# RohitMovva/VexAutonomousPlanner

Measured on NVIDIA B200. Metric: profiled trajectories/sec (8-node paths), higher is better.
Workload: dtype f64

## Files before the change

include/vap.h:

```cpp
#ifndef VAP_H
#define VAP_H

#include <stdint.h>

#ifdef __cplusplus
extern "C" {
#endif

#define VAP_NODE_ATTRS 12
#define VAP_AP_ATTRS 4
#define VAP_FLAG_REVERSE 1
#define VAP_FLAG_STOP 2
#define VAP_FLAG_TANGENT 4

#define VAP_OK 0
#define VAP_ERR_FALSE (-1)
#define VAP_ERR_INDEX (-2)
#define VAP_ERR_VALUE (-3)
#define VAP_ERR_CAPACITY (-4)
#define VAP_ERR_DIVERGED (-5)
#define VAP_ERR_EVENTS (-6)

int vap_version(void);
const char* vap_last_error(void);

int vap_build_path(int64_t B, int N_max, const double* node_attr, const int32_t* node_flags,
                   const int32_t* n_nodes, double* seg, int32_t* first_node, double* param_end,
                   double* seglen, int32_t* n_splines, int32_t* status, double* scratch, double* params,
                   double* derivs, void* stream);

int vap_fit_splines(int64_t R, int n_max, const int32_t* n_pts, const double* xy, const int32_t* tan_has,
                    const double* tan_in, const double* tan_out, const int32_t* bnd_has, const double* bnd,
                    double* seg, double* seglen, double* params, int32_t* status, double* scratch,
                    const double* deriv_in, double* deriv_out, void* stream);

int vap_eval(int64_t n, const int32_t* path, const double* t, int which, int N_max, const double* seg,
             const int32_t* first_node, const double* param_end, const int32_t* n_splines, double* out,
             void* stream);

int vap_build_lut(int64_t B, int N_max, const double* seg, const int32_t* first_node, const double* param_end,
                  const int32_t* n_splines, const int32_t* status, int samples, int64_t Q_cap, double* lut_d,
                  double* lut_t, double* total_len, void* stream);
int64_t vap_lut_index_row_ints(int64_t Q_cap);
int vap_build_lut_index(int64_t B, const int32_t* n_splines, const int32_t* status, int samples, int64_t Q_cap,
                        const double* lut_d, const double* total_len, int32_t* lut_inv, void* stream);

int vap_build_props(int64_t B, int N_max, const int32_t* n_nodes, const double* seg, const int32_t* first_node,
                    const double* param_end, const int32_t* n_splines, const int32_t* status, int spn,
                    int64_t P_cap, double* prop_k, double* prop_h, void* stream);

int vap_query_tables(int64_t n, const int32_t* path, const double* x, int what, const int32_t* n_nodes,
                     const int32_t* n_splines, int samples, int64_t Q_cap, const double* lut_d,
                     const double* lut_t, const double* total_len, int spn, int64_t P_cap, const double* prop_k,
                     const double* prop_h, double* out, void* stream);

int vap_build_dgrid(int64_t n, double dd, double* dgrid, void* stream);

int vap_dist_sample(int64_t B, const int32_t* n_nodes, const int32_t* n_splines, int32_t* status, int64_t n_grid,
                    const double* dgrid, int samples, int64_t Q_cap, const double* lut_d, const double* lut_t,
                    const double* total_len, int spn, int64_t P_cap, const double* prop_k, const double* prop_h,
                    int64_t D_cap, int32_t* n_samples, double* t, double* kap, double* th, void* stream);

int vap_fwd_bwd(int64_t B, int N_max, int A_max, const double* node_attr, const int32_t* node_flags,
                const int32_t* n_nodes, const double* ap_attr, const int32_t* ap_flags, const int32_t* n_ap,
                const double* cons, const int32_t* status, double dd, double dt, double start_vel, double end_vel,
                int64_t D_cap, const int32_t* n_samples, const double* t, const double* kap, const double* th,
                double* vel, int E_cap, double* max_accels, int32_t* bidx, int32_t* bval, int32_t* n_ev,
                double* t_est, int mode, void* stream);

int vap_dist_sample_events(int64_t B, int N_max, int A_max, const double* node_attr, const int32_t* node_flags,
                           const int32_t* n_nodes, const double* ap_attr, const int32_t* ap_flags, const int32_t* n_ap,
                           const double* cons, const int32_t* n_splines, int32_t* status, int64_t n_grid,
                           const double* dgrid, int samples, int64_t Q_cap, const double* lut_d, const double* lut_t,
                           const double* total_len, int spn, int64_t P_cap, const double* prop_k, const double* prop_h,
                           int64_t D_cap, int32_t* n_samples, double* t, double* kap, double* th, int E_cap,
                           double* max_accels, int32_t* bidx, int32_t* bval, int32_t* n_ev, int32_t* vr_idx,
                           double* vr_val, int32_t* st_idx, int32_t* n_vr, double dt, float* ins_est,
                           int32_t* ev_scratch, const int32_t* lut_inv, void* stream);
int64_t vap_event_scratch_ints(int64_t B, int N_max, int A_max);
int64_t vap_pass_row_slots(int64_t D_cap, int chunks);
int vap_fwd_bwd_chunked(int64_t B, const double* cons, const int32_t* status, double dd, double dt, double start_vel,
                        double end_vel, int64_t D_cap, const int32_t* n_samples, const double* kap, const double* th,
                        int E_cap, const double* max_accels, const int32_t* bidx, const int32_t* bval,
                        const int32_t* n_ev, const int32_t* vr_idx, const double* vr_val, const int32_t* st_idx,
                        const int32_t* n_vr, double* rec, double* statB, double* vel_f, double* vel, float* t_est,
                        int32_t* rounds, int chunks, int mode, void* stream);

int vap_velocity_profile(int64_t B, int N_max, int A_max, const double* node_attr, const int32_t* node_flags,
                         const int32_t* n_nodes, const double* ap_attr, const int32_t* ap_flags, const int32_t* n_ap,
                         const double* cons, const int32_t* n_splines, int32_t* status, int64_t n_grid,
                         const double* dgrid, int samples, int64_t Q_cap, const double* lut_d, const double* lut_t,
                         const double* total_len, int spn, int64_t P_cap, const double* prop_k, const double* prop_h,
                         const int32_t* lut_inv, double dd, double dt, double start_vel, double end_vel, int64_t D_cap,
                         int32_t* n_samples, double* t, double* kap, double* th, int E_cap, double* max_accels,
                         int32_t* bidx, int32_t* bval, int32_t* n_ev, int32_t* vr_idx, double* vr_val, int32_t* st_idx,
                         int32_t* n_vr, float* ins_est, int32_t* ev_scratch, double* rec, double* statB, double* vel_f,
                         double* vel, float* t_est, int32_t* rounds, int chunks, int mode, void* stream);

int vap_resample(int64_t B, int N_max, int A_max, const double* node_attr, const int32_t* node_flags,
                 const int32_t* n_nodes, const double* ap_attr, const int32_t* ap_flags, const int32_t* n_ap,
                 const double* cons, int32_t* status, double dt, double dd, const double* seg,
                 const int32_t* first_node, const double* param_end, const int32_t* n_splines, int samples,
                 int64_t Q_cap, const double* lut_d, const double* lut_t, const double* total_len, int spn,
                 int64_t P_cap, const double* prop_k, const double* prop_h, int64_t D_cap,
                 const int32_t* n_samples, const double* vel, int64_t T_cap, double* out, int32_t* nodes_map,
                 int32_t* actions_map, int32_t* n_maps, int32_t* n_out, double* summary, void* stream);

int vap_time_profile(int64_t B, int N_max, int A_max, const double* node_attr, const int32_t* node_flags,
                     const int32_t* n_nodes, const double* ap_attr, const int32_t* ap_flags, const int32_t* n_ap,
                     const double* cons, int32_t* status, double dt, double dd, const double* seg,
                     const int32_t* first_node, const double* param_end, const int32_t* n_splines, int samples,
                     int64_t Q_cap, const double* lut_d, const double* lut_t, const double* total_len, int spn,
                     int64_t P_cap, const double* prop_k, const double* prop_h, int64_t D_cap,
                     const int32_t* n_samples, const double* vel, int64_t T_cap, double* out, int32_t* nodes_map,
                     int32_t* actions_map, int32_t* n_maps, int32_t* n_out, double* summary, int32_t* n_main,
                     double* stage, int E_cap, int32_t* seg_tab, int32_t* ev_scratch, int64_t out_plane_stride,
                     const int32_t* lut_inv, const double* rden, int64_t n_rden, void* stream);
int vap_build_lerp_recip(int64_t n, double dd, double* rden, void* stream);

int64_t vap_workspace_bytes(int64_t B, int N_max, int A_max, int max_splines, int lut_samples, int samples_per_node,
                            int64_t D_cap, int64_t T_cap, int chunks);
int vap_profile_batch(int64_t B, int N_max, int A_max, int max_splines, const double* node_attr,
                      const int32_t* node_flags, const int32_t* n_nodes, const double* ap_attr, const int32_t* ap_flags,
                      const int32_t* n_ap, const double* cons, double dt, double dd, double start_vel, double end_vel,
                      int lut_samples, int samples_per_node, int64_t D_cap, int64_t T_cap, int chunks, const double* dgrid,
                      int64_t n_grid, const double* rden, int64_t n_rden, void* workspace, int64_t workspace_bytes,
                      double* out, int64_t out_plane_stride, int32_t* n_out, int32_t* nodes_map, int32_t* actions_map,
                      int32_t* n_maps, int32_t* status, double* summary, double* vel, int32_t* n_samples, int64_t* need,
                      void* stream);
int vap_summary(int64_t B, int64_t T_cap, int64_t out_plane_stride, const double* out, const int32_t* n_out,
                const int32_t* status, const double* total_len, double* summary, void* stream);

int vap_gl(int64_t n, const int32_t* path, const int32_t* spl, const double* a, const double* b, int mode,
           int max_iter, int npts, const double* gl_pts, const double* gl_wts, int N_max, const double* seg,
           const int32_t* first_node, const double* param_end, double* out, int32_t* qstatus, void* stream);

int vap_turn_profile(int64_t n, const double* q, int mode, int64_t K_cap, double* out_a, double* out_b,
                     int32_t* counts, void* stream);

int vap_lerp(int64_t n, const double* x, int64_t m, const double* xs, const double* ys, double* out, void* stream);
int vap_wheel_trajectory(int64_t n, const double* lin, const double* ang, double track_width, double* left,
                         double* right, void* stream);

int vap_pack_rows(int64_t B, int64_t T_cap, int64_t out_plane_stride, const double* out, const int32_t* n_out,
                  const int32_t* status, int64_t* offsets, double* dst, void* stream);

int vap_export_rows(int64_t B, int64_t T_cap, int64_t out_plane_stride, const double* out, const int32_t* n_out,
                    const int32_t* status, int64_t* offsets, double* dst, void* stream);

int vap_row_kinds(int64_t B, int N_max, int A_max, const double* node_attr, const int32_t* n_nodes, const double* ap_attr,
                  const int32_t* n_ap, const double* cons, const int32_t* status, double dt, const int32_t* nodes_map,
                  const int32_t* actions_map, const int32_t* n_maps, const int32_t* n_out, int64_t T_cap,
                  const int64_t* offsets, int64_t n_kinds, uint8_t* kinds, void* stream);
int vap_format_doubles(int64_t n, const double* x, char* out32, int32_t* lens, void* stream);
int vap_row_text_stride(void);
int vap_format_rows(int64_t R, const double* rows, const uint8_t* kinds, char* slots, int32_t* lens, void* stream);
int vap_compact_rows(int64_t R, const char* slots, const int32_t* lens, const int64_t* offsets, char* text, void* stream);

int vap_diag_read(uint64_t* out_host, int reset);

int vap_bench_dfma(int64_t ctas, int64_t iters, double* out, void* stream);

int vap_test_div_const(int64_t n, uint64_t seed, double b, uint64_t* bad, void* stream);
int vap_test_div_recip(int64_t n, uint64_t seed, uint64_t* bad, void* stream);

#ifdef __cplusplus
}
#endif
#endif
```

vexautonomousplanner_b200/csrc/vap_device.cuh:

```cuda
#pragma once
#include <cstdint>
#include <math.h>

#define NA 12
enum { A_X = 0, A_Y, A_TURN, A_WAIT, A_MAXVEL, A_MAXACC, A_TX, A_TY, A_INMAG, A_OUTMAG, A_RCOS, A_RSIN };
#define F_REVERSE 1
#define F_STOP 2
#define F_TANGENT 4
#define APA 4
enum { P_T = 0, P_WAIT, P_MAXVEL, P_MAXACC };

#define ST_OK 0
#define ST_FALSE (-1)
#define ST_INDEX (-2)
#define ST_VALUE (-3)
#define ST_CAPACITY (-4)
#define ST_DIVERGED (-5)
#define ST_EVENTS (-6)
#define VAP_ROW_LIMIT 50000000LL

#define VAP_PI 3.141592653589793

__device__ __forceinline__ void cp_async16(void* smem, const void* gmem)
{
    unsigned sa = (unsigned)__cvta_generic_to_shared(smem);
    asm volatile("cp.async.ca.shared.global [%0], [%1], 16;" ::"r"(sa), "l"(gmem));
}
__device__ __forceinline__ void cp_async_commit() { asm volatile("cp.async.commit_group;" ::); }
template <int N>
__device__ __forceinline__ void cp_async_wait() { asm volatile("cp.async.wait_group %0;" ::"n"(N) : "memory"); }

__device__ __forceinline__ void mbar_init(unsigned a, unsigned count)
{
    asm volatile("mbarrier.init.shared::cta.b64 [%0], %1;" ::"r"(a), "r"(count) : "memory");
}
__device__ __forceinline__ void mbar_expect_tx(unsigned a, unsigned bytes)
{
    asm volatile("mbarrier.arrive.expect_tx.shared::cta.b64 _, [%0], %1;" ::"r"(a), "r"(bytes) : "memory");
}
__device__ __forceinline__ void bulk_g2s(unsigned dst, const void* src, unsigned bytes, unsigned mbar)
{
    asm volatile("cp.async.bulk.shared::cluster.global.mbarrier::complete_tx::bytes [%0], [%1], %2, [%3];"
                 ::"r"(dst), "l"(src), "r"(bytes), "r"(mbar) : "memory");
}
__device__ __forceinline__ void mbar_wait(unsigned a, unsigned parity)
{
    asm volatile("{\n"
                 ".reg .pred P1;\n"
                 "LAB_WAIT:\n"
                 "mbarrier.try_wait.parity.shared::cta.b64 P1, [%0], %1;\n"
                 "@P1 bra DONE;\n"
                 "bra LAB_WAIT;\n"
                 "DONE:\n"
                 "}" ::"r"(a), "r"(parity) : "memory");
}

__device__ __forceinline__ void fence_mbar_init() { asm volatile("fence.mbarrier_init.release.cluster;" ::: "memory"); }
__device__ __forceinline__ void fence_proxy_async() { asm volatile("fence.proxy.async.shared::cta;" ::: "memory"); }

#ifdef VAP_BOUNDS_CHECK
#define VAP_DIAG_SITES 32
__device__ unsigned long long g_vap_diag[VAP_DIAG_SITES];
#define VAP_CHECK(site, cond) do { if (!(cond)) atomicAdd(&g_vap_diag[site], 1ull); else atomicAdd(&g_vap_diag[16 + ((site) & 15)], 1ull); } while (0)
#else
#define VAP_CHECK(site, cond) do { } while (0)
#endif

struct PathTile { long long b; unsigned x; };
__device__ __forceinline__ PathTile path_tile(unsigned tiles_x)
{
    PathTile p;
    const unsigned q = blockIdx.x / tiles_x;
    p.b = q; p.x = blockIdx.x - q * tiles_x;
    return p;
}

__device__ __forceinline__ double pymin(double a, double b) { return (b < a) ? b : a; }
__device__ __forceinline__ double pymax(double a, double b) { return (b > a) ? b : a; }
__device__ __forceinline__ double norm1d(double x, double y) { return sqrt(fma(y, y, x * x)); }
__device__ __forceinline__ double norm_ax1(double x, double y) { return sqrt(x * x + y * y); }
__device__ __forceinline__ double frac1(double t) { return t - floor(t); }
__device__ __forceinline__ double pymod_pos(double x, double y)
{
    double m = fmod(x, y);
    if (m != 0.0) { if (m < 0) m += y; } else m = 0.0;
    return m;
}

template <int WHICH>
__device__ __forceinline__ void basis(double t, double* H)
{
    double t2 = t * t, t3 = t2 * t;
    if (WHICH == 0) {
        double t4 = t3 * t, t5 = t4 * t;
        H[0] = 1 - 10 * t3 + 15 * t4 - 6 * t5;
        H[1] = 10 * t3 - 15 * t4 + 6 * t5;
        H[2] = t - 6 * t3 + 8 * t4 - 3 * t5;
        H[3] = -4 * t3 + 7 * t4 - 3 * t5;
        H[4] = 0.5 * t2 - 1.5 * t3 + 1.5 * t4 - 0.5 * t5;
        H[5] = 0.5 * t3 - t4 + 0.5 * t5;
    } else if (WHICH == 1) {
        double t4 = t3 * t;
        H[0] = -30 * t2 + 60 * t3 - 30 * t4;
        H[1] = 30 * t2 - 60 * t3 + 30 * t4;
        H[2] = 1 - 18 * t2 + 32 * t3 - 15 * t4;
        H[3] = -12 * t2 + 28 * t3 - 15 * t4;
        H[4] = t - 4.5 * t2 + 6 * t3 - 2.5 * t4;
        H[5] = 1.5 * t2 - 4 * t3 + 2.5 * t4;
    } else {
        H[0] = -60 * t + 180 * t2 - 120 * t3;
        H[1] = 60 * t - 180 * t2 + 120 * t3;
        H[2] = -36 * t + 96 * t2 - 60 * t3;
        H[3] = -24 * t + 84 * t2 - 60 * t3;
        H[4] = 1 - 9 * t + 18 * t2 - 10 * t3;
        H[5] = 3 * t - 12 * t2 + 10 * t3;
    }
}

__device__ __forceinline__ void normalize_param(double t, int nseg, double pend, int& idx, double& u)
{
    double tt = pymax(0.0, pymin(t, pend));
    idx = (int)tt;
    if (idx == nseg) idx = nseg - 1;
    u = tt - (double)idx;
}

template <int WHICH>
__device__ __forceinline__ void eval_spline(const double* __restrict__ seg, int nseg, double pend, double t,
                                            double& ox, double& oy)
{
    int idx; double u;
    normalize_param(t, nseg, pend, idx, u);
    double H[6];
    basis<WHICH>(u, H);
    const double2* s = reinterpret_cast<const double2*>(seg + (size_t)idx * 12);
    double ax = 0.0, ay = 0.0;
#pragma unroll
    for (int i = 0; i < 6; i++) { double2 r = __ldg(s + i); ax += H[i] * r.x; ay += H[i] * r.y; }
    ox = ax; oy = ay;
}

__device__ __forceinline__ void eval_spline_d12(const double* __restrict__ seg, int nseg, double pend, double t,
                                                double& dx, double& dy, double& ddx, double& ddy)
{
    int idx; double u;
    normalize_param(t, nseg, pend, idx, u);
    double H1[6], H2[6];
    basis<1>(u, H1);
    basis<2>(u, H2);
    const double2* s = reinterpret_cast<const double2*>(seg + (size_t)idx * 12);
    double ax = 0.0, ay = 0.0, bx = 0.0, by = 0.0;
#pragma unroll
    for (int i = 0; i < 6; i++) {
        double2 r = __ldg(s + i);
        ax += H1[i] * r.x; ay += H1[i] * r.y;
        bx += H2[i] * r.x; by += H2[i] * r.y;
    }
    dx = ax; dy = ay; ddx = bx; ddy = by;
}

struct PathGeo {
    const double* seg;
    const int* first;
    const double* pend;
    int S;
};
__device__ __forceinline__ int map_spline(const PathGeo& g, double t)
{
    int k = 0;
    if (g.S <= 8) {
        while (k < g.S - 1 && !(t <= (double)g.first[k + 1])) k++;
    } else {
        int lo = 0, hi = g.S - 1;
        while (lo < hi) {
            int mid = (lo + hi) >> 1;
            if (t <= (double)g.first[mid + 1]) hi = mid; else lo = mid + 1;
        }
        k = lo;
    }
    return k;
}
__device__ __forceinline__ PathGeo path_geo(long long b, int N_max, const double* seg, const int* first_node,
                                            const double* param_end, const int* n_splines)
{
    PathGeo g;
    g.seg = seg + (size_t)b * (N_max - 1) * 12;
    g.first = first_node + (size_t)b * (N_max + 1);
    g.pend = param_end + (size_t)b * N_max;
    g.S = n_splines[b];
    return g;
}

template <int WHICH>
__device__ __forceinline__ void eval_path(const PathGeo& g, double t, double& ox, double& oy)
{
    int k = map_spline(g, t);
    int f0 = g.first[k], f1 = g.first[k + 1];
    eval_spline<WHICH>(g.seg + (size_t)f0 * 12, f1 - f0, g.pend[k], t - (double)f0, ox, oy);
}
__device__ __forceinline__ void eval_path_d12(const PathGeo& g, double t, double& dx, double& dy, double& ddx,
                                              double& ddy)
{
    int k = map_spline(g, t);
    int f0 = g.first[k], f1 = g.first[k + 1];
    eval_spline_d12(g.seg + (size_t)f0 * 12, f1 - f0, g.pend[k], t - (double)f0, dx, dy, ddx, ddy);
}

__device__ __forceinline__ void curv_heading(double dx, double dy, double ddx, double ddy, double& kap, double& th)
{
    double s2 = dx * dx + dy * dy;
    double num = dx * ddy - dy * ddx;
// ... 208 lines not shown
```

vexautonomousplanner_b200/csrc/vap_kernels.cu:

```cuda
#include <cuda_runtime.h>
#include <cstdio>
#include <cstring>
#include <cstdlib>

#include "../../include/vap.h"
#include "vap_device.cuh"
#include "vap_velocity.cuh"
#include "vap_timeloop.cuh"
#include "vap_format.cuh"

static thread_local char g_err[512] = "";
static int set_err(const char* where, cudaError_t e)
{
    snprintf(g_err, sizeof(g_err), "%s: %s", where, cudaGetErrorString(e));
    return -100;
}
static int arg_err(const char* msg)
{
    snprintf(g_err, sizeof(g_err), "%s", msg);
    return -101;
}
#define CHECK_LAUNCH(name)                                   \
    do {                                                     \
        cudaError_t e__ = cudaGetLastError();                \
// ... 999 lines not shown
    CHECK_LAUNCH("vap_build_dgrid");
    return 0;
}

extern "C" int vap_build_lerp_recip(int64_t n, double dd, double* rden, void* stream)
{
    if (n <= 0) return 0;
    k_build_lerp_recip<<<blocks_for(n, 256), 256, 0, STREAM>>>(n, dd, rden);
    CHECK_LAUNCH("vap_build_lerp_recip");
    return 0;
}

extern "C" int vap_dist_sample(int64_t B, const int32_t* n_nodes, const int32_t* n_splines, int32_t* status,
                               int64_t n_grid, const double* dgrid, int samples, int64_t Q_cap, const double* lut_d,
                               const double* lut_t, const double* total_len, int spn, int64_t P_cap,
                               const double* prop_k, const double* prop_h, int64_t D_cap, int32_t* n_samples,
                               double* t, double* kap, double* th, void* stream)
{
    if (B <= 0) return 0;
    k_count_samples<<<blocks_for(B, 128), 128, 0, STREAM>>>(B, status, status, n_grid, dgrid, total_len, D_cap, n_samples);
    CHECK_LAUNCH("vap_dist_sample/count");
    const unsigned tx = blocks_for(D_cap, 256);
    if ((long long)tx * B > 2147483647LL) return arg_err("vap_dist_sample: more than 2^31 CTAs (tile the batch)");
    const unsigned grid = tx * (unsigned)B;
    k_dist_sample<<<grid, 256, 0, STREAM>>>(n_nodes, n_splines, status, dgrid, samples, Q_cap, lut_d, lut_t, total_len,
                                            spn, P_cap, prop_k, prop_h, D_cap, n_samples, t, kap, th, tx);
    CHECK_LAUNCH("vap_dist_sample");
    return 0;
}

extern "C" int vap_fwd_bwd(int64_t B, int N_max, int A_max, const double* node_attr, const int32_t* node_flags,
                           const int32_t* n_nodes, const double* ap_attr, const int32_t* ap_flags, const int32_t* n_ap,
                           const double* cons, const int32_t* status, double dd, double dt, double start_vel,
                           double end_vel, int64_t D_cap, const int32_t* n_samples, const double* t, const double* kap,
                           const double* th, double* vel, int E_cap, double* max_accels, int32_t* bidx, int32_t* bval,
                           int32_t* n_ev, double* t_est, int mode, void* stream)
{
    if (B <= 0) return 0;
    if (E_cap < N_max + A_max + 2) return arg_err("vap_fwd_bwd: E_cap < N_max + A_max + 2");
    k_fwd_bwd<<<blocks_for(B, 32), 32, 0, STREAM>>>(B, N_max, A_max, node_attr, node_flags, n_nodes, ap_attr, ap_flags,
                                                   n_ap, cons, status, dd, dt, start_vel, end_vel, D_cap, n_samples, t,
                                                   kap, th, vel, E_cap, max_accels, bidx, bval, n_ev, t_est, mode);
    CHECK_LAUNCH("vap_fwd_bwd");
    return 0;
}

extern "C" int vap_resample(int64_t B, int N_max, int A_max, const double* node_attr, const int32_t* node_flags,
                            const int32_t* n_nodes, const double* ap_attr, const int32_t* ap_flags, const int32_t* n_ap,
                            const double* cons, int32_t* status, double dt, double dd, const double* seg,
                            const int32_t* first_node, const double* param_end, const int32_t* n_splines, int samples,
                            int64_t Q_cap, const double* lut_d, const double* lut_t, const double* total_len, int spn,
                            int64_t P_cap, const double* prop_k, const double* prop_h, int64_t D_cap,
                            const int32_t* n_samples, const double* vel, int64_t T_cap, double* out,
                            int32_t* nodes_map, int32_t* actions_map, int32_t* n_maps, int32_t* n_out, double* summary,
                            void* stream)
{
    if (B <= 0) return 0;
    k_resample<<<blocks_for(B, 32), 32, 0, STREAM>>>(B, N_max, A_max, node_attr, node_flags, n_nodes, ap_attr, ap_flags,
                                                    n_ap, cons, status, dt, dd, seg, first_node, param_end, n_splines,
                                                    samples, Q_cap, lut_d, lut_t, total_len, spn, P_cap, prop_k, prop_h,
                                                    D_cap, n_samples, vel, T_cap, out, nodes_map, actions_map, n_maps,
                                                    n_out, summary, 0, 0);
    CHECK_LAUNCH("vap_resample");
    return 0;
}

extern "C" int vap_gl(int64_t n, const int32_t* path, const int32_t* spl, const double* a, const double* b, int mode,
                      int max_iter, int npts, const double* gl_pts, const double* gl_wts, int N_max, const double* seg,
                      const int32_t* first_node, const double* param_end, double* out, int32_t* qstatus, void* stream)
{
    if (n <= 0) return 0;
    if (npts < 1 || npts > 128) return arg_err("vap_gl: npts must be in [1, 128]");
    k_gl<<<blocks_for(n, 64), 64, 0, STREAM>>>(n, path, spl, a, b, mode, max_iter, npts, gl_pts, gl_wts, N_max, seg,
                                              first_node, param_end, out, qstatus);
    CHECK_LAUNCH("vap_gl");
    return 0;
}

extern "C" int vap_turn_profile(int64_t n, const double* q, int mode, int64_t K_cap, double* out_a, double* out_b,
                                int32_t* counts, void* stream)
{
    if (n <= 0) return 0;
    k_turn_profile<<<blocks_for(n, 64), 64, 0, STREAM>>>(n, q, mode, K_cap, out_a, out_b, counts);
    CHECK_LAUNCH("vap_turn_profile");
    return 0;
}

extern "C" int vap_lerp(int64_t n, const double* x, int64_t m, const double* xs, const double* ys, double* out,
                        void* stream)
{
    if (n <= 0) return 0;
    if (m < 1) return arg_err("vap_lerp: empty table");
    k_lerp<<<blocks_for(n, 128), 128, 0, STREAM>>>(n, x, m, xs, ys, out);
    CHECK_LAUNCH("vap_lerp");
    return 0;
}

extern "C" int vap_wheel_trajectory(int64_t n, const double* lin, const double* ang, double track_width, double* left,
                                    double* right, void* stream)
{
    if (n <= 0) return 0;
    k_wheel<<<blocks_for(n, 256), 256, 0, STREAM>>>(n, lin, ang, track_width, left, right);
    CHECK_LAUNCH("vap_wheel_trajectory");
    return 0;
}

extern "C" int vap_dist_sample_events(int64_t B, int N_max, int A_max, const double* node_attr,
                                      const int32_t* node_flags, const int32_t* n_nodes, const double* ap_attr,
                                      const int32_t* ap_flags, const int32_t* n_ap, const double* cons,
                                      const int32_t* n_splines, int32_t* status, int64_t n_grid, const double* dgrid,
                                      int samples, int64_t Q_cap, const double* lut_d, const double* lut_t,
                                      const double* total_len, int spn, int64_t P_cap, const double* prop_k,
                                      const double* prop_h, int64_t D_cap, int32_t* n_samples, double* t, double* kap,
                                      double* th, int E_cap, double* max_accels, int32_t* bidx, int32_t* bval,
                                      int32_t* n_ev, int32_t* vr_idx, double* vr_val, int32_t* st_idx, int32_t* n_vr,
                                      double dt, float* ins_est, int32_t* ev_scratch, const int32_t* lut_inv,
                                      void* stream)
{
    if (B <= 0) return 0;
    if (E_cap < N_max + A_max + 2) return arg_err("vap_dist_sample_events: E_cap < N_max + A_max + 2");
    int Am = A_max > 0 ? A_max : 1;
    int32_t* ev_wrap = ev_scratch;
    int32_t* ev_nwrap = ev_wrap + (size_t)B * N_max;
    int32_t* ev_apc = ev_nwrap + B;
    int32_t* ev_napc = ev_apc + (size_t)B * Am * EV_AP_CAND;
    cudaError_t e = cudaMemsetAsync(ev_nwrap, 0, sizeof(int32_t) * (size_t)B, STREAM);
    if (e != cudaSuccess) return set_err("vap_dist_sample_events/memset", e);
    e = cudaMemsetAsync(ev_napc, 0, sizeof(int32_t) * (size_t)B * Am, STREAM);
    if (e != cudaSuccess) return set_err("vap_dist_sample_events/memset", e);
    k_count_samples<<<blocks_for(B, 128), 128, 0, STREAM>>>(B, status, status, n_grid, dgrid, total_len, D_cap, n_samples);
    CHECK_LAUNCH("vap_dist_sample_events/count");
    const unsigned tx = blocks_for(D_cap, 256);
    if ((long long)tx * B > 2147483647LL) return arg_err("vap_dist_sample_events: more than 2^31 CTAs (tile the batch)");
    const unsigned grid = tx * (unsigned)B;
    k_dist_sample_ev<<<grid, 256, 0, STREAM>>>(N_max, Am, n_nodes, n_splines, status, ap_attr, n_ap, dgrid, samples, Q_cap,
                                               lut_d, lut_t, total_len, spn, P_cap, prop_k, prop_h, D_cap, n_samples, t,
                                               kap, th, ev_wrap, ev_nwrap, ev_apc, ev_napc, lut_inv, tx);
    CHECK_LAUNCH("vap_dist_sample_events/sample");
    k_resolve_events<<<blocks_for(B, 64), 64, 0, STREAM>>>(B, N_max, Am, node_attr, node_flags, n_nodes, ap_attr, ap_flags,
                                                          n_ap, cons, status, ev_wrap, ev_nwrap, ev_apc, ev_napc, E_cap,
                                                          max_accels, bidx, bval, n_ev, vr_idx, vr_val, st_idx, n_vr, dt, ins_est);
    CHECK_LAUNCH("vap_dist_sample_events/resolve");
    return 0;
}

extern "C" int64_t vap_event_scratch_ints(int64_t B, int N_max, int A_max)
{
    int Am = A_max > 0 ? A_max : 1;
    return B * N_max + B + B * Am * EV_AP_CAND + B * Am;
}

extern "C" int64_t vap_pass_row_slots(int64_t D_cap, int chunks) { return ((D_cap + 8 * (int64_t)chunks + 64 + 1) / 2) * 2; }

template <int NT, bool TMA>
static int launch_passes_v(int64_t B, size_t ss, cudaStream_t st, const double* cons, const int32_t* status, double dd, double dt,
                           double start_vel, double end_vel, long long RS, long long D_cap, const int32_t* n_samples,
                           const double* rec, int E_cap, const double* max_accels, const int32_t* bidx, const int32_t* bval,
                           const int32_t* n_ev, const int32_t* vr_idx, const double* vr_val, const int32_t* st_idx,
                           const int32_t* n_vr, double* vel_f, double* vel, float* t_est, int32_t* rounds, bool backward,
                           int warm, int max_rounds, const double* statB)
{
    const int warps = (NT + 31) / 32;
    const int ring_off = (int)((ss + 127) / 128 * 128);
    const int planes = backward ? 6 : 5;
    const size_t smem = TMA ? (size_t)ring_off + (size_t)warps * (2 * planes * TMA_PLANE_DOUBLES * 8 + 16) : ss;
    cudaError_t e = cudaSuccess;
    if (!backward) {
        if (smem > 48 * 1024) e = cudaFuncSetAttribute(k_fwd_chunked<NT, TMA>, cudaFuncAttributeMaxDynamicSharedMemorySize, (int)smem);
        if (e != cudaSuccess) return set_err("vap_fwd_bwd_chunked/attr", e);
        k_fwd_chunked<NT, TMA><<<(unsigned)B, NT, smem, st>>>(status, cons, dd, start_vel, end_vel, RS, n_samples, rec, E_cap,
                                                             max_accels, bidx, bval, n_ev, vr_idx, vr_val, st_idx, n_vr, vel_f,
                                                             rounds, warm, max_rounds, ring_off);
    } else {
        if (smem > 48 * 1024) e = cudaFuncSetAttribute(k_bwd_chunked<NT, TMA>, cudaFuncAttributeMaxDynamicSharedMemorySize, (int)smem);
        if (e != cudaSuccess) return set_err("vap_fwd_bwd_chunked/attr", e);
        k_bwd_chunked<NT, TMA><<<(unsigned)B, NT, smem, st>>>(status, cons, dd, dt, end_vel, RS, D_cap, n_samples, rec, E_cap,
                                                             max_accels, bidx, bval, n_ev, vel_f, vel, t_est, rounds, warm,
                                                             max_rounds, statB, ring_off);
    }
    return 0;
}
template <int NT, typename... Args>
static int launch_passes(bool tma, Args... args)
{
    return tma ? launch_passes_v<NT, true>(args...) : launch_passes_v<NT, false>(args...);
}

static int run_passes(int64_t B, const double* cons, const int32_t* status, double dd, double dt, double start_vel,
                      double end_vel, int64_t D_cap, const int32_t* n_samples, int E_cap, const double* max_accels,
                      const int32_t* bidx, const int32_t* bval, const int32_t* n_ev, const int32_t* vr_idx,
                      const double* vr_val, const int32_t* st_idx, const int32_t* n_vr, const double* rec,
                      const double* statB, double* vel_f, double* vel, float* t_est, int32_t* rounds, int chunks, int mode,
                      cudaStream_t stream)
{
    const long long RS = vap_pass_row_slots(D_cap, chunks);
    const size_t VC = 3 * (size_t)E_cap + 2;
    const size_t ss = ((size_t)chunks * 4 + E_cap + VC) * sizeof(double) + (E_cap + VC) * sizeof(int);
    int warm = 0, max_rounds = 1 << 30;
    if (const char* ev = getenv("VAP_CHUNK_WARM")) warm = atoi(ev);
#ifdef VAP_DIAG_MAXROUNDS
    if (const char* ev = getenv("VAP_CHUNK_MAXROUNDS")) max_rounds = atoi(ev);
#endif
    if (warm < 0) warm = 0;
    bool tma = true;
    if (const char* ev = getenv("VAP_PASS_TMA")) tma = atoi(ev) != 0;
    auto passes = [&](bool backward) -> int {
        switch (chunks) {
#define VAP_PASS_CASE(N_) case N_: return launch_passes<N_>(tma, B, ss, STREAM, cons, status, dd, dt, start_vel, end_vel, RS, D_cap,   \
                                              n_samples, rec, E_cap, max_accels, bidx, bval, n_ev, vr_idx, vr_val, st_idx, n_vr,  \
                                              vel_f, vel, t_est, rounds, backward, warm, max_rounds, statB);
            VAP_PASS_CASE(8) VAP_PASS_CASE(16) VAP_PASS_CASE(32) VAP_PASS_CASE(64) VAP_PASS_CASE(128) VAP_PASS_CASE(256)
#undef VAP_PASS_CASE
        }
        return 0;
    };
    if (int rc = passes(false)) return rc;
    CHECK_LAUNCH("vap_fwd_bwd_chunked/fwd");
    if (mode == 1) {
        const unsigned tx2 = blocks_for(D_cap, 256);
        if ((long long)tx2 * B > 2147483647LL) return arg_err("vap_fwd_bwd_chunked: more than 2^31 CTAs (tile the batch)");
        k_untranspose<<<tx2 * (unsigned)B, 256, 0, STREAM>>>(status, n_samples, D_cap, RS, chunks, vel_f, vel, tx2);
        CHECK_LAUNCH("vap_fwd_bwd_chunked/untranspose");
        return 0;
    }
    if (int rc = passes(true)) return rc;
    CHECK_LAUNCH("vap_fwd_bwd_chunked/bwd");
    return 0;
}

static int check_pass_args(const char* who, int64_t B, int64_t D_cap, int chunks)
{
    (void)B;
    if (chunks < 8 || chunks > 256 || (chunks & (chunks - 1)) != 0) { snprintf(g_err, sizeof(g_err), "%s: chunks must be a power of two in 8 .. 256", who); return -1; }
    if (D_cap > 400000000LL) { snprintf(g_err, sizeof(g_err), "%s: D_cap too large", who); return -1; }
    if (D_cap & 1) { snprintf(g_err, sizeof(g_err), "%s: D_cap must be even (the passes move 16-byte pairs)", who); return -1; }
    return 0;
}

extern "C" int vap_fwd_bwd_chunked(int64_t B, const double* cons, const int32_t* status, double dd, double dt,
                                   double start_vel, double end_vel, int64_t D_cap, const int32_t* n_samples,
                                   const double* kap, const double* th, int E_cap, const double* max_accels,
                                   const int32_t* bidx, const int32_t* bval, const int32_t* n_ev, const int32_t* vr_idx,
                                   const double* vr_val, const int32_t* st_idx, const int32_t* n_vr, double* rec,
                                   double* statB, double* vel_f, double* vel, float* t_est, int32_t* rounds,
                                   int chunks, int mode, void* stream)
{
    if (B <= 0) return 0;
    if (check_pass_args("vap_fwd_bwd_chunked", B, D_cap, chunks)) return -1;
    const long long RS = vap_pass_row_slots(D_cap, chunks);
    const unsigned tx = blocks_for(D_cap + 4 * chunks, 256 * PP_TILES);
    if ((long long)tx * B > 2147483647LL) return arg_err("vap_fwd_bwd_chunked: more than 2^31 CTAs (tile the batch)");
    const unsigned grid = tx * (unsigned)B;
    const size_t sm = 2 * 2 * sizeof(double) * (size_t)prepass_tile_cols(chunks) * prepass_tile_stride(chunks);
    k_prepass<<<grid, 256, sm, STREAM>>>(status, cons, D_cap, n_samples, kap, th, chunks, RS, rec, E_cap, max_accels, bidx,
                                         bval, n_ev, statB, tx);
    CHECK_LAUNCH("vap_fwd_bwd_chunked/prepass");
    return run_passes(B, cons, status, dd, dt, start_vel, end_vel, D_cap, n_samples, E_cap, max_accels, bidx, bval, n_ev, vr_idx,
                      vr_val, st_idx, n_vr, rec, statB, vel_f, vel, t_est, rounds, chunks, mode, STREAM);
}

extern "C" int vap_velocity_profile(int64_t B, int N_max, int A_max, const double* node_attr, const int32_t* node_flags,
                                    const int32_t* n_nodes, const double* ap_attr, const int32_t* ap_flags,
                                    const int32_t* n_ap, const double* cons, const int32_t* n_splines, int32_t* status,
                                    int64_t n_grid, const double* dgrid, int samples, int64_t Q_cap, const double* lut_d,
                                    const double* lut_t, const double* total_len, int spn, int64_t P_cap,
                                    const double* prop_k, const double* prop_h, const int32_t* lut_inv, double dd, double dt,
                                    double start_vel, double end_vel, int64_t D_cap, int32_t* n_samples, double* t,
                                    double* kap, double* th, int E_cap, double* max_accels, int32_t* bidx, int32_t* bval,
                                    int32_t* n_ev, int32_t* vr_idx, double* vr_val, int32_t* st_idx, int32_t* n_vr,
                                    float* ins_est, int32_t* ev_scratch, double* rec, double* statB, double* vel_f,
                                    double* vel, float* t_est, int32_t* rounds, int chunks, int mode, void* stream)
{
    if (B <= 0) return 0;
    if (E_cap < N_max + A_max + 2) return arg_err("vap_velocity_profile: E_cap < N_max + A_max + 2");
    if (check_pass_args("vap_velocity_profile", B, D_cap, chunks)) return -1;
    if ((t != nullptr) != (kap != nullptr) || (t != nullptr) != (th != nullptr))
        return arg_err("vap_velocity_profile: t, kap and th are inspection outputs: pass all three or none");
    int Am = A_max > 0 ? A_max : 1;
    int32_t* ev_wrap = ev_scratch;
    int32_t* ev_nwrap = ev_wrap + (size_t)B * N_max;
    int32_t* ev_apc = ev_nwrap + B;
    int32_t* ev_napc = ev_apc + (size_t)B * Am * EV_AP_CAND;
    cudaError_t e = cudaMemsetAsync(ev_nwrap, 0, sizeof(int32_t) * (size_t)B, STREAM);
    if (e != cudaSuccess) return set_err("vap_velocity_profile/memset", e);
    e = cudaMemsetAsync(ev_napc, 0, sizeof(int32_t) * (size_t)B * Am, STREAM);
    if (e != cudaSuccess) return set_err("vap_velocity_profile/memset", e);
    k_count_samples<<<blocks_for(B, 128), 128, 0, STREAM>>>(B, status, status, n_grid, dgrid, total_len, D_cap, n_samples);
    CHECK_LAUNCH("vap_velocity_profile/count");
    const long long RS = vap_pass_row_slots(D_cap, chunks);
    const unsigned tx = blocks_for(D_cap + 4 * chunks, 256 * SP_TILES);
    if ((long long)tx * B > 2147483647LL) return arg_err("vap_velocity_profile: more than 2^31 CTAs (tile the batch)");
    const int tc = prepass_tile_cols(chunks);
    const size_t sm = 2 * 3 * sizeof(double) * (size_t)tc * (((256 / tc) + 2) | 1);
    k_sample_prepass<<<tx * (unsigned)B, 256, sm, STREAM>>>(N_max, Am, n_nodes, n_splines, status, cons, ap_attr, n_ap, dgrid,
                                                           samples, Q_cap, lut_d, lut_t, total_len, spn, P_cap, prop_k, prop_h,
                                                           D_cap, n_samples, t, kap, th, ev_wrap, ev_nwrap, ev_apc, ev_napc,
                                                           lut_inv, chunks, RS, rec, tx);
    CHECK_LAUNCH("vap_velocity_profile/sample_prepass");
    k_resolve_events<<<blocks_for(B, 64), 64, 0, STREAM>>>(B, N_max, Am, node_attr, node_flags, n_nodes, ap_attr, ap_flags,
                                                          n_ap, cons, status, ev_wrap, ev_nwrap, ev_apc, ev_napc, E_cap,
                                                          max_accels, bidx, bval, n_ev, vr_idx, vr_val, st_idx, n_vr, dt, ins_est);
    CHECK_LAUNCH("vap_velocity_profile/resolve");
    k_prepass_ovr<<<(unsigned)B, 256, 0, STREAM>>>(status, cons, n_samples, chunks, RS, rec, E_cap, max_accels, bidx, bval, n_ev,
                                                  statB);
    CHECK_LAUNCH("vap_velocity_profile/prepass_ovr");
    return run_passes(B, cons, status, dd, dt, start_vel, end_vel, D_cap, n_samples, E_cap, max_accels, bidx, bval, n_ev, vr_idx,
                      vr_val, st_idx, n_vr, rec, statB, vel_f, vel, t_est, rounds, chunks, mode, STREAM);
}

extern "C" int vap_time_profile(int64_t B, int N_max, int A_max, const double* node_attr, const int32_t* node_flags,
                                const int32_t* n_nodes, const double* ap_attr, const int32_t* ap_flags,
                                const int32_t* n_ap, const double* cons, int32_t* status, double dt, double dd,
                                const double* seg, const int32_t* first_node, const double* param_end,
                                const int32_t* n_splines, int samples, int64_t Q_cap, const double* lut_d,
                                const double* lut_t, const double* total_len, int spn, int64_t P_cap,
                                const double* prop_k, const double* prop_h, int64_t D_cap, const int32_t* n_samples,
                                const double* vel, int64_t T_cap, double* out, int32_t* nodes_map,
                                int32_t* actions_map, int32_t* n_maps, int32_t* n_out, double* summary,
                                int32_t* n_main, double* stage, int E_cap, int32_t* seg_tab, int32_t* ev_scratch,
                                int64_t out_plane_stride, const int32_t* lut_inv, const double* rden, int64_t n_rden,
                                void* stream)
{
    const long long oplane = out_plane_stride > 0 ? out_plane_stride : B * T_cap;
    if (B <= 0) return 0;
    if (E_cap < N_max + A_max + 2) return arg_err("vap_time_profile: E_cap < N_max + A_max + 2");
    int Am = A_max > 0 ? A_max : 1;
    const int64_t M_cap = T_cap;
    int32_t* ev_wrap = ev_scratch;
    int32_t* ev_nwrap = ev_wrap + (size_t)B * N_max;
    int32_t* ev_apc = ev_nwrap + B;
    int32_t* ev_napc = ev_apc + (size_t)B * Am * EV_AP_CAND;
    int32_t* seg_k = seg_tab;
    int32_t* seg_off = seg_k + (size_t)B * E_cap;
    int32_t* seg_rev = seg_off + (size_t)B * E_cap;
    int32_t* n_seg = seg_rev + (size_t)B * E_cap;
    cudaError_t e = cudaMemsetAsync(ev_nwrap, 0, sizeof(int32_t) * (size_t)B, STREAM);
    if (e != cudaSuccess) return set_err("vap_time_profile/memset", e);
    e = cudaMemsetAsync(ev_napc, 0, sizeof(int32_t) * (size_t)B * Am, STREAM);
    if (e != cudaSuccess) return set_err("vap_time_profile/memset", e);
    if (D_cap % 128 != 0) return arg_err("vap_time_profile: D_cap must be a multiple of 128 (rows are staged in 128-sample blocks)");
    int lanes = (int)((B + 591) / 592);
    if (lanes > 10) lanes = 10;
    if (const char* ev = getenv("VAP_STATE_LANES")) lanes = atoi(ev);
    lanes = lanes < 1 ? 1 : (lanes > 32 ? 32 : lanes);
    bool big = B > 148 * 32;
    if (const char* ev = getenv("VAP_STATE_BLK")) big = atoi(ev) == 64;
    const size_t ring_bytes = (size_t)lanes * ((big ? ts_stride(64) : ts_stride(128)) * sizeof(double) + 16);
    if (ring_bytes > 48 * 1024) {
        const int mx = (int)(32 * (ts_stride(128) * sizeof(double) + 16));
        cudaError_t ea = big ? cudaFuncSetAttribute(k_time_state<64>, cudaFuncAttributeMaxDynamicSharedMemorySize, mx)
                             : cudaFuncSetAttribute(k_time_state<128>, cudaFuncAttributeMaxDynamicSharedMemorySize, mx);
        if (ea != cudaSuccess) return set_err("vap_time_profile/attr", ea);
    }
    if (big)
        k_time_state<64><<<blocks_for(B, lanes), lanes, ring_bytes, STREAM>>>(B, cons, status, dt, dd, total_len, D_cap, n_samples,
                                                                             vel, M_cap, stage, n_main, rden, rden ? n_rden : 0);
    else
        k_time_state<128><<<blocks_for(B, lanes), lanes, ring_bytes, STREAM>>>(B, cons, status, dt, dd, total_len, D_cap, n_samples,
                                                                              vel, M_cap, stage, n_main, rden, rden ? n_rden : 0);
    CHECK_LAUNCH("vap_time_profile/state");
    const unsigned tx = blocks_for(M_cap, 256);
    if ((long long)tx * B > 2147483647LL) return arg_err("vap_time_profile: more than 2^31 CTAs (tile the batch)");
    const unsigned grid = tx * (unsigned)B;
    k_time_sample<<<grid, 256, 0, STREAM>>>(B, N_max, Am, n_nodes, status, ap_attr, n_ap, seg, first_node, param_end,
                                            n_splines, samples, Q_cap, lut_d, lut_t, total_len, spn, P_cap, prop_k, prop_h,
                                            M_cap, n_main, stage, ev_wrap, ev_nwrap, ev_apc, ev_napc, lut_inv, tx);
    CHECK_LAUNCH("vap_time_profile/sample");
    k_time_events<<<blocks_for(B, lanes), lanes, 0, STREAM>>>(B, N_max, Am, node_attr, node_flags, n_nodes, ap_attr, n_ap, cons,
                                                       status, dt, seg, first_node, param_end, n_splines, spn, P_cap,
                                                       prop_h, total_len, M_cap, n_main, stage, ev_wrap, ev_nwrap, ev_apc,
                                                       ev_napc, E_cap, seg_k, seg_off, seg_rev, n_seg, T_cap, oplane,
                                                       out, nodes_map, actions_map, n_maps, n_out, summary);
    CHECK_LAUNCH("vap_time_profile/events");
    k_time_finalize<<<grid, 256, 0, STREAM>>>(B, status, M_cap, n_main, stage, E_cap, seg_k, seg_off, seg_rev, n_seg,
                                              T_cap, oplane, out, summary, tx);
    CHECK_LAUNCH("vap_time_profile/finalize");
    k_resample<<<blocks_for(B, 32), 32, 0, STREAM>>>(B, N_max, A_max, node_attr, node_flags, n_nodes, ap_attr, ap_flags, n_ap,
                                                    cons, status, dt, dd, seg, first_node, param_end, n_splines, samples,
                                                    Q_cap, lut_d, lut_t, total_len, spn, P_cap, prop_k, prop_h, D_cap,
                                                    n_samples, vel, T_cap, out, nodes_map, actions_map, n_maps, n_out,
                                                    summary, oplane, ST_EVENTS);
    CHECK_LAUNCH("vap_time_profile/serial redo");
    return 0;
}

__global__ void __launch_bounds__(256) k_bench_dfma(long long iters, double* __restrict__ out)
{
    double a[8];
#pragma unroll
    for (int k = 0; k < 8; k++) a[k] = 1.0 + 1e-9 * (double)(threadIdx.x + 37 * k);
    const double m = 0.9999999, c = 1e-7;
    for (long long i = 0; i < iters; i++) {
#pragma unroll
        for (int k = 0; k < 8; k++) a[k] = fma(a[k], m, c);
    }
    double s = 0.0;
#pragma unroll
    for (int k = 0; k < 8; k++) s += a[k];
    if (s == 123456.789) out[0] = s;
}
extern "C" int vap_bench_dfma(int64_t ctas, int64_t iters, double* out, void* stream)
{
    if (ctas <= 0 || iters <= 0) return 0;
    k_bench_dfma<<<(unsigned)ctas, 256, 0, STREAM>>>(iters, out);
    CHECK_LAUNCH("vap_bench_dfma");
    return 0;
}

extern "C" int vap_test_div_const(int64_t n, uint64_t seed, double b, uint64_t* bad, void* stream)
{
    if (n <= 0) return 0;
    k_test_div_const<<<blocks_for(n, 256), 256, 0, STREAM>>>(n, seed, b, reinterpret_cast<unsigned long long*>(bad));
    CHECK_LAUNCH("vap_test_div_const");
    return 0;
}

__global__ void k_test_div_recip(long long n, unsigned long long seed, unsigned long long* __restrict__ bad)
{
    long long i = (long long)blockIdx.x * blockDim.x + threadIdx.x;
    if (i >= n) return;
    auto mix = [](unsigned long long z) {
        z = (z ^ (z >> 30)) * 0xBF58476D1CE4E5B9ULL; z = (z ^ (z >> 27)) * 0x94D049BB133111EBULL; return z ^ (z >> 31);
    };
    unsigned long long z1 = mix(seed + 0x9E3779B97F4A7C15ULL * (unsigned long long)(2 * i + 1));
    unsigned long long z2 = mix(seed + 0x9E3779B97F4A7C15ULL * (unsigned long long)(2 * i + 2));
    int e1 = (int)((z1 >> 52) % 118) - 110 + 1023;
    unsigned long long nb = ((z1 >> 63) << 63) | ((unsigned long long)e1 << 52) | (z1 & 0x000FFFFFFFFFFFFFULL);
    if (((z1 >> 40) & 63) == 0) nb &= 0x8000000000000000ULL;
    double num = __longlong_as_double((long long)nb);
    int e2 = (int)((z2 >> 52) % 60) - 57 + 1023;
    unsigned long long gb = ((unsigned long long)e2 << 52) | (z2 & 0x000FFFFFFFFFFFFFULL);
    if (((z2 >> 40) & 63) == 1) gb |= 0x000FFFFFFFFFFFFFULL;
    double g = __longlong_as_double((long long)gb);
    if (((z2 >> 46) & 31) == 0) g = 0.0;
    const double rc = recip_for_pass(g);
    const double q1 = accel_ang_fast(num, g, rc);
    double n2 = num, g2 = g;
    asm volatile("" : "+d"(n2), "+d"(g2));
    const double q2 = n2 / g2;
    bool same = (__double_as_longlong(q1) == __double_as_longlong(q2)) || (q1 != q1 && q2 != q2) || (q1 == 0.0 && q2 == 0.0);
    if (!same) atomicAdd(bad, 1ULL);
}
extern "C" int vap_test_div_recip(int64_t n, uint64_t seed, uint64_t* bad, void* stream)
{
    if (n <= 0) return 0;
    k_test_div_recip<<<blocks_for(n, 256), 256, 0, STREAM>>>(n, seed, reinterpret_cast<unsigned long long*>(bad));
    CHECK_LAUNCH("vap_test_div_recip");
    return 0;
}

extern "C" int vap_pack_rows(int64_t B, int64_t T_cap, int64_t out_plane_stride, const double* out, const int32_t* n_out,
                             const int32_t* status, int64_t* offsets, double* dst, void* stream)
{
    if (B <= 0) return 0;
    const long long oplane = out_plane_stride > 0 ? out_plane_stride : B * T_cap;
    k_row_offsets<<<1, 1024, 0, STREAM>>>(B, n_out, status, T_cap, reinterpret_cast<long long*>(offsets));
    CHECK_LAUNCH("vap_pack_rows/offsets");
    int ctas = 16;
    if (const char* ev = getenv("VAP_PACK_CTAS")) ctas = atoi(ev);
    if (ctas < 1) ctas = 1;
    k_pack_rows<<<ctas, 256, 0, STREAM>>>(B, n_out, status, T_cap, oplane, out, reinterpret_cast<const long long*>(offsets), dst);
    CHECK_LAUNCH("vap_pack_rows");
    return 0;
}

extern "C" int vap_export_rows(int64_t B, int64_t T_cap, int64_t out_plane_stride, const double* out, const int32_t* n_out,
                               const int32_t* status, int64_t* offsets, double* dst, void* stream)
{
    if (B <= 0) return 0;
    const long long oplane = out_plane_stride > 0 ? out_plane_stride : B * T_cap;
    k_row_offsets<<<1, 1024, 0, STREAM>>>(B, n_out, status, T_cap, reinterpret_cast<long long*>(offsets));
    CHECK_LAUNCH("vap_export_rows/offsets");
    const unsigned tx = blocks_for(T_cap, 256);
    if ((long long)tx * B > 2147483647LL) return arg_err("vap_export_rows: more than 2^31 CTAs (tile the batch)");
    const unsigned grid = tx * (unsigned)B;
    k_export_rows<<<grid, 256, 0, STREAM>>>(B, n_out, status, T_cap, oplane, out, reinterpret_cast<const long long*>(offsets), dst, tx);
    CHECK_LAUNCH("vap_export_rows");
    return 0;
}

extern "C" int vap_format_doubles(int64_t n, const double* x, char* out32, int32_t* lens, void* stream)
{
    if (n <= 0) return 0;
    k_format_doubles<<<blocks_for(n, 256), 256, 0, STREAM>>>(n, x, out32, lens);
    CHECK_LAUNCH("vap_format_doubles");
    return 0;
}
extern "C" int vap_row_text_stride(void) { return VAP_ROW_STRIDE; }
__global__ void k_row_kinds(long long B, int N_max, int A_max, const double* __restrict__ node_attr,
                            const int* __restrict__ n_nodes, const double* __restrict__ ap_attr, const int* __restrict__ n_ap,
                            const double* __restrict__ cons, const int* __restrict__ status, double dt,
                            const int* __restrict__ nodes_map, const int* __restrict__ actions_map,
                            const int* __restrict__ n_maps, const int* __restrict__ n_out, long long T_cap,
                            const long long* __restrict__ offsets, unsigned char* __restrict__ kinds)
{
    long long b = (long long)blockIdx.x * blockDim.x + threadIdx.x;
    if (b >= B || status[b] != ST_OK) return;
    long long T = n_out[b];
    if (T > T_cap) T = T_cap;
    unsigned char* kr = kinds + (offsets ? offsets[b] : b * T_cap);
    auto mark = [&](long long r0, long long cnt, unsigned char k) {
        for (long long r = r0; r < r0 + cnt && r < T; r++) if (r >= 0) kr[r] |= k;
    };
    const double* na = node_attr + (size_t)b * N_max * NA;
    const double V = cons[b * 6 + 0], max_acc = cons[b * 6 + 1], w = cons[b * 6 + 5];
    if (na[A_WAIT] > 0) mark(0, (long long)(na[A_WAIT] / dt), RK_INSERTED | RK_OMEGA_INT | RK_POS_INT);
    else if (T > 0) kr[0] |= RK_TIME_INT;
    const int nm = n_maps[2 * b], am = n_maps[2 * b + 1];
    const int* nmap = nodes_map + (size_t)b * (N_max + 1);
    const int n = n_nodes[b];
    for (int i = 1; i < nm - 1 && i < n; i++) {
        const double* a = na + (size_t)i * NA;
        long long r = nmap[i];
        if (a[A_TURN] != 0) {
            const double angle = a[A_TURN] * (VAP_PI / 180.0);
            const Trapezoid tz = trapezoid_setup(V, max_acc, fabs(angle) * w / 2, dt);
            mark(r, 1, RK_INSERTED | RK_OMEGA_INT);
            mark(r + 1, tz.K - 1, RK_INSERTED);
            r += tz.K;
        }
        if (a[A_WAIT] > 0) mark(r, (long long)(a[A_WAIT] / dt), RK_INSERTED | RK_OMEGA_INT | RK_POS_INT);
    }
    const int* amap = actions_map + (size_t)b * (A_max > 0 ? A_max : 1);
    const int A = n_ap ? n_ap[b] : 0;
    for (int j = 0; j < am && j < A; j++) {
        const double wt = ap_attr[((size_t)b * A_max + j) * APA + P_WAIT];
        if (wt > 0) mark(amap[j], (long long)(wt / dt), RK_INSERTED | RK_OMEGA_INT | RK_POS_INT);
    }
}

extern "C" int vap_row_kinds(int64_t B, int N_max, int A_max, const double* node_attr, const int32_t* n_nodes,
                             const double* ap_attr, const int32_t* n_ap, const double* cons, const int32_t* status,
                             double dt, const int32_t* nodes_map, const int32_t* actions_map, const int32_t* n_maps,
                             const int32_t* n_out, int64_t T_cap, const int64_t* offsets, int64_t n_kinds, uint8_t* kinds,
                             void* stream)
{
    if (B <= 0 || n_kinds <= 0) return 0;
    cudaError_t e = cudaMemsetAsync(kinds, 0, (size_t)n_kinds, STREAM);
    if (e != cudaSuccess) return set_err("vap_row_kinds/memset", e);
    k_row_kinds<<<blocks_for(B, 64), 64, 0, STREAM>>>(B, N_max, A_max, node_attr, n_nodes, ap_attr, n_ap, cons, status, dt,
                                                     nodes_map, actions_map, n_maps, n_out, T_cap,
                                                     reinterpret_cast<const long long*>(offsets), kinds);
    CHECK_LAUNCH("vap_row_kinds");
    return 0;
}

extern "C" int vap_format_rows(int64_t R, const double* rows, const uint8_t* int_time, char* slots, int32_t* lens, void* stream)
{
    if (R <= 0) return 0;
    k_format_rows<<<blocks_for(R, 128), 128, 0, STREAM>>>(R, rows, int_time, slots, lens);
    CHECK_LAUNCH("vap_format_rows");
    return 0;
}
extern "C" int vap_compact_rows(int64_t R, const char* slots, const int32_t* lens, const int64_t* offsets, char* text,
                                void* stream)
{
    if (R <= 0) return 0;
    k_compact_rows<<<blocks_for(R * 32, 256), 256, 0, STREAM>>>(R, slots, lens, reinterpret_cast<const long long*>(offsets), text);
    CHECK_LAUNCH("vap_compact_rows");
    return 0;
}

#define VAP_DIST_LIMIT 5.0e7
#define VAP_TIME_LIMIT 1.0e7

__global__ void k_flag_lengths(long long B, const int* __restrict__ gstatus, const double* __restrict__ total_len, double dd,
                               int* __restrict__ status)
{
    long long b = (long long)blockIdx.x * blockDim.x + threadIdx.x;
    if (b >= B) return;
    int s = gstatus[b];
    if (s == ST_OK && total_len[b] / dd > VAP_DIST_LIMIT) s = ST_DIVERGED;
    status[b] = s;
}
__global__ void k_flag_times(long long B, int* __restrict__ status, const int* __restrict__ n_samples,
                             const float* __restrict__ t_est, const float* __restrict__ ins_est,
                             unsigned long long* __restrict__ need)
{
    long long b = (long long)blockIdx.x * blockDim.x + threadIdx.x;
    if (b >= B) return;
    const int s = status[b];
    if (s != ST_OK && s != ST_CAPACITY) return;
    atomicMax(need, (unsigned long long)(n_samples[b] > 0 ? n_samples[b] : 0));
    if (s != ST_OK) return;
    const float est = t_est[b] + ins_est[b];
    if (!(est < (float)VAP_TIME_LIMIT)) { status[b] = ST_DIVERGED; return; }
    atomicMax(need + 1, (unsigned long long)est);
}
__global__ void k_need_rows(long long B, const int* __restrict__ status, const int* __restrict__ n_main,
                            const float* __restrict__ ins_est, unsigned long long* __restrict__ need)
{
    long long b = (long long)blockIdx.x * blockDim.x + threadIdx.x;
    if (b >= B) return;
    const int s = status[b];
    if (s == ST_OK || s == ST_CAPACITY)
        atomicMax(need + 2, (unsigned long long)(n_main[b] > 0 ? n_main[b] : 0) + (unsigned long long)ceilf(ins_est[b]) + 8ull);
}

struct WsCarver {
    char* base; size_t off;
    template <typename T> T* take(size_t n)
    {
        off = (off + 255) & ~(size_t)255;
        T* p = base ? reinterpret_cast<T*>(base + off) : nullptr;
        off += n * sizeof(T);
        return p;
    }
};
struct BatchScratch {
    double *seg, *param_end, *seglen, *scratch9, *lut_d, *lut_t, *total_len, *prop_k, *prop_h, *ma, *vr_val, *rec, *statB, *vel_f,
           *stage;
    int32_t *first_node, *n_splines, *gstatus, *lut_inv, *bidx, *bval, *n_ev, *vr_idx, *st_idx, *n_vr, *scr, *rounds, *seg_tab,
            *scr2, *n_main;
    float *ins_est, *t_est;
    unsigned long long* need;
    int64_t Q_cap, P_cap, RS; int E_cap;
};
static size_t carve_batch(char* base, int64_t B, int N_max, int A_max, int max_splines, int samples, int spn, int64_t D_cap,
                          int64_t T_cap, int chunks, BatchScratch& s)
{
    WsCarver w{base, 0};
    const int S = max_splines > 0 ? max_splines : 1;
    s.Q_cap = (int64_t)samples * S; s.P_cap = (int64_t)spn * N_max; s.E_cap = N_max + A_max + 2;
    s.RS = vap_pass_row_slots(D_cap, chunks);
    const size_t nscr = (size_t)vap_event_scratch_ints(B, N_max, A_max);
    s.seg = w.take<double>((size_t)B * (N_max > 1 ? N_max - 1 : 1) * 12);
    s.first_node = w.take<int32_t>((size_t)B * (N_max + 1));
    s.param_end = w.take<double>((size_t)B * N_max);
    s.seglen = w.take<double>((size_t)B * N_max);
    s.n_splines = w.take<int32_t>(B);
    s.gstatus = w.take<int32_t>(B);
    s.scratch9 = w.take<double>((size_t)B * N_max * 9);
    s.lut_d = w.take<double>((size_t)B * s.Q_cap);
    s.lut_t = w.take<double>((size_t)B * s.Q_cap);
    s.total_len = w.take<double>(B);
    s.lut_inv = w.take<int32_t>((size_t)B * vap_lut_index_row_ints(s.Q_cap));
    s.prop_k = w.take<double>((size_t)B * s.P_cap);
    s.prop_h = w.take<double>((size_t)B * s.P_cap);
    s.ma = w.take<double>((size_t)B * s.E_cap);
    s.bidx = w.take<int32_t>((size_t)B * s.E_cap);
    s.bval = w.take<int32_t>((size_t)B * s.E_cap);
    s.n_ev = w.take<int32_t>((size_t)B * 2);
    s.vr_idx = w.take<int32_t>((size_t)B * s.E_cap);
    s.vr_val = w.take<double>((size_t)B * s.E_cap);
    s.st_idx = w.take<int32_t>((size_t)B * s.E_cap);
    s.n_vr = w.take<int32_t>((size_t)B * 2);
    s.ins_est = w.take<float>(B);
    s.t_est = w.take<float>(B);
    s.scr = w.take<int32_t>(nscr);
    s.rounds = w.take<int32_t>((size_t)B * 2);
    s.rec = w.take<double>((size_t)B * s.RS * 5);
    s.statB = w.take<double>((size_t)B * s.RS);
    s.vel_f = w.take<double>((size_t)B * s.RS);
    s.stage = w.take<double>((size_t)8 * B * (T_cap + 1));
    s.seg_tab = w.take<int32_t>((size_t)3 * B * s.E_cap + B);
    s.scr2 = w.take<int32_t>(nscr);
    s.n_main = w.take<int32_t>(B);
    s.need = w.take<unsigned long long>(4);
    return (w.off + 255) & ~(size_t)255;
}

static int check_batch_args(const char* who, int64_t B, int N_max, int A_max, int max_splines, int samples, int spn,
                            int64_t D_cap, int64_t T_cap, int chunks)
{
    if (B < 0 || N_max < 2 || A_max < 0 || max_splines < 1 || max_splines > N_max || samples < 2 || spn < 2 || T_cap < 1) {
        snprintf(g_err, sizeof(g_err), "%s: bad sizes", who); return -1;
    }
    if (D_cap < 128 || D_cap % 128 != 0) { snprintf(g_err, sizeof(g_err), "%s: D_cap must be a positive multiple of 128", who); return -1; }
    return check_pass_args(who, B, D_cap, chunks);
}

extern "C" int64_t vap_workspace_bytes(int64_t B, int N_max, int A_max, int max_splines, int lut_samples, int samples_per_node,
                                       int64_t D_cap, int64_t T_cap, int chunks)
{
    if (check_batch_args("vap_workspace_bytes", B, N_max, A_max, max_splines, lut_samples, samples_per_node, D_cap, T_cap, chunks))
        return -1;
    BatchScratch s;
    return (int64_t)carve_batch(nullptr, B, N_max, A_max, max_splines, lut_samples, samples_per_node, D_cap, T_cap, chunks, s);
}

extern "C" int vap_profile_batch(int64_t B, int N_max, int A_max, int max_splines, const double* node_attr,
                                 const int32_t* node_flags, const int32_t* n_nodes, const double* ap_attr,
                                 const int32_t* ap_flags, const int32_t* n_ap, const double* cons, double dt, double dd,
                                 double start_vel, double end_vel, int lut_samples, int samples_per_node, int64_t D_cap,
                                 int64_t T_cap, int chunks, const double* dgrid, int64_t n_grid, const double* rden,
                                 int64_t n_rden, void* workspace, int64_t workspace_bytes, double* out,
                                 int64_t out_plane_stride, int32_t* n_out, int32_t* nodes_map, int32_t* actions_map,
                                 int32_t* n_maps, int32_t* status, double* summary, double* vel, int32_t* n_samples,
                                 int64_t* need, void* stream)
{
    if (B == 0) return 0;
    if (check_batch_args("vap_profile_batch", B, N_max, A_max, max_splines, lut_samples, samples_per_node, D_cap, T_cap, chunks))
        return -1;
    if (!dgrid || n_grid < D_cap + 2) return arg_err("vap_profile_batch: dgrid (vap_build_dgrid) must hold at least D_cap + 2 entries");
    if (!workspace) return arg_err("vap_profile_batch: workspace is NULL");
    BatchScratch s;
    const size_t bytes = carve_batch(static_cast<char*>(workspace), B, N_max, A_max, max_splines, lut_samples, samples_per_node,
                                     D_cap, T_cap, chunks, s);
    if ((int64_t)bytes > workspace_bytes) return arg_err("vap_profile_batch: workspace smaller than vap_workspace_bytes(...)");
    if ((reinterpret_cast<uintptr_t>(workspace) & 255) != 0) return arg_err("vap_profile_batch: workspace must be 256-byte aligned");
    cudaError_t e = cudaMemsetAsync(s.need, 0, 4 * sizeof(unsigned long long), STREAM);
    if (e != cudaSuccess) return set_err("vap_profile_batch/memset", e);
    int rc;
    if ((rc = vap_build_path(B, N_max, node_attr, node_flags, n_nodes, s.seg, s.first_node, s.param_end, s.seglen, s.n_splines,
                             s.gstatus, s.scratch9, nullptr, nullptr, stream))) return rc;
    if ((rc = vap_build_lut(B, N_max, s.seg, s.first_node, s.param_end, s.n_splines, s.gstatus, lut_samples, s.Q_cap, s.lut_d,
                            s.lut_t, s.total_len, stream))) return rc;
    if ((rc = vap_build_lut_index(B, s.n_splines, s.gstatus, lut_samples, s.Q_cap, s.lut_d, s.total_len, s.lut_inv, stream))) return rc;
    if ((rc = vap_build_props(B, N_max, n_nodes, s.seg, s.first_node, s.param_end, s.n_splines, s.gstatus, samples_per_node,
                              s.P_cap, s.prop_k, s.prop_h, stream))) return rc;
    k_flag_lengths<<<blocks_for(B, 128), 128, 0, STREAM>>>(B, s.gstatus, s.total_len, dd, status);
    CHECK_LAUNCH("vap_profile_batch/flag_lengths");
    if ((rc = vap_velocity_profile(B, N_max, A_max, node_attr, node_flags, n_nodes, ap_attr, ap_flags, n_ap, cons, s.n_splines,
                                   status, n_grid, dgrid, lut_samples, s.Q_cap, s.lut_d, s.lut_t, s.total_len, samples_per_node,
                                   s.P_cap, s.prop_k, s.prop_h, s.lut_inv, dd, dt, start_vel, end_vel, D_cap, n_samples, nullptr,
                                   nullptr, nullptr, s.E_cap, s.ma, s.bidx, s.bval, s.n_ev, s.vr_idx, s.vr_val, s.st_idx, s.n_vr,
                                   s.ins_est, s.scr, s.rec, s.statB, s.vel_f, vel, s.t_est, s.rounds, chunks, 0, stream))) return rc;
    k_flag_times<<<blocks_for(B, 128), 128, 0, STREAM>>>(B, status, n_samples, s.t_est, s.ins_est, s.need);
    CHECK_LAUNCH("vap_profile_batch/flag_times");
    if ((rc = vap_time_profile(B, N_max, A_max, node_attr, node_flags, n_nodes, ap_attr, ap_flags, n_ap, cons, status, dt, dd,
                               s.seg, s.first_node, s.param_end, s.n_splines, lut_samples, s.Q_cap, s.lut_d, s.lut_t, s.total_len,
                               samples_per_node, s.P_cap, s.prop_k, s.prop_h, D_cap, n_samples, vel, T_cap, out, nodes_map,
                               actions_map, n_maps, n_out, summary, s.n_main, s.stage, s.E_cap, s.seg_tab, s.scr2,
                               out_plane_stride, s.lut_inv, rden, rden ? n_rden : 0, stream))) return rc;
    k_need_rows<<<blocks_for(B, 128), 128, 0, STREAM>>>(B, status, s.n_main, s.ins_est, s.need);
    CHECK_LAUNCH("vap_profile_batch/need_rows");
    if (need) {
        e = cudaMemcpyAsync(need, s.need, 3 * sizeof(int64_t), cudaMemcpyDeviceToDevice, STREAM);
        if (e != cudaSuccess) return set_err("vap_profile_batch/need", e);
    }
    return 0;
}

__global__ void __launch_bounds__(128) k_summary(long long T_cap, long long plane, const double* __restrict__ out,
                                                 const int* __restrict__ n_out, const int* __restrict__ status,
                                                 const double* __restrict__ total_len, double* __restrict__ summary)
{
    const long long b = blockIdx.x;
    __shared__ double s_m[128];
    const int st = status[b];
    const long long T = (st == ST_OK) ? n_out[b] : 0;
    const double* v = out + 2 * plane + (size_t)b * T_cap;
    double m = 0.0;
    for (long long i = threadIdx.x; i < T; i += blockDim.x) m = fmax(m, fabs(v[i]));
    s_m[threadIdx.x] = m;
    __syncthreads();
    for (int k = 64; k > 0; k >>= 1) { if ((int)threadIdx.x < k) s_m[threadIdx.x] = fmax(s_m[threadIdx.x], s_m[threadIdx.x + k]); __syncthreads(); }
    if (threadIdx.x == 0) {
        double* r = summary + (size_t)b * 5;
        r[0] = (double)n_out[b]; r[1] = total_len ? total_len[b] : 0.0;
        r[2] = T > 0 ? out[(size_t)b * T_cap + T - 1] : 0.0; r[3] = s_m[0]; r[4] = (double)st;
    }
}
extern "C" int vap_summary(int64_t B, int64_t T_cap, int64_t out_plane_stride, const double* out, const int32_t* n_out,
                           const int32_t* status, const double* total_len, double* summary, void* stream)
{
    if (B <= 0) return 0;
    const long long plane = out_plane_stride > 0 ? out_plane_stride : B * T_cap;
    k_summary<<<(unsigned)B, 128, 0, STREAM>>>(T_cap, plane, out, n_out, status, total_len, summary);
    CHECK_LAUNCH("vap_summary");
    return 0;
}

extern "C" int vap_diag_read(uint64_t* out_host, int reset)
{
#ifdef VAP_BOUNDS_CHECK
    cudaError_t e = cudaMemcpyFromSymbol(out_host, g_vap_diag, sizeof(unsigned long long) * VAP_DIAG_SITES);
    if (e != cudaSuccess) return set_err("vap_diag_read", e);
    if (reset) {
        unsigned long long z[VAP_DIAG_SITES] = {0};
        e = cudaMemcpyToSymbol(g_vap_diag, z, sizeof(z));
        if (e != cudaSuccess) return set_err("vap_diag_read/reset", e);
    }
    return 0;
#else
    (void)out_host; (void)reset;
    return arg_err("vap_diag_read: this build has no bounds diagnostics (compile with -DVAP_BOUNDS_CHECK)");
#endif
}
```

vexautonomousplanner_b200/csrc/vap_velocity.cuh:

```cuda
#pragma once
#include "vap_device.cuh"

#define EV_AP_CAND 4

__device__ __forceinline__ double4 ldg_d4(const double4* p)
{
    const double2* q = reinterpret_cast<const double2*>(p);
    double2 a = __ldg(q), b = __ldg(q + 1);
    return make_double4(a.x, a.y, b.x, b.y);
}

__global__ void __launch_bounds__(256, 8) k_dist_sample_ev(
    int N_max, int A_max, const int* __restrict__ n_nodes, const int* __restrict__ n_splines,
    const int* __restrict__ status, const double* __restrict__ ap_attr, const int* __restrict__ n_ap,
    const double* __restrict__ dgrid, int samples, long long Q_cap, const double* __restrict__ lut_d,
    const double* __restrict__ lut_t, const double* __restrict__ total_len, int spn, long long P_cap,
    const double* __restrict__ prop_k, const double* __restrict__ prop_h, long long D_cap,
    const int* __restrict__ n_samples, double* __restrict__ t_out, double* __restrict__ kap, double* __restrict__ th,
    int* __restrict__ ev_wrap, int* __restrict__ ev_nwrap, int* __restrict__ ev_apc, int* __restrict__ ev_napc,
    const int* __restrict__ lut_inv, unsigned tiles_x)
{
    __shared__ double s_t[257];
    const PathTile pt = path_tile(tiles_x);
    long long b = pt.b;
// ... 439 lines not shown
        const int e = c * Lc + s;
        if (s >= Lc || e >= steps) continue;
        const int tl = (c - c0) * st + (s - s0) + 1;
        {
            const double t = t_t[tl], tp = t_t[tl - 1];
            if (frac1(tp) > frac1(t) && t < tn) {
                const int slot = atomicAdd(ev_nwrap + b, 1);
                if (slot < N_max) ev_wrap[(size_t)b * N_max + slot] = e;
            }
            for (int q = 0; q < A; q++) {
                const double x = ap_attr[((size_t)b * A_max + q) * APA + P_T];
                if (tp < x && t >= x) {
                    const int slot = atomicAdd(ev_napc + (size_t)b * A_max + q, 1);
                    if (slot < EV_AP_CAND) ev_apc[((size_t)b * A_max + q) * EV_AP_CAND + slot] = e;
                }
            }
        }
        const double gh = 2 * fabs(t_th[tl + 1] - t_th[tl]);
        const size_t o = (size_t)(j >> (sh + 2)) * (5 * PS) + (size_t)(j & (PS - 1));
        VAP_CHECK(9, tl >= 1 && tl + 1 < TC * st && o + 4 * PS < (size_t)(5 * RS - 3) && c - c0 >= 0 && c - c0 < TC && s - s0 >= 0 && s - s0 < TR);
        const SampleTerms tm = prepass_sample<false>(V, A0, A0, w, s_c[0], s_c[1], t_k[tl]);
        pr[o] = tm.ak; pr[o + PS] = tm.G; pr[o + 2 * PS] = tm.stat; pr[o + 3 * PS] = gh; pr[o + 4 * PS] = recip_for_pass(gh);
        if (e == steps - 1) {
            double kl, hl;
            snap_gather2_32(pk, ph, tn, pg, kl, hl);
            const SampleTerms u = prepass_sample<false>(V, A0, A0, w, s_c[0], s_c[1], kl);
            pr[5 * RS - 3] = u.ak; pr[5 * RS - 2] = u.G; pr[5 * RS - 1] = u.stat;
            if (t_out) { t_out[orow + D - 1] = tn; kap_out[orow + D - 1] = kl; th_out[orow + D - 1] = hl; }
        }
    }
}

__global__ void __launch_bounds__(256) k_prepass_ovr(
    const int* __restrict__ status, const double* __restrict__ cons, const int* __restrict__ n_samples, int NT, long long RS,
    double* __restrict__ rec, int E_cap, const double* __restrict__ max_accels, const int* __restrict__ bidx,
    const int* __restrict__ bval, const int* __restrict__ n_ev, double* __restrict__ statB)
{
    const long long b = blockIdx.x;
    if (status[b] != ST_OK) return;
    const double A0 = cons[b * 6 + 1];
    if (!pass_has_override(max_accels + (size_t)b * E_cap, n_ev[2 * b], A0)) return;
    const int D = n_samples[b];
    const int steps = D - 1;
    if (steps <= 0) return;
    const int sh = 31 - __clz(NT);
    const int Lc = chunk_len(steps, NT);
    const double V = cons[b * 6 + 0], w = cons[b * 6 + 5];
    const double mav = 2 * V / w, maa = 2 * A0 / w;
    const int PS = PB * NT;
    double* pr = rec + (size_t)b * RS * 5;
    const int nb = n_ev[2 * b + 1];
    const double dec_b = max_accels[(size_t)b * E_cap + bval[(size_t)b * E_cap + nb - 1]];
    for (int j = threadIdx.x; j < (Lc << sh); j += blockDim.x) {
        const int c = (j >> 2) & (NT - 1);
        const int s = ((j >> (sh + 2)) << 2) + (j & 3);
        const int e = c * Lc + s;
        if (e >= steps) continue;
        const size_t o = (size_t)(j >> (sh + 2)) * (5 * PS) + (size_t)(j & (PS - 1));
        const double acc_f = max_accels[(size_t)b * E_cap + bval[(size_t)b * E_cap + last_le(bidx + (size_t)b * E_cap, nb, e)]];
        const SampleTerms t = prepass_sample<true>(V, acc_f, dec_b, w, mav, maa, pr[o]);
        pr[o + 2 * PS] = t.stat;
        statB[(size_t)b * RS + j] = t.stat_b;
        if (e == steps - 1) {
            const SampleTerms u = prepass_sample<true>(V, dec_b, dec_b, w, mav, maa, pr[5 * RS - 3]);
            pr[5 * RS - 1] = u.stat;
            statB[(size_t)b * RS + RS - 1] = u.stat_b;
        }
    }
}

__device__ __forceinline__ bool same_bits(double a, double b)
{
    return __double_as_longlong(a) == __double_as_longlong(b);
}

__device__ __noinline__ double accel_ang_div(double num, double h2)
{
    bool special = !(h2 > 0.0) || num == 0.0 || !(fabs(num) < 1e300);
    double n = special ? 1.0 : num, d = special ? 1.0 : h2;
    asm volatile("" : "+d"(n), "+d"(d));
    double q = n / d;
    if (!special) return q;
    const double qnan = __longlong_as_double(0x7ff8000000000000LL);
    const double inf = __longlong_as_double(0x7ff0000000000000LL);
    if (h2 > 0.0) {
        if (num == 0.0) return num;
        return (num != num) ? qnan : copysign(inf, num);
    }
    if (h2 == 0.0) {
        if (num > 0.0) return inf;
        if (num < 0.0) return -inf;
        return qnan;
    }
    return qnan;
}

__device__ __forceinline__ double recip_for_pass(double g)
{
    const long long bits = __double_as_longlong(g);
    const bool safe = (g >= 2.2250738585072014e-308) && (g < 1e300) &&
                      ((bits & 0x000FFFFFFFFFFFFFLL) != 0x000FFFFFFFFFFFFFLL);
    double d = safe ? g : 1.0;
    asm volatile("" : "+d"(d));
    const double r = 1.0 / d;
    return safe ? r : ((g == 0.0) ? __longlong_as_double(0x7ff0000000000000LL) : -1.0);
}

__device__ __forceinline__ double accel_ang_fast(double num, double h2, double rce)
{
    const double q0 = num * rce;
    double q = fma(fma(-h2, q0, num), rce, q0);
    q = fma(fma(-h2, q, num), rce, q);
    const bool corr = rce <= 1.7976931348623157e308;
    const double an = fabs(num);
    const bool in_range = (an < 1e200) && ((an > 1e-200) || (num == 0.0));
    if (rce < 0.0 || (corr && !in_range)) return accel_ang_div(num, h2);
    return corr ? q : q0;
}

__device__ __forceinline__ double fwd_step(double ak, double gh, double rg, double stat, double cap, double v, double& sq,
                                           double acc, double hw, double dd)
{
    const double ang_vel = v * ak;
    const double sqn = ang_vel * ang_vel;
    const double rce = (ak < 1e-6) ? __longlong_as_double(0x7ff8000000000000LL) : rg;
    const double accel_ang = accel_ang_fast(sqn - sq, gh, rce);
    const double x = fabs(accel_ang) * hw;
    const double l = acc + x, rr = acc - x;
    double a_wheel = (fabs(l) < fabs(rr)) ? l : rr;
    if (a_wheel < 0) a_wheel = 0;
    const double a = pymin(stat, a_wheel);
    const double s = sqrt(v * v + 2 * a * dd);
    sq = sqn;
    return pymin(cap, s);
}
__device__ __forceinline__ double bwd_step(double ak, double gh, double rg, double stat, double cap, double v, double& sq,
                                           double acc, double hw, double dd)
{
    const double ang_vel = v * ak;
    const double sqn = ang_vel * ang_vel;
    const double rce = (ak < 1e-6) ? __longlong_as_double(0x7ff8000000000000LL) : rg;
    const double accel_ang = accel_ang_fast(sqn - sq, gh, rce);
    const double x = accel_ang * hw;
    const double l = acc + x, rr = acc - x;
    double a_wheel = (fabs(l) < fabs(rr)) ? l : rr;
    if (a_wheel < 0) a_wheel = 0;
    const double dcl = pymin(stat, a_wheel);
    const double pv = sqrt(v * v + 2 * dcl * dd);
    sq = sqn;
    return pymin(pv, cap);
}

#define CH_INT_MAX 2147483647
#ifndef VAP_PASS_REGS
#define VAP_PASS_REGS 72
#endif
#ifndef VAP_PASS_REGS_TMA
#define VAP_PASS_REGS_TMA 112
#endif

__device__ __forceinline__ double2 ldg_d2(const double* p) { return __ldg(reinterpret_cast<const double2*>(p)); }
__device__ __forceinline__ void st_d2(double* p, double x, double y) { *reinterpret_cast<double2*>(p) = make_double2(x, y); }

#define RERUN_PF 4
__device__ __forceinline__ void l2_prefetch(const void* g) { asm volatile("prefetch.global.L2 [%0];" ::"l"(g)); }

__device__ __forceinline__ float t_est_term(double va, double vb, float dd_over_dt)
{
    const float vm = 0.5f * ((float)va + (float)vb);
    return __fdividef(dd_over_dt, fmaxf(vm, 0.05f));
}

struct FwdTables {
    const int* bi; const double* acc; int n_b;
    const int* vi; const double* vv; int n_v;
};

#define RUN_SWEEP 0
#define RUN_RERUN 1
#define RUN_DRY 2
template <int NT, int MODE>
__device__ __forceinline__ bool fwd_run(const double* __restrict__ p, double* __restrict__ q, double* __restrict__ tail,
                                        double old_end, int lo, int len, const FwdTables& T, double hw,
                                        double dd, double& v, double& sq, bool prev_same)
{
    constexpr int PS = PB * NT, BS = 5 * PS;
    constexpr bool RERUN = (MODE == RUN_RERUN);
    constexpr bool DRY = (MODE == RUN_DRY);
    constexpr bool SWEEP = (MODE == RUN_SWEEP);
    int j = 0;
    while (j + 1 < T.n_b && T.bi[j + 1] <= lo) j++;
    double acc = T.acc[j];
    int nb_next = (j + 1 < T.n_b) ? T.bi[j + 1] : CH_INT_MAX;
    int jv = 0;
    while (jv + 1 < T.n_v && T.vi[jv + 1] <= lo + 1) jv++;
    double v0n = T.vv[jv];
    int nv_next = (jv + 1 < T.n_v) ? T.vi[jv + 1] : CH_INT_MAX;
    int e = lo;
    const int hi = lo + len;
#define FWD_ONE(AK_, G_, ST_, GH_, RG_, OLD_)                                                                        \
        if (e == nb_next) { j++; acc = T.acc[j]; nb_next = (j + 1 < T.n_b) ? T.bi[j + 1] : CH_INT_MAX; }              \
        if (e + 1 == nv_next) { jv++; v0n = T.vv[jv]; nv_next = (jv + 1 < T.n_v) ? T.vi[jv + 1] : CH_INT_MAX; }      \
        v = fwd_step(AK_, GH_, RG_, ST_, pymin(v0n, G_), v, sq, acc, hw, dd);                                        \
        if (RERUN) {                                                                                                 \
            const bool same = same_bits(OLD_, v);                                                                    \
            if (same && prev_same) return true;               \
            prev_same = same;                                                                                        \
        }                                                                                                            \
        ++e;
    double2 akA = ldg_d2(p), GA = ldg_d2(p + PS), stA = ldg_d2(p + 2 * PS), ghA = ldg_d2(p + 3 * PS), rgA = ldg_d2(p + 4 * PS);
    double2 akB, GB, stB, ghB, rgB;
    double2 oA = make_double2(0.0, 0.0), oB = oA;
    if (RERUN) oA = *reinterpret_cast<const double2*>(q);
    if (RERUN) {
#pragma unroll
        for (int k = 1; k < RERUN_PF; k++)
            if (k < (len >> 2)) {
#pragma unroll
                for (int f = 0; f < 5; f++) l2_prefetch(p + (size_t)k * BS + f * PS);
                l2_prefetch(q + (size_t)k * PS);
            }
    }
    for (int blk = len >> 2; blk > 0; --blk) {
        if (RERUN && blk > RERUN_PF) {
#pragma unroll
            for (int f = 0; f < 5; f++) l2_prefetch(p + (size_t)RERUN_PF * BS + f * PS);
            l2_prefetch(q + (size_t)RERUN_PF * PS);
        }
        akB = ldg_d2(p + 2); GB = ldg_d2(p + PS + 2); stB = ldg_d2(p + 2 * PS + 2); ghB = ldg_d2(p + 3 * PS + 2); rgB = ldg_d2(p + 4 * PS + 2);
        if (RERUN) oB = *reinterpret_cast<const double2*>(q + 2);
        const double vin = v;
        FWD_ONE(akA.x, GA.x, stA.x, ghA.x, rgA.x, oA.y)
        const double v1 = v;
        if (RERUN) st_d2(q, vin, v1);
        FWD_ONE(akA.y, GA.y, stA.y, ghA.y, rgA.y, oB.x)
        const double v2 = v;
        p += BS;
        akA = ldg_d2(p); GA = ldg_d2(p + PS); stA = ldg_d2(p + 2 * PS); ghA = ldg_d2(p + 3 * PS); rgA = ldg_d2(p + 4 * PS);
        if (RERUN) oA = *reinterpret_cast<const double2*>(q + PS);
        FWD_ONE(akB.x, GB.x, stB.x, ghB.x, rgB.x, oB.y)
        if (RERUN) st_d2(q + 2, v2, v);
        if (SWEEP) { st_d2(q, vin, v1); st_d2(q + 2, v2, v); }
        FWD_ONE(akB.y, GB.y, stB.y, ghB.y, rgB.y, ((e + 1 < hi) ? oA.x : old_end))
        q += PS;
    }
    if (e < hi) {
        if (!DRY) q[0] = v;
        const int rem = hi - e;
        {
            const double old = RERUN ? ((rem > 1) ? oA.y : old_end) : 0.0;
            FWD_ONE(akA.x, GA.x, stA.x, ghA.x, rgA.x, old)
            if (!DRY && e < hi) q[1] = v;
        }
        if (e < hi) {
            const double old = RERUN ? ((rem > 2) ? q[2] : old_end) : 0.0;
            FWD_ONE(akA.y, GA.y, stA.y, ghA.y, rgA.y, old)
            if (!DRY && e < hi) q[2] = v;
        }
        if (e < hi) {
            const double a2 = __ldg(p + 2), g2 = __ldg(p + PS + 2), s2 = __ldg(p + 2 * PS + 2), h2 = __ldg(p + 3 * PS + 2),
                         r2 = __ldg(p + 4 * PS + 2);
            FWD_ONE(a2, g2, s2, h2, r2, old_end)
        }
    }
#undef FWD_ONE
    if (!DRY && tail) *tail = v;
    return false;
}

#define TMA_PLANE_DOUBLES (PB * 32)
struct WarpRing {
    double* stage;
    unsigned bar;
    int planes;
    unsigned bytes;
#ifdef VAP_BOUNDS_CHECK
    const double *rec_lo, *rec_hi, *x_lo, *x_hi;
    unsigned smem_lo, smem_hi, bar_hi;
#endif
};
template <int NT>
__device__ __forceinline__ void ring_issue(const WarpRing& R, int s, const double* rec_row0, const double* x_row0,
                                           const double* sb_row0, int rb)
{
    constexpr int PS = PB * NT, BS = 5 * PS;
    const unsigned bar = R.bar + 8 * s;
    const unsigned dst = (unsigned)__cvta_generic_to_shared(R.stage + (size_t)s * R.planes * TMA_PLANE_DOUBLES);
    fence_proxy_async();
    mbar_expect_tx(bar, R.bytes * R.planes);
    const double* src = rec_row0 + (size_t)rb * BS;
    if (NT == 32 && !sb_row0) {
#ifdef VAP_BOUNDS_CHECK
        VAP_CHECK(1, rb >= 0 && src >= R.rec_lo && src + 5 * R.bytes / 8 <= R.rec_hi && (reinterpret_cast<uintptr_t>(src) & 15) == 0);
        VAP_CHECK(2, dst >= R.smem_lo && dst + 5 * R.bytes <= R.smem_hi && bar >= R.smem_hi && bar + 8 <= R.bar_hi);
#endif
        bulk_g2s(dst, src, 5 * R.bytes, bar);
    } else
#pragma unroll
    for (int f = 0; f < 5; f++) {
        const double* g = (f == 2 && sb_row0) ? sb_row0 + (size_t)rb * PS : src + f * PS;
#ifdef VAP_BOUNDS_CHECK
        if (f == 2 && sb_row0) VAP_CHECK(0, rb >= 0 && (reinterpret_cast<uintptr_t>(g) & 15) == 0);
        else VAP_CHECK(1, rb >= 0 && g >= R.rec_lo && g + R.bytes / 8 <= R.rec_hi && (reinterpret_cast<uintptr_t>(g) & 15) == 0);
        VAP_CHECK(2, dst + f * TMA_PLANE_DOUBLES * 8 >= R.smem_lo && dst + f * TMA_PLANE_DOUBLES * 8 + R.bytes <= R.smem_hi && bar >= R.smem_hi && bar + 8 <= R.bar_hi);
#endif
        bulk_g2s(dst + f * TMA_PLANE_DOUBLES * 8, g, R.bytes, bar);
    }
    if (x_row0) {
#ifdef VAP_BOUNDS_CHECK
        VAP_CHECK(3, x_row0 + (size_t)rb * PS >= R.x_lo && x_row0 + (size_t)rb * PS + R.bytes / 8 <= R.x_hi);
        VAP_CHECK(2, dst + 5 * TMA_PLANE_DOUBLES * 8 + R.bytes <= R.smem_hi);
#endif
        bulk_g2s(dst + 5 * TMA_PLANE_DOUBLES * 8, x_row0 + (size_t)rb * PS, R.bytes, bar);
    }
}

template <int NT>
__device__ __forceinline__ void fwd_sweep_tma(const WarpRing& R, const double* __restrict__ rec_w, int lc, double* __restrict__ q,
                                              double* __restrict__ tail, int lo, int len, const FwdTables& T, double hw,
                                              double dd, double& v, double& sq)
{
    constexpr int PS = PB * NT;
    constexpr int PD = TMA_PLANE_DOUBLES;
    const int lane = threadIdx.x & 31;
    const int nbw = __reduce_max_sync(0xffffffffu, (len + PB - 1) >> 2);
    if (lane == 0) {
        if (nbw > 0) ring_issue<NT>(R, 0, rec_w, nullptr, nullptr, 0);
        if (nbw > 1) ring_issue<NT>(R, 1, rec_w, nullptr, nullptr, 1);
    }
    int j = 0;
    while (j + 1 < T.n_b && T.bi[j + 1] <= lo) j++;
    double acc = T.acc[j];
    int nb_next = (j + 1 < T.n_b) ? T.bi[j + 1] : CH_INT_MAX;
    int jv = 0;
    while (jv + 1 < T.n_v && T.vi[jv + 1] <= lo + 1) jv++;
    double v0n = T.vv[jv];
    int nv_next = (jv + 1 < T.n_v) ? T.vi[jv + 1] : CH_INT_MAX;
    int e = lo;
    const int hi = lo + len;
    const int nfull = len >> 2;
#define FWD_T(ROW_)                                                                                                  \
        {                                                                                                            \
            const double ak_ = S[ROW_], G_ = S[PD + ROW_], st_ = S[2 * PD + ROW_], gh_ = S[3 * PD + ROW_],             \
                         rg_ = S[4 * PD + ROW_];                                                                     \
            if (e == nb_next) { j++; acc = T.acc[j]; nb_next = (j + 1 < T.n_b) ? T.bi[j + 1] : CH_INT_MAX; }          \
            if (e + 1 == nv_next) { jv++; v0n = T.vv[jv]; nv_next = (jv + 1 < T.n_v) ? T.vi[jv + 1] : CH_INT_MAX; }  \
            v = fwd_step(ak_, gh_, rg_, st_, pymin(v0n, G_), v, sq, acc, hw, dd);                                    \
            ++e;                                                                                                     \
        }
    for (int blk = 0; blk < nbw; ++blk) {
        const int s = blk & 1;
        mbar_wait(R.bar + 8 * s, (blk >> 1) & 1);
        const double* S = R.stage + (size_t)s * 5 * PD + lc * PB;
        VAP_CHECK(6, lc >= 0 && lc < 32 && (unsigned)__cvta_generic_to_shared(S + 4 * PD + 3) + 8 <= R.smem_hi);
        if (blk < nfull) {
            const double vin = v;
            FWD_T(0)
            const double v1 = v;
            FWD_T(1)
            const double v2 = v;
            FWD_T(2)
            st_d2(q, vin, v1); st_d2(q + 2, v2, v);
            FWD_T(3)
            q += PS;
        } else if (e < hi) {
            q[0] = v;
            FWD_T(0)
            if (e < hi) { q[1] = v; FWD_T(1) }
            if (e < hi) { q[2] = v; FWD_T(2) }
        }
        __syncwarp();
        if (lane == 0 && blk + 2 < nbw) ring_issue<NT>(R, s, rec_w, nullptr, nullptr, blk + 2);
    }
#undef FWD_T
    if (tail && len > 0) *tail = v;
}

template <int NT>
__device__ __noinline__ bool fwd_rerun(const double* p, double* q, double* tail, double old_end, int lo, int len, FwdTables T,
                                       double hw, double dd, double* st, bool prev_same)
{
    double v = st[0], sq = st[1];
    const bool merged = fwd_run<NT, RUN_RERUN>(p, q, tail, old_end, lo, len, T, hw, dd, v, sq, prev_same);
    st[0] = v; st[1] = sq;
    return merged;
}
template <int NT>
__device__ __noinline__ void fwd_dry(const double* p, int lo, int len, FwdTables T, double hw, double dd, double* st)
{
    double v = st[0], sq = st[1];
    fwd_run<NT, RUN_DRY>(p, nullptr, nullptr, 0.0, lo, len, T, hw, dd, v, sq, false);
    st[0] = v; st[1] = sq;
}

template <int NT, bool TMA>
__global__ void __maxnreg__(TMA ? VAP_PASS_REGS_TMA : VAP_PASS_REGS) k_fwd_chunked(
    const int* __restrict__ status, const double* __restrict__ cons, double dd, double start_vel, double end_vel,
    long long RS, const int* __restrict__ n_samples, const double* __restrict__ rec, int E_cap,
    const double* __restrict__ max_accels, const int* __restrict__ bidx, const int* __restrict__ bval,
    const int* __restrict__ n_ev, const int* __restrict__ vr_idx, const double* __restrict__ vr_val,
    const int* __restrict__ st_idx, const int* __restrict__ n_vr, double* __restrict__ vfT, int* __restrict__ rounds_out,
    int warm, int max_rounds, int ring_off)
{
    extern __shared__ __align__(128) unsigned char s_mem[];
    const int c = threadIdx.x;
    const long long b = blockIdx.x;
    const int VC = 3 * E_cap + 2;
    double* s_endv = reinterpret_cast<double*>(s_mem);
    double* s_endw = s_endv + NT;
    double* s_usev = s_endw + NT;
    double* s_usew = s_usev + NT;
    double* s_acc = s_usew + NT;
    double* s_vv = s_acc + E_cap;
    int* s_bi = reinterpret_cast<int*>(s_vv + VC);
    int* s_vi = s_bi + E_cap;
    __shared__ int s_nv;
    if (status[b] != ST_OK) return;
    const int D = n_samples[b];
    const int steps = D - 1;
    double* vf = vfT + (size_t)b * RS;
    if (c == 0) { vf[0] = start_vel; vf[RS - 1] = start_vel; if (rounds_out) rounds_out[2 * b] = 0; }
    if (steps <= 0) return;
    const int n_b = n_ev[2 * b + 1];
    for (int k = c; k < n_b; k += NT) {
        s_bi[k] = bidx[(size_t)b * E_cap + k];
        s_acc[k] = max_accels[(size_t)b * E_cap + bval[(size_t)b * E_cap + k]];
    }
    if (c == 0) {
        const int* vi = vr_idx + (size_t)b * E_cap;
        const double* vv = vr_val + (size_t)b * E_cap;
        const int* si = st_idx + (size_t)b * E_cap;
        const int nvr = n_vr[2 * b], nst = n_vr[2 * b + 1];
        int pv = 0, ps = 0, pa = 0, n = 0, reg = 0;
        while (true) {
            int x = CH_INT_MAX;
            if (pv < nvr) x = vi[pv];
            if (ps < nst && si[ps] < x) x = si[ps];
            if (pa < nst && si[pa] + 1 < x) x = si[pa] + 1;
            if (x >= D - 1) break;
            bool stop = false;
            while (pv < nvr && vi[pv] == x) { reg = pv; pv++; }
            while (ps < nst && si[ps] == x) { stop = true; ps++; }
            while (pa < nst && si[pa] + 1 == x) pa++;
            s_vi[n] = x; s_vv[n] = stop ? 0.01 : vv[reg]; n++;
        }
        s_vi[n] = D - 1; s_vv[n] = end_vel; n++;
        s_nv = n;
    }
    const int Lc = chunk_len(steps, NT);
    const int nch = (steps + Lc - 1) / Lc;
    const bool active = c < nch;
    const int lo = c * Lc;
    const int len = (lo + Lc < steps) ? Lc : steps - lo;
    const double* P = rec + (size_t)b * RS * 5;
    double* tail = (active && lo + len == steps) ? vf + (RS - 1) : nullptr;
    const double hw = cons[b * 6 + 5] * 0.5;
    WarpRing R;
    if (TMA) {
        constexpr int WARPS = (NT + 31) / 32;
        const int w = c >> 5;
        R.stage = reinterpret_cast<double*>(s_mem + ring_off) + (size_t)w * 2 * 5 * TMA_PLANE_DOUBLES;
        R.bar = (unsigned)__cvta_generic_to_shared(s_mem + ring_off + (size_t)WARPS * 2 * 5 * TMA_PLANE_DOUBLES * 8 + 16 * w);
        R.planes = 5;
        R.bytes = (NT < 32 ? NT : 32) * PB * 8;
#ifdef VAP_BOUNDS_CHECK
        R.rec_lo = P; R.rec_hi = P + 5 * RS; R.x_lo = R.x_hi = nullptr;
        R.smem_lo = (unsigned)__cvta_generic_to_shared(s_mem + ring_off);
        R.smem_hi = R.smem_lo + WARPS * 2 * 5 * TMA_PLANE_DOUBLES * 8;
        R.bar_hi = R.smem_hi + 16 * WARPS;
#endif
        if ((c & 31) == 0) { mbar_init(R.bar, 1); mbar_init(R.bar + 8, 1); fence_mbar_init(); }
    }
    __syncthreads();
    FwdTables T;
    T.bi = s_bi; T.acc = s_acc; T.n_b = n_b; T.vi = s_vi; T.vv = s_vv; T.n_v = s_nv;

    {
        double v = start_vel, sq = 0.0;
        if (active) {
            if (c > 0) {
                auto v0_at = [&](int x) { int q = 0; while (q + 1 < T.n_v && T.vi[q + 1] <= x) q++; return T.vv[q]; };
                auto term = [&](int x, int fld) { const int cx = x / Lc, rx = x - cx * Lc; return __ldg(P + rec_index(rx, fld, cx, NT)); };
                int wl = warm < Lc ? warm : Lc;
                if (wl > lo - 2) wl = lo - 2 > 0 ? lo - 2 : 0;
                wl &= ~(PB - 1);
                const int s0 = lo - wl;
                const double vm1 = (s0 >= 2) ? pymin(v0_at(s0 - 1), term(s0 - 2, 1)) : start_vel;
                v = pymin(v0_at(s0), term(s0 - 1, 1));
                const double wp = vm1 * term(s0 - 1, 0);
                sq = wp * wp;
                if (wl > 0) {
                    double st[2] = {v, sq};
                    fwd_dry<NT>(P + rec_index(Lc - wl, 0, c - 1, NT), s0, wl, T, hw, dd, st);
                    v = st[0]; sq = st[1];
                }
            }
            s_usev[c] = v; s_usew[c] = sq;
            VAP_CHECK(4, c * PB + PB <= PB * NT && (size_t)(((len + 3) >> 2) + 1) * 5 * PB * NT <= (size_t)(5 * RS - 3) &&
                             (size_t)(((len + 3) >> 2) + 1) * PB * NT <= (size_t)(RS - 1) && lo + len <= steps);
            if (!TMA) fwd_run<NT, RUN_SWEEP>(P + c * PB, vf + c * PB, tail, 0.0, lo, len, T, hw, dd, v, sq, false);
        }
        if (TMA) fwd_sweep_tma<NT>(R, P + (c & ~31) * PB, c & 31, vf + c * PB, tail, lo, active ? len : 0, T, hw, dd, v, sq);
        s_endv[c] = v; s_endw[c] = sq;
    }
    __syncthreads();

    int rounds = 0;
    for (int round = 1; round < NT && round <= max_rounds; round++) {
        bool need = false;
        double in_v = 0.0, in_w = 0.0;
        if (active && c >= round) {
            in_v = s_endv[c - 1]; in_w = s_endw[c - 1];
            need = !(same_bits(in_v, s_usev[c]) && same_bits(in_w, s_usew[c]));
        }
        if (!__syncthreads_or(need)) break;
        rounds = round;
        if (need) {
            double st[2] = {in_v, in_w};
            const bool merged = fwd_rerun<NT>(P + c * PB, vf + c * PB, tail, s_endv[c], lo, len, T, hw, dd, st,
                                              same_bits(in_v, s_usev[c]));
            s_usev[c] = in_v; s_usew[c] = in_w;
            if (!merged) { s_endv[c] = st[0]; s_endw[c] = st[1]; }
        }
        __syncthreads();
    }
    if (c == 0 && rounds_out) rounds_out[2 * b] = rounds;
}

template <int NT, int MODE, bool OVR>
__device__ __forceinline__ bool bwd_run(const double* __restrict__ p, const double* __restrict__ f, double* __restrict__ o,
                                        const double* __restrict__ sb, int lo, int len, double top_ak, double top_G,
                                        double top_st, const int* s_bi, const double* s_acc, int n_b, double acc0, double hw,
                                        double dd, double& v, double& sq, bool prev_same, float& est, float dd_over_dt,
                                        double old_top = 0.0)
{
    constexpr int PS = PB * NT, BS = 5 * PS;
    constexpr bool RERUN = (MODE == RUN_RERUN);
    constexpr bool DRY = (MODE == RUN_DRY);
    constexpr bool SWEEP = (MODE == RUN_SWEEP);
    int e = lo + len - 1;
    int j = n_b - 1;
    double acc = acc0;
    while (j >= 0 && s_bi[j] > e + 1) { acc = s_acc[j]; j--; }
    int nb_next = (j >= 0) ? s_bi[j] : -1;
#define BWD_ONE(AK_, G_, ST_, GH_, RG_, F_, OLD_, OLDUP_)                                                            \
        if (e + 1 == nb_next) { acc = s_acc[j]; j--; nb_next = (j >= 0) ? s_bi[j] : -1; }                             \
        {                                                                                                            \
            const double vup = v;                                                                                    \
            v = bwd_step(AK_, GH_, RG_, ST_, pymin(F_, G_), v, sq, acc, hw, dd);                                     \
            if (!DRY) est += t_est_term(vup, v, dd_over_dt);                                                         \
            if (RERUN) est -= t_est_term(OLDUP_, OLD_, dd_over_dt);                                                  \
        }                                                                                                            \
        if (RERUN) {                                                                                                 \
            const bool same = same_bits(OLD_, v);                                                                    \
            if (same && prev_same) return true;                                                                      \
            prev_same = same;                                                                                        \
        }                                                                                                            \
        --e;
    int blk = len >> 2;
    p += (size_t)blk * BS; f += (size_t)blk * PS; sb += (size_t)blk * PS; if (!DRY) o += blk * PB;
    double tak = top_ak, tG = top_G, tst = top_st;
    double oup = old_top;
    for (int r = (len & 3) - 1; r >= 0; --r) {
        const double gh = __ldg(p + 3 * PS + r), rg = __ldg(p + 4 * PS + r), fv = __ldg(f + r);
        const double old = RERUN ? o[r] : 0.0;
        BWD_ONE(tak, tG, tst, gh, rg, fv, old, oup)
        if (!DRY) o[r] = v;
        oup = old;
        tak = __ldg(p + r); tG = __ldg(p + PS + r); tst = OVR ? __ldg(sb + r) : __ldg(p + 2 * PS + r);
    }
    if (blk == 0) return false;
    p -= BS; f -= PS; sb -= PS; if (!DRY) o -= PB;
    if (RERUN) {
#pragma unroll
        for (int k = 1; k < RERUN_PF; k++)
            if (k < blk) {
#pragma unroll
                for (int fl = 0; fl < 5; fl++) if (!(OVR && fl == 2)) l2_prefetch(p - (size_t)k * BS + fl * PS);
                l2_prefetch(f - (size_t)k * PS);
                l2_prefetch(o - k * PB);
                if (OVR) l2_prefetch(sb - (size_t)k * PS);
            }
    }
    double2 akB = ldg_d2(p + 2), GB = ldg_d2(p + PS + 2), stB = OVR ? ldg_d2(sb + 2) : ldg_d2(p + 2 * PS + 2),
            ghB = ldg_d2(p + 3 * PS + 2), rgB = ldg_d2(p + 4 * PS + 2), fB = ldg_d2(f + 2);
    double2 akA, GA, stA, ghA, rgA, fA;
    double2 oA = make_double2(0.0, 0.0), oB = oA;
    if (RERUN) oB = *reinterpret_cast<const double2*>(o + 2);
    while (true) {
        if (RERUN && blk > RERUN_PF) {
#pragma unroll
            for (int fl = 0; fl < 5; fl++) if (!(OVR && fl == 2)) l2_prefetch(p - (size_t)RERUN_PF * BS + fl * PS);
            l2_prefetch(f - (size_t)RERUN_PF * PS);
            l2_prefetch(o - RERUN_PF * PB);
            if (OVR) l2_prefetch(sb - (size_t)RERUN_PF * PS);
        }
        akA = ldg_d2(p); GA = ldg_d2(p + PS); stA = OVR ? ldg_d2(sb) : ldg_d2(p + 2 * PS); ghA = ldg_d2(p + 3 * PS); rgA = ldg_d2(p + 4 * PS);
        fA = ldg_d2(f);
        if (RERUN) oA = *reinterpret_cast<const double2*>(o);
        BWD_ONE(tak, tG, tst, ghB.y, rgB.y, fB.y, oB.y, oup)
        const double v3 = v;
        BWD_ONE(akB.y, GB.y, stB.y, ghB.x, rgB.x, fB.x, oB.x, oB.y)
        const double v2 = v;
        if (RERUN) st_d2(o + 2, v2, v3);
        const double a2 = akB.x, g2 = GB.x, s2 = stB.x;
        const double ob0 = oB.x;
        const bool more = --blk > 0;
        if (more) {
            akB = ldg_d2(p - BS + 2); GB = ldg_d2(p - BS + PS + 2); stB = OVR ? ldg_d2(sb - PS + 2) : ldg_d2(p - BS + 2 * PS + 2);
            ghB = ldg_d2(p - BS + 3 * PS + 2); rgB = ldg_d2(p - BS + 4 * PS + 2); fB = ldg_d2(f - PS + 2);
            if (RERUN) oB = *reinterpret_cast<const double2*>(o - PB + 2);
        }
        BWD_ONE(a2, g2, s2, ghA.y, rgA.y, fA.y, oA.y, ob0)
        const double v1 = v;
        BWD_ONE(akA.y, GA.y, stA.y, ghA.x, rgA.x, fA.x, oA.x, oA.y)
        if (RERUN) st_d2(o, v, v1);
        if (SWEEP) { st_d2(o, v, v1); st_d2(o + 2, v2, v3); }
        if (!more) break;
        oup = oA.x;
        tak = akA.x; tG = GA.x; tst = stA.x;
        p -= BS; f -= PS; sb -= PS; if (!DRY) o -= PB;
    }
#undef BWD_ONE
    return false;
}

template <int NT>
__device__ __forceinline__ void bwd_sweep_tma(const WarpRing& R, const double* __restrict__ rec_w, const double* __restrict__ vf_w,
                                              const double* __restrict__ sb_w, int lc, double* __restrict__ o, int lo, int len,
                                              double top_ak, double top_G, double top_st, const int* s_bi, const double* s_acc,
                                              int n_b, double acc0, double hw, double dd, double& v, double& sq, float& est,
                                              float dd_over_dt)
{
    constexpr int PD = TMA_PLANE_DOUBLES;
    const int lane = threadIdx.x & 31;
    const int nbl = (len + PB - 1) >> 2;
    const int nbw = __reduce_max_sync(0xffffffffu, nbl);
    if (lane == 0) {
        if (nbw > 0) ring_issue<NT>(R, 0, rec_w, vf_w, sb_w, nbw - 1);
        if (nbw > 1) ring_issue<NT>(R, 1, rec_w, vf_w, sb_w, nbw - 2);
    }
    int e = lo + len - 1;
    int j = n_b - 1;
    double acc = acc0;
    while (j >= 0 && s_bi[j] > e + 1) { acc = s_acc[j]; j--; }
    int nb_next = (j >= 0) ? s_bi[j] : -1;
    double tak = top_ak, tG = top_G, tst = top_st;
#define BWD_T(ROW_)                                                                                                  \
        {                                                                                                            \
            const double gh_ = S[3 * PD + ROW_], rg_ = S[4 * PD + ROW_], f_ = S[5 * PD + ROW_];                       \
            if (e + 1 == nb_next) { acc = s_acc[j]; j--; nb_next = (j >= 0) ? s_bi[j] : -1; }                         \
            const double vup = v;                                                                                    \
            v = bwd_step(tak, gh_, rg_, tst, pymin(f_, tG), v, sq, acc, hw, dd);                                     \
            est += t_est_term(vup, v, dd_over_dt);                                                                   \
            tak = S[ROW_]; tG = S[PD + ROW_]; tst = S[2 * PD + ROW_];                                                \
            --e;                                                                                                     \
        }
    const int nfull = len >> 2, rem = len & 3;
    o += nfull * PB;
    for (int it = 0; it < nbw; ++it) {
        const int rb = nbw - 1 - it;
        const int s = it & 1;
        mbar_wait(R.bar + 8 * s, (it >> 1) & 1);
        const double* S = R.stage + (size_t)s * 6 * PD + lc * PB;
        VAP_CHECK(7, lc >= 0 && lc < 32 && (unsigned)__cvta_generic_to_shared(S + 5 * PD + 3) + 8 <= R.smem_hi);
        if (rb < nfull) {
            o -= PB;
            BWD_T(3)
            const double v3 = v;
            BWD_T(2)
            const double v2 = v;
            BWD_T(1)
            const double v1 = v;
            BWD_T(0)
            st_d2(o, v, v1); st_d2(o + 2, v2, v3);
        } else if (rb == nfull && rem > 0) {
            if (rem > 2) { BWD_T(2) o[2] = v; }
            if (rem > 1) { BWD_T(1) o[1] = v; }
            BWD_T(0) o[0] = v;
        }
        __syncwarp();
        if (lane == 0 && it + 2 < nbw) ring_issue<NT>(R, s, rec_w, vf_w, sb_w, nbw - 3 - it);
    }
#undef BWD_T
}

struct BwdArgs {
    const double* p; const double* f; double* o; const double* sb; int lo, len; double top_ak, top_G, top_st;
    const int* s_bi; const double* s_acc; int n_b; double acc0, hw, dd; float dd_over_dt;
};
template <int NT, bool OVR>
__device__ __noinline__ bool bwd_rerun(const BwdArgs a, double* st, float* est, bool prev_same, double old_top)
{
    double v = st[0], sq = st[1];
    float e = *est;
    const bool merged = bwd_run<NT, RUN_RERUN, OVR>(a.p, a.f, a.o, a.sb, a.lo, a.len, a.top_ak, a.top_G, a.top_st, a.s_bi, a.s_acc,
                                                    a.n_b, a.acc0, a.hw, a.dd, v, sq, prev_same, e, a.dd_over_dt, old_top);
    st[0] = v; st[1] = sq; *est = e;
    return merged;
}
template <int NT, bool OVR>
__device__ __noinline__ void bwd_dry(const BwdArgs a, double* st)
{
    double v = st[0], sq = st[1];
    float e = 0.f;
    bwd_run<NT, RUN_DRY, OVR>(a.p, a.f, nullptr, a.sb, a.lo, a.len, a.top_ak, a.top_G, a.top_st, a.s_bi, a.s_acc, a.n_b, a.acc0,
                              a.hw, a.dd, v, sq, false, e, a.dd_over_dt);
    st[0] = v; st[1] = sq;
}

template <int NT, bool TMA>
__global__ void __maxnreg__(TMA ? VAP_PASS_REGS_TMA : VAP_PASS_REGS) k_bwd_chunked(
    const int* __restrict__ status, const double* __restrict__ cons, double dd, double dt, double end_vel,
    long long RS, long long D_cap, const int* __restrict__ n_samples, const double* __restrict__ rec, int E_cap,
    const double* __restrict__ max_accels, const int* __restrict__ bidx, const int* __restrict__ bval,
    const int* __restrict__ n_ev, const double* __restrict__ vfT, double* __restrict__ vel, float* __restrict__ t_est,
    int* __restrict__ rounds_out, int warm, int max_rounds, const double* __restrict__ statB, int ring_off)
{
    extern __shared__ __align__(128) unsigned char s_mem[];
    const int k = threadIdx.x;
    const long long b = blockIdx.x;
    double* s_endv = reinterpret_cast<double*>(s_mem);
    double* s_endw = s_endv + NT;
    double* s_usev = s_endw + NT;
    double* s_usew = s_usev + NT;
    double* s_acc = s_usew + NT;
    int* s_bi = reinterpret_cast<int*>(s_acc + E_cap);
    if (k == 0 && t_est) t_est[b] = 0.f;
    if (status[b] != ST_OK) return;
    const int D = n_samples[b];
    const int steps = D - 1;
    double* vo = vel + (size_t)b * D_cap;
    if (k == 0) { vo[D - 1] = end_vel; if (rounds_out) rounds_out[2 * b + 1] = 0; }
    if (steps <= 0) return;
    const int n_b = n_ev[2 * b + 1];
    for (int q = k; q < n_b; q += NT) {
        s_bi[q] = bidx[(size_t)b * E_cap + q];
        s_acc[q] = max_accels[(size_t)b * E_cap + bval[(size_t)b * E_cap + q] + 1];
    }
    const double acc0 = max_accels[(size_t)b * E_cap + bval[(size_t)b * E_cap + n_b - 1]];
    const int Lc = chunk_len(steps, NT);
    const int nch = (steps + Lc - 1) / Lc;
    const bool active = k < nch;
    const int col = active ? nch - 1 - k : 0;
    const int lo = col * Lc;
    const int len = (lo + Lc < steps) ? Lc : steps - lo;
    const double* P = rec + (size_t)b * RS * 5;
    const double* vf = vfT + (size_t)b * RS;
    const double hw = cons[b * 6 + 5] * 0.5;
    const bool ovr = pass_has_override(max_accels + (size_t)b * E_cap, n_ev[2 * b], cons[b * 6 + 1]) != 0;
    const double* SB = statB + (size_t)b * RS;
    WarpRing R;
    if (TMA) {
        constexpr int WARPS = (NT + 31) / 32;
        const int w = k >> 5;
        R.stage = reinterpret_cast<double*>(s_mem + ring_off) + (size_t)w * 2 * 6 * TMA_PLANE_DOUBLES;
        R.bar = (unsigned)__cvta_generic_to_shared(s_mem + ring_off + (size_t)WARPS * 2 * 6 * TMA_PLANE_DOUBLES * 8 + 16 * w);
        R.planes = 6;
        R.bytes = (NT < 32 ? NT : 32) * PB * 8;
#ifdef VAP_BOUNDS_CHECK
        R.rec_lo = P; R.rec_hi = P + 5 * RS; R.x_lo = vf; R.x_hi = vf + RS;
        R.smem_lo = (unsigned)__cvta_generic_to_shared(s_mem + ring_off);
        R.smem_hi = R.smem_lo + WARPS * 2 * 6 * TMA_PLANE_DOUBLES * 8;
        R.bar_hi = R.smem_hi + 16 * WARPS;
#endif
        if ((k & 31) == 0) { mbar_init(R.bar, 1); mbar_init(R.bar + 8, 1); fence_mbar_init(); }
    }
    __syncthreads();

    auto rec_of = [&](int x, int fld) {
        if (fld == 2 && ovr) return __ldg(SB + (x >= steps ? (int)(RS - 1) : edge_slot(x, Lc, NT)));
        if (x >= steps) return __ldg(P + 5 * RS - 3 + fld);
        const int cx = x / Lc, rx = x - cx * Lc;
        return __ldg(P + rec_index(rx, fld, cx, NT));
    };
    auto vf_at = [&](int x) { return vf[x >= steps ? (int)(RS - 1) : edge_slot(x, Lc, NT)]; };
    double top_ak = 0.0, top_G = 0.0, top_st = 0.0;
    if (active) { top_ak = rec_of(lo + len, 0); top_G = rec_of(lo + len, 1); top_st = rec_of(lo + len, 2); }
    BwdArgs A;
    A.p = P + col * PB; A.f = vf + col * PB; A.o = vo + lo; A.sb = SB + col * PB; A.lo = lo; A.len = len;
    A.top_ak = top_ak; A.top_G = top_G; A.top_st = top_st; A.s_bi = s_bi; A.s_acc = s_acc; A.n_b = n_b; A.acc0 = acc0;
    A.hw = hw; A.dd = dd; A.dd_over_dt = (float)dd / (float)dt;
    float est = 0.f;

    {
        double v = end_vel, sq = 0.0;
        if (active) {
            if (k > 0) {
                const int hi = lo + len;
                const int len_up = (hi + Lc < steps) ? Lc : steps - hi;
                int wl = warm < len_up ? warm : len_up;
                if (hi + wl + 2 > D - 1) wl = (D - 1) - hi - 2 > 0 ? (D - 1) - hi - 2 : 0;
                wl &= ~(PB - 1);
                const int s0 = hi + wl;
                v = pymin(vf_at(s0), rec_of(s0 + 1, 1));
                double vp1 = end_vel;
                if (s0 + 2 <= D - 1) vp1 = pymin(vf_at(s0 + 1), rec_of(s0 + 2, 1));
                const double wp = vp1 * rec_of(s0 + 1, 0);
                sq = wp * wp;
                if (wl > 0) {
                    BwdArgs W = A;
                    W.p = P + (col + 1) * PB; W.f = vf + (col + 1) * PB; W.o = nullptr; W.sb = SB + (col + 1) * PB;
                    W.lo = hi; W.len = wl; W.top_ak = rec_of(s0, 0); W.top_G = rec_of(s0, 1); W.top_st = rec_of(s0, 2);
                    double st[2] = {v, sq};
                    if (ovr) bwd_dry<NT, true>(W, st); else bwd_dry<NT, false>(W, st);
                    v = st[0]; sq = st[1];
                }
            }
            s_usev[k] = v; s_usew[k] = sq;
            VAP_CHECK(5, col >= 0 && col * PB + PB <= PB * NT && (size_t)(((len + 3) >> 2) + 1) * 5 * PB * NT <= (size_t)(5 * RS - 3) &&
                             (size_t)(((len + 3) >> 2) + 1) * PB * NT <= (size_t)(RS - 1) && A.o + len <= vo + D - 1 &&
                             lo + len <= steps && D <= D_cap);
            if (!TMA) {
                if (ovr) bwd_run<NT, RUN_SWEEP, true>(A.p, A.f, A.o, A.sb, lo, len, top_ak, top_G, top_st, s_bi, s_acc, n_b, acc0, hw,
                                                      dd, v, sq, false, est, A.dd_over_dt);
                else bwd_run<NT, RUN_SWEEP, false>(A.p, A.f, A.o, A.sb, lo, len, top_ak, top_G, top_st, s_bi, s_acc, n_b, acc0, hw,
                                                   dd, v, sq, false, est, A.dd_over_dt);
            }
        }
        if (TMA) {
            const int col_hi = nch - 1 - (k & ~31);
            const int cs = col_hi > 31 ? col_hi - 31 : 0;
            bwd_sweep_tma<NT>(R, P + cs * PB, vf + cs * PB, ovr ? SB + cs * PB : nullptr, active ? col - cs : 0, vo + lo, lo,
                              active ? len : 0, top_ak, top_G, top_st, s_bi, s_acc, n_b, acc0, hw, dd, v, sq, est, A.dd_over_dt);
        }
        s_endv[k] = v; s_endw[k] = sq;
    }
    __syncthreads();

    int rounds = 0;
    for (int round = 1; round < NT && round <= max_rounds; round++) {
        bool need = false;
        double in_v = 0.0, in_w = 0.0;
        if (active && k >= round) {
            in_v = s_endv[k - 1]; in_w = s_endw[k - 1];
            need = !(same_bits(in_v, s_usev[k]) && same_bits(in_w, s_usew[k]));
        }
        if (!__syncthreads_or(need)) break;
        rounds = round;
        if (need) {
            double st[2] = {in_v, in_w};
            const bool ps = same_bits(in_v, s_usev[k]);
            const bool merged = ovr ? bwd_rerun<NT, true>(A, st, &est, ps, s_usev[k]) : bwd_rerun<NT, false>(A, st, &est, ps, s_usev[k]);
            s_usev[k] = in_v; s_usew[k] = in_w;
            if (!merged) { s_endv[k] = st[0]; s_endw[k] = st[1]; }
        }
        __syncthreads();
    }
    if (k == 0 && rounds_out) rounds_out[2 * b + 1] = rounds;

    __syncthreads();
    float* s_f = reinterpret_cast<float*>(s_endv);
    s_f[k] = active ? est : 0.f;
    __syncthreads();
    if (k == 0 && t_est) {
        float tot = 0.f;
        for (int q = 0; q < NT; q++) tot += s_f[q];
        t_est[b] = tot;
    }
}

__global__ void __launch_bounds__(256) k_untranspose(const int* __restrict__ status, const int* __restrict__ n_samples,
                                                     long long D_cap, long long RS, int NT,
                                                     const double* __restrict__ vT, double* __restrict__ vel,
                                                     unsigned tiles_x)
{
    const PathTile pt = path_tile(tiles_x);
    const long long b = pt.b;
    if (status[b] != ST_OK) return;
    const int D = n_samples[b];
    const int steps = D - 1;
    const int e = pt.x * blockDim.x + threadIdx.x;
    if (e >= D) return;
    const double* src = vT + (size_t)b * RS;
    const int Lc = steps > 0 ? chunk_len(steps, NT) : 1;
    vel[(size_t)b * D_cap + e] = (e < steps) ? src[edge_slot(e, Lc, NT)] : src[RS - 1];
}
```

vexautonomousplanner_b200/engine.py:

```python
from __future__ import annotations

import ctypes as C
import os
from contextlib import contextmanager
from dataclasses import dataclass, field
from typing import Dict, Optional

import numpy as np
import torch

from . import _lib
from .packing import PackedPaths

OUT_NAMES = ("times", "positions", "linear_vels", "accelerations", "headings", "angular_vels", "x", "y")
ST_OK, ST_FALSE, ST_INDEX, ST_VALUE, ST_CAPACITY, ST_DIVERGED, ST_EVENTS = 0, -1, -2, -3, -4, -5, -6
ROW_LIMIT = 1.0e7
DIST_LIMIT = 5.0e7
_POISON = bool(int(os.environ.get("VAP_POISON", "0")))
MAX_RETRIES = 2


def _p(t: Optional[torch.Tensor]):
    return C.c_void_p(0 if t is None else t.data_ptr())

# ... 128 lines not shown
        yield
        e.record()
        self.stage_events.append((name, s, e))

    def _stream(self):
        return C.c_void_p(torch.cuda.current_stream(self.device).cuda_stream)

    def _empty(self, shape, dtype=torch.float64):
        t = torch.empty(shape, dtype=dtype, device=self.device)
        if _POISON:
            t.fill_(float("nan") if dtype.is_floating_point else (1 if dtype == torch.uint8 else 0x5a5a5a5))
        return t

    def upload(self, p: PackedPaths) -> DeviceBatch:
        return DeviceBatch.from_packed(p, self.device)

    def dgrid(self, n: int) -> torch.Tensor:
        if self._dgrid is None or self._dgrid.numel() < n:
            m = max(int(n * 1.5), 1 << 14)
            g = self._empty((m,))
            _lib.check(self.lib.vap_build_dgrid(C.c_int64(m), C.c_double(self.dd), _p(g), self._stream()), "vap_build_dgrid")
            self.launches += 1
            if self._dgrid is not None:
                self._retired.append(self._dgrid)
            self._dgrid = g
        return self._dgrid

    def lerp_recip(self, n: int) -> torch.Tensor:
        if self._rden is None or self._rden.numel() < n:
            m = max(int(n * 1.5), 1 << 14)
            r = self._empty((m,))
            _lib.check(self.lib.vap_build_lerp_recip(C.c_int64(m), C.c_double(self.dd), _p(r), self._stream()), "vap_build_lerp_recip")
            self.launches += 1
            if self._rden is not None:
                self._retired.append(self._rden)
            self._rden = r
        return self._rden

    def build_geometry(self, db: DeviceBatch, with_params: bool = False) -> Geometry:
        B, N = db.B, db.N_max
        g = Geometry(self._empty((B, max(N - 1, 1), 6, 2)), self._empty((B, N + 1), torch.int32), self._empty((B, N)),
                     self._empty((B, N)), self._empty((B,), torch.int32), self._empty((B,), torch.int32))
        scratch = self._empty((B, N, 9))
        if with_params:
            g.params = torch.zeros((B, 2 * N), dtype=torch.float64, device=self.device)
            g.derivs = torch.zeros((B, 2 * N, 4), dtype=torch.float64, device=self.device)
        _lib.check(self.lib.vap_build_path(C.c_int64(B), C.c_int(N), _p(db.node_attr), _p(db.node_flags), _p(db.n_nodes),
                                           _p(g.seg), _p(g.first_node), _p(g.param_end), _p(g.seglen), _p(g.n_splines),
                                           _p(g.status), _p(scratch), _p(g.params), _p(g.derivs), self._stream()),
                   "vap_build_path")
        self.launches += 1
        return g

    def build_lut(self, db: DeviceBatch, g: Geometry, samples: Optional[int] = None) -> Tables:
        samples = samples or self.samples
        B = db.B
        Q_cap = samples * max(db.max_splines, 1)
        t = Tables(samples, self.spn, Q_cap, 0, self._empty((B, Q_cap)), self._empty((B, Q_cap)), self._empty((B,)))
        _lib.check(self.lib.vap_build_lut(C.c_int64(B), C.c_int(db.N_max), _p(g.seg), _p(g.first_node), _p(g.param_end),
                                          _p(g.n_splines), _p(g.status), C.c_int(samples), C.c_int64(Q_cap), _p(t.lut_d),
                                          _p(t.lut_t), _p(t.total_len), self._stream()), "vap_build_lut")
        self.launches += 1
        t.lut_inv = self._empty((B, int(self.lib.vap_lut_index_row_ints(C.c_int64(Q_cap)))), torch.int32)
        _lib.check(self.lib.vap_build_lut_index(C.c_int64(B), _p(g.n_splines), _p(g.status), C.c_int(samples), C.c_int64(Q_cap),
                                                _p(t.lut_d), _p(t.total_len), _p(t.lut_inv), self._stream()), "vap_build_lut_index")
        self.launches += 1
        return t

    def build_props(self, db: DeviceBatch, g: Geometry, t: Tables, spn: Optional[int] = None) -> Tables:
        spn = spn or self.spn
        B = db.B
        t.spn = spn
        t.P_cap = spn * db.N_max
        t.prop_k = self._empty((B, t.P_cap))
        t.prop_h = self._empty((B, t.P_cap))
        _lib.check(self.lib.vap_build_props(C.c_int64(B), C.c_int(db.N_max), _p(db.n_nodes), _p(g.seg), _p(g.first_node),
                                            _p(g.param_end), _p(g.n_splines), _p(g.status), C.c_int(spn), C.c_int64(t.P_cap),
                                            _p(t.prop_k), _p(t.prop_h), self._stream()), "vap_build_props")
        self.launches += 1
        return t

    def gl_queries(self, g: Geometry, path, spl, a, b, mode: int = 0, num_points: int = 20, max_iter: int = 50):
        path = torch.as_tensor(path, dtype=torch.int32).to(self.device)
        spl = torch.as_tensor(spl, dtype=torch.int32).to(self.device)
        a = torch.as_tensor(a, dtype=torch.float64).to(self.device)
        b = torch.as_tensor(b, dtype=torch.float64).to(self.device).expand_as(a).contiguous()
        n = int(a.numel())
        pts, wts = np.polynomial.legendre.leggauss(num_points)
        dp, dw = torch.from_numpy(pts).to(self.device), torch.from_numpy(wts).to(self.device)
        out = self._empty((n,)); qst = self._empty((n,), torch.int32)
        N_max = g.param_end.shape[1]
        _lib.check(self.lib.vap_gl(C.c_int64(n), _p(path), _p(spl), _p(a), _p(b), C.c_int(mode), C.c_int(max_iter),
                                   C.c_int(num_points), _p(dp), _p(dw), C.c_int(N_max), _p(g.seg), _p(g.first_node),
                                   _p(g.param_end), _p(out), _p(qst), self._stream()), "vap_gl")
        self.launches += 1
        torch.cuda.current_stream(self.device).synchronize()
        return out, qst

    def dist_sample(self, db: DeviceBatch, g: Geometry, t: Tables, status: torch.Tensor, D_cap: int):
        B = db.B
        grid = self.dgrid(D_cap + 2)
        n_samples = self._empty((B,), torch.int32)
        tq, kap, th = self._empty((B, D_cap)), self._empty((B, D_cap)), self._empty((B, D_cap))
        _lib.check(self.lib.vap_dist_sample(C.c_int64(B), _p(db.n_nodes), _p(g.n_splines), _p(status), C.c_int64(grid.numel()),
                                            _p(grid), C.c_int(t.samples), C.c_int64(t.Q_cap), _p(t.lut_d), _p(t.lut_t),
                                            _p(t.total_len), C.c_int(t.spn), C.c_int64(t.P_cap), _p(t.prop_k), _p(t.prop_h),
                                            C.c_int64(D_cap), _p(n_samples), _p(tq), _p(kap), _p(th), self._stream()),
                   "vap_dist_sample")
        self.launches += 2
        return n_samples, tq, kap, th

    def fwd_bwd(self, db: DeviceBatch, status, D_cap, n_samples, tq, kap, th, mode: int = 0):
        B = db.B
        E_cap = db.N_max + db.A_max + 2
        vel = self._empty((B, D_cap))
        ma = self._empty((B, E_cap))
        bidx = self._empty((B, E_cap), torch.int32)
        bval = self._empty((B, E_cap), torch.int32)
        n_ev = self._empty((B, 2), torch.int32)
        t_est = self._empty((B,))
        _lib.check(self.lib.vap_fwd_bwd(C.c_int64(B), C.c_int(db.N_max), C.c_int(db.A_max), _p(db.node_attr),
                                        _p(db.node_flags), _p(db.n_nodes), _p(db.ap_attr), _p(db.ap_flags), _p(db.n_ap),
                                        _p(db.cons), _p(status), C.c_double(self.dd), C.c_double(self.dt),
                                        C.c_double(self.start_vel), C.c_double(self.end_vel), C.c_int64(D_cap),
                                        _p(n_samples), _p(tq), _p(kap), _p(th), _p(vel), C.c_int(E_cap), _p(ma), _p(bidx),
                                        _p(bval), _p(n_ev), _p(t_est), C.c_int(mode), self._stream()), "vap_fwd_bwd")
        self.launches += 1
        return vel, ma, bidx, bval, n_ev, t_est

    def velocity_chunked(self, db: DeviceBatch, g: Geometry, t: Tables, status: torch.Tensor, D_cap: int, mode: int = 0,
                         outs: Optional[dict] = None, want_t: bool = True, fused: Optional[bool] = None):
        B = db.B
        fused = self.fused_velocity if fused is None else fused
        E_cap = db.N_max + db.A_max + 2
        grid = self.dgrid(D_cap + 2)
        n_samples = outs["n_samples"] if outs else self._empty((B,), torch.int32)
        need_kth = want_t or not fused
        tq = self._empty((B, D_cap)) if need_kth else None
        kap = self._empty((B, D_cap)) if need_kth else None
        th = self._empty((B, D_cap)) if need_kth else None
        ma = self._empty((B, E_cap)); bidx = self._empty((B, E_cap), torch.int32); bval = self._empty((B, E_cap), torch.int32)
        n_ev = self._empty((B, 2), torch.int32)
        vr_idx = self._empty((B, E_cap), torch.int32); vr_val = self._empty((B, E_cap))
        st_idx = self._empty((B, E_cap), torch.int32); n_vr = self._empty((B, 2), torch.int32)
        ins_est = self._empty((B,), torch.float32)
        nscr = int(self.lib.vap_event_scratch_ints(C.c_int64(B), C.c_int(db.N_max), C.c_int(db.A_max)))
        scr = self._empty((nscr,), torch.int32)
        chunks = self.chunks if D_cap <= 65536 else 256
        RS = int(self.lib.vap_pass_row_slots(C.c_int64(D_cap), C.c_int(chunks)))
        rec = self._empty((B, RS, 5)); statB = self._empty((B, RS))
        vel_f = self._empty((B, RS)); vel = outs["vel"] if outs else self._empty((B, D_cap))
        t_est = self._empty((B,), torch.float32)
        rounds = torch.zeros((B, 2), dtype=torch.int32, device=self.device)
        inv = t.lut_inv if self.accelerators else None
        if fused:
            with self._stage("S345_velocity"):
                _lib.check(self.lib.vap_velocity_profile(
                    C.c_int64(B), C.c_int(db.N_max), C.c_int(db.A_max), _p(db.node_attr), _p(db.node_flags), _p(db.n_nodes),
                    _p(db.ap_attr), _p(db.ap_flags), _p(db.n_ap), _p(db.cons), _p(g.n_splines), _p(status),
                    C.c_int64(grid.numel()), _p(grid), C.c_int(t.samples), C.c_int64(t.Q_cap), _p(t.lut_d), _p(t.lut_t),
                    _p(t.total_len), C.c_int(t.spn), C.c_int64(t.P_cap), _p(t.prop_k), _p(t.prop_h), _p(inv),
                    C.c_double(self.dd), C.c_double(self.dt), C.c_double(self.start_vel), C.c_double(self.end_vel),
                    C.c_int64(D_cap), _p(n_samples), _p(tq), _p(kap), _p(th), C.c_int(E_cap), _p(ma), _p(bidx), _p(bval),
                    _p(n_ev), _p(vr_idx), _p(vr_val), _p(st_idx), _p(n_vr), _p(ins_est), _p(scr), _p(rec), _p(statB),
                    _p(vel_f), _p(vel), _p(t_est), _p(rounds), C.c_int(chunks), C.c_int(mode), self._stream()),
                    "vap_velocity_profile")
                self.launches += 6 if mode == 0 else 6
        else:
            with self._stage("S3_dist_sample"):
                _lib.check(self.lib.vap_dist_sample_events(
                    C.c_int64(B), C.c_int(db.N_max), C.c_int(db.A_max), _p(db.node_attr), _p(db.node_flags), _p(db.n_nodes),
                    _p(db.ap_attr), _p(db.ap_flags), _p(db.n_ap), _p(db.cons), _p(g.n_splines), _p(status),
                    C.c_int64(grid.numel()), _p(grid), C.c_int(t.samples), C.c_int64(t.Q_cap), _p(t.lut_d), _p(t.lut_t),
                    _p(t.total_len), C.c_int(t.spn), C.c_int64(t.P_cap), _p(t.prop_k), _p(t.prop_h), C.c_int64(D_cap),
                    _p(n_samples), _p(tq), _p(kap), _p(th), C.c_int(E_cap), _p(ma), _p(bidx), _p(bval), _p(n_ev), _p(vr_idx),
                    _p(vr_val), _p(st_idx), _p(n_vr), C.c_double(self.dt), _p(ins_est), _p(scr), _p(inv), self._stream()),
                    "vap_dist_sample_events")
                self.launches += 3
            with self._stage("S45_fwd_bwd"):
                _lib.check(self.lib.vap_fwd_bwd_chunked(
                    C.c_int64(B), _p(db.cons), _p(status), C.c_double(self.dd), C.c_double(self.dt), C.c_double(self.start_vel),
                    C.c_double(self.end_vel), C.c_int64(D_cap), _p(n_samples), _p(kap), _p(th), C.c_int(E_cap), _p(ma),
                    _p(bidx), _p(bval), _p(n_ev), _p(vr_idx), _p(vr_val), _p(st_idx), _p(n_vr), _p(rec), _p(statB),
                    _p(vel_f), _p(vel), _p(t_est), _p(rounds), C.c_int(chunks), C.c_int(mode), self._stream()), "vap_fwd_bwd_chunked")
                self.launches += 3
        extra = dict(t=tq, kap=kap, th=th, max_accels=ma, bidx=bidx, bval=bval, n_ev=n_ev, vel_f=vel_f, rounds=rounds,
                     vr_idx=vr_idx, vr_val=vr_val, st_idx=st_idx, n_vr=n_vr)
        return n_samples, vel, t_est + ins_est, extra

    def velocity_serial(self, db: DeviceBatch, g: Geometry, t: Tables, status: torch.Tensor, D_cap: int, mode: int = 0):
        with self._stage("S3_dist_sample"):
            n_samples, tq, kap, th = self.dist_sample(db, g, t, status, D_cap)
        with self._stage("S45_fwd_bwd"):
            vel, ma, bidx, bval, n_ev, t_est = self.fwd_bwd(db, status, D_cap, n_samples, tq, kap, th, mode)
        extra = dict(t=tq, kap=kap, th=th, max_accels=ma, bidx=bidx, bval=bval, n_ev=n_ev)
        return n_samples, vel, t_est, extra

    def resample(self, db: DeviceBatch, g: Geometry, t: Tables, status, D_cap, n_samples, vel, T_cap):
        B = db.B
        out = self._empty((8, B, T_cap))
        nodes_map = self._empty((B, db.N_max + 1), torch.int32)
        actions_map = self._empty((B, max(db.A_max, 1)), torch.int32)
        n_maps = self._empty((B, 2), torch.int32)
        n_out = self._empty((B,), torch.int32)
        summary = self._empty((B, 5))
        _lib.check(self.lib.vap_resample(C.c_int64(B), C.c_int(db.N_max), C.c_int(db.A_max), _p(db.node_attr),
                                         _p(db.node_flags), _p(db.n_nodes), _p(db.ap_attr), _p(db.ap_flags), _p(db.n_ap),
                                         _p(db.cons), _p(status), C.c_double(self.dt), C.c_double(self.dd), _p(g.seg),
                                         _p(g.first_node), _p(g.param_end), _p(g.n_splines), C.c_int(t.samples),
                                         C.c_int64(t.Q_cap), _p(t.lut_d), _p(t.lut_t), _p(t.total_len), C.c_int(t.spn),
                                         C.c_int64(t.P_cap), _p(t.prop_k), _p(t.prop_h), C.c_int64(D_cap), _p(n_samples),
                                         _p(vel), C.c_int64(T_cap), _p(out), _p(nodes_map), _p(actions_map), _p(n_maps),
                                         _p(n_out), _p(summary), self._stream()), "vap_resample")
        self.launches += 1
        return out, nodes_map, actions_map, n_maps, n_out, summary

    def _insert_bound(self, db: DeviceBatch, status: Optional[torch.Tensor] = None) -> int:
        na = db.node_attr
        waits = (na[:, :, 3] / self.dt).floor().clamp(min=0).sum(dim=1) + (db.ap_attr[:, :, 1] / self.dt).floor().clamp(min=0).sum(dim=1)
        V, A, w = db.cons[:, 0:1], db.cons[:, 1:2], db.cons[:, 5:6]
        arc = (na[:, :, 2].abs() * (3.141592653589793 / 180.0)) * w / 2
        turn_rows = torch.where(na[:, :, 2] != 0, ((2 * V / A + arc / V) / self.dt).ceil() + 3, torch.zeros_like(arc)).sum(dim=1)
        rows = torch.nan_to_num(waits + turn_rows, nan=0.0, posinf=0.0)
        if status is not None:
            rows = torch.where(status == ST_OK, rows, torch.zeros_like(rows))
        return int(rows.max().item()) if rows.numel() else 0

    def time_profile(self, db: DeviceBatch, g: Geometry, t: Tables, status, D_cap, n_samples, vel, T_cap,
                     outs: Optional[dict] = None):
        B = db.B
        E_cap = db.N_max + db.A_max + 2
        plane_stride = 0
        if outs:
            out, nodes_map, actions_map = outs["out"], outs["nodes_map"], outs["actions_map"]
            n_maps, n_out, summary, n_main = outs["n_maps"], outs["n_out"], outs["summary"], outs["n_main"]
            plane_stride = outs["plane_stride"]
        else:
            out = self._empty((8, B, T_cap))
            nodes_map = self._empty((B, db.N_max + 1), torch.int32)
            actions_map = self._empty((B, max(db.A_max, 1)), torch.int32)
            n_maps = self._empty((B, 2), torch.int32)
            n_out = self._empty((B,), torch.int32)
            summary = self._empty((B, 5))
            n_main = self._empty((B,), torch.int32)
        rden = self.lerp_recip(D_cap + 2)
        stage = self._empty((8, B, T_cap + 1))
        seg_tab = self._empty((3 * B * E_cap + B,), torch.int32)
        nscr = int(self.lib.vap_event_scratch_ints(C.c_int64(B), C.c_int(db.N_max), C.c_int(db.A_max)))
        scr = self._empty((nscr,), torch.int32)
        _lib.check(self.lib.vap_time_profile(
            C.c_int64(B), C.c_int(db.N_max), C.c_int(db.A_max), _p(db.node_attr), _p(db.node_flags), _p(db.n_nodes),
            _p(db.ap_attr), _p(db.ap_flags), _p(db.n_ap), _p(db.cons), _p(status), C.c_double(self.dt), C.c_double(self.dd),
            _p(g.seg), _p(g.first_node), _p(g.param_end), _p(g.n_splines), C.c_int(t.samples), C.c_int64(t.Q_cap),
            _p(t.lut_d), _p(t.lut_t), _p(t.total_len), C.c_int(t.spn), C.c_int64(t.P_cap), _p(t.prop_k), _p(t.prop_h),
            C.c_int64(D_cap), _p(n_samples), _p(vel), C.c_int64(T_cap), _p(out), _p(nodes_map), _p(actions_map), _p(n_maps),
            _p(n_out), _p(summary), _p(n_main), _p(stage), C.c_int(E_cap), _p(seg_tab), _p(scr), C.c_int64(plane_stride),
            _p(t.lut_inv if self.accelerators else None), _p(rden if self.accelerators else None), C.c_int64(rden.numel()),
            self._stream()), "vap_time_profile")
        self.launches += 5
        self._n_main = n_main
        return out, nodes_map, actions_map, n_maps, n_out, summary

    def _profile_tiled(self, db: DeviceBatch, D_cap: int, T_cap: int, tiles: int, host: "Optional[HostResult]" = None,
                       dense: Optional[torch.Tensor] = None, events: Optional[list] = None,
                       stagger: bool = True) -> ProfileResult:
        B = db.B
        main = torch.cuda.current_stream(self.device)
        out = self._empty((8, B, T_cap))
        whole = dict(nodes_map=self._empty((B, db.N_max + 1), torch.int32),
                     actions_map=self._empty((B, max(db.A_max, 1)), torch.int32), n_maps=self._empty((B, 2), torch.int32),
                     n_out=self._empty((B,), torch.int32), summary=self._empty((B, 5)), n_main=self._empty((B,), torch.int32),
                     n_samples=self._empty((B,), torch.int32), vel=self._empty((B, D_cap)),
                     status=self._empty((B,), torch.int32), status_pre=self._empty((B,), torch.int32))
        self.dgrid(D_cap + 2)
        self.lerp_recip(D_cap + 2)
        while len(self._streams) < tiles:
            k = len(self._streams)
            self._streams.append(torch.cuda.Stream(device=self.device, priority=max(-5, -(5 - min(k, 5)))))
        bounds = [(B * k // tiles, B * (k + 1) // tiles) for k in range(tiles)]
        sampled = None
        for k, (lo, hi) in enumerate(bounds):
            if hi <= lo:
                continue
            s = self._streams[k]
            s.wait_stream(main)
            if sampled is not None and stagger:
                s.wait_event(sampled)
            sampled = torch.cuda.Event()
            with torch.cuda.stream(s):
                sub = DeviceBatch(db.node_attr[lo:hi], db.node_flags[lo:hi], db.n_nodes[lo:hi], db.ap_attr[lo:hi],
                                  db.ap_flags[lo:hi], db.n_ap[lo:hi], db.cons[lo:hi], db.max_splines)
                outs = {key: val[lo:hi] for key, val in whole.items()}
                outs["out"] = out[:, lo:hi]
                outs["plane_stride"] = B * T_cap
                g = self.build_geometry(sub)
                t = self.build_lut(sub, g)
                self.build_props(sub, g, t)
                outs["status"].copy_(g.status)
                n_samples, vel, _, _ = self.velocity_chunked(sub, g, t, outs["status"], D_cap, outs=outs, want_t=False)
                sampled.record(s)
                outs["status_pre"].copy_(outs["status"])
                self.time_profile(sub, g, t, outs["status"], D_cap, n_samples, vel, T_cap, outs=outs)
                if host is not None:
                    offs = host.dev_offsets[lo + k: hi + k + 1]
                    base = host.packed if dense is None else dense
                    dst = C.c_void_p(base.data_ptr() + 8 * 8 * lo * T_cap)
                    _lib.check(self.lib.vap_pack_rows(C.c_int64(hi - lo), C.c_int64(T_cap), C.c_int64(B * T_cap),
                                                      _p(outs["out"]), _p(outs["n_out"]), _p(outs["status"]), _p(offs), dst,
                                                      self._stream()), "vap_pack_rows")
                    self.launches += 2
                    host.offsets[lo + k: hi + k + 1].copy_(offs, non_blocking=True)
                    for name in ("n_out", "status", "nodes_map", "actions_map", "n_maps", "summary"):
                        getattr(host, name)[lo:hi].copy_(outs[name], non_blocking=True)
                    if events is not None:
                        events[k].record(s)
        for k in range(tiles):
            main.wait_stream(self._streams[k])
        self._n_main = whole["n_main"]
        res = ProfileResult(B, T_cap, out, whole["n_out"], whole["nodes_map"], whole["actions_map"], whole["n_maps"],
                            whole["status"], whole["summary"], whole["vel"], whole["n_samples"])
        res.extra = dict(status_pre=whole["status_pre"])
        return res

    def profile_many(self, packed: PackedPaths, tile_paths: int = 16384, sink=None) -> torch.Tensor:
        B = packed.B
        rows = []
        for lo in range(0, B, tile_paths):
            hi = min(B, lo + tile_paths)
            res = self.profile(self.upload(packed.slice(lo, hi)), reuse_plan=True)
            if sink is not None:
                sink(lo, hi, res)
            rows.append(res.summary)
        return torch.cat(rows, dim=0) if rows else self._empty((0, 5))

    def _host_state(self, packed: PackedPaths, tiles: int, state: Optional[dict]) -> dict:
        B = packed.B
        key = (B, packed.N_max, packed.A_max, packed.max_splines())
# ... 344 lines not shown
```

Measured before the change: 1.216 million.

## Fuse forward and backward passes into persistent kernel with length-sorted work queue

Replaces separate per-path forward and backward chunked-pass kernel launches with a single persistent kernel sized to the device's occupancy. Paths are pulled from a queue ordered longest-first by a new single-block histogram/counting-sort kernel over sample counts. Each CTA runs the forward sweep, fences async proxy, then runs the backward sweep for the same path. The goal is fewer launches and less tail imbalance. The cost is an extra ordering kernel, a global atomic for work distribution, the TMA toggle being dropped, and larger shared memory per block.

```diff
diff --git a/include/vap.h b/include/vap.h
--- a/include/vap.h
+++ b/include/vap.h
@@ -84,7 +84,7 @@
                         int E_cap, const double* max_accels, const int32_t* bidx, const int32_t* bval,
                         const int32_t* n_ev, const int32_t* vr_idx, const double* vr_val, const int32_t* st_idx,
                         const int32_t* n_vr, double* rec, double* statB, double* vel_f, double* vel, float* t_est,
-                        int32_t* rounds, int chunks, int mode, void* stream);
+                        int32_t* rounds, int32_t* pass_queue, int chunks, int mode, void* stream);
 
 int vap_velocity_profile(int64_t B, int N_max, int A_max, const double* node_attr, const int32_t* node_flags,
                          const int32_t* n_nodes, const double* ap_attr, const int32_t* ap_flags, const int32_t* n_ap,
@@ -95,7 +95,8 @@
                          int32_t* n_samples, double* t, double* kap, double* th, int E_cap, double* max_accels,
                          int32_t* bidx, int32_t* bval, int32_t* n_ev, int32_t* vr_idx, double* vr_val, int32_t* st_idx,
                          int32_t* n_vr, float* ins_est, int32_t* ev_scratch, double* rec, double* statB, double* vel_f,
-                         double* vel, float* t_est, int32_t* rounds, int chunks, int mode, void* stream);
+                         double* vel, float* t_est, int32_t* rounds, int32_t* pass_queue, int chunks, int mode,
+                         void* stream);
 
 int vap_resample(int64_t B, int N_max, int A_max, const double* node_attr, const int32_t* node_flags,
                  const int32_t* n_nodes, const double* ap_attr, const int32_t* ap_flags, const int32_t* n_ap,
diff --git a/vexautonomousplanner_b200/csrc/vap_device.cuh b/vexautonomousplanner_b200/csrc/vap_device.cuh
--- a/vexautonomousplanner_b200/csrc/vap_device.cuh
+++ b/vexautonomousplanner_b200/csrc/vap_device.cuh
@@ -57,6 +57,7 @@
 
 __device__ __forceinline__ void fence_mbar_init() { asm volatile("fence.mbarrier_init.release.cluster;" ::: "memory"); }
 __device__ __forceinline__ void fence_proxy_async() { asm volatile("fence.proxy.async.shared::cta;" ::: "memory"); }
+__device__ __forceinline__ void fence_proxy_async_global() { asm volatile("fence.proxy.async.global;" ::: "memory"); }
 
 #ifdef VAP_BOUNDS_CHECK
 #define VAP_DIAG_SITES 32
diff --git a/vexautonomousplanner_b200/csrc/vap_kernels.cu b/vexautonomousplanner_b200/csrc/vap_kernels.cu
--- a/vexautonomousplanner_b200/csrc/vap_kernels.cu
+++ b/vexautonomousplanner_b200/csrc/vap_kernels.cu
@@ -1175,79 +1175,103 @@
 
 extern "C" int64_t vap_pass_row_slots(int64_t D_cap, int chunks) { return ((D_cap + 8 * (int64_t)chunks + 64 + 1) / 2) * 2; }
 
-template <int NT, bool TMA>
-static int launch_passes_v(int64_t B, size_t ss, cudaStream_t st, const double* cons, const int32_t* status, double dd, double dt,
-                           double start_vel, double end_vel, long long RS, long long D_cap, const int32_t* n_samples,
-                           const double* rec, int E_cap, const double* max_accels, const int32_t* bidx, const int32_t* bval,
-                           const int32_t* n_ev, const int32_t* vr_idx, const double* vr_val, const int32_t* st_idx,
-                           const int32_t* n_vr, double* vel_f, double* vel, float* t_est, int32_t* rounds, bool backward,
-                           int warm, int max_rounds, const double* statB)
+#define PASS_ORDER_BINS 1024
+__global__ void __launch_bounds__(PASS_ORDER_BINS) k_pass_order(long long B, const int* __restrict__ status,
+                                                                const int* __restrict__ n_samples, long long D_cap,
+                                                                int* __restrict__ order, int* __restrict__ next_path)
+{
+    __shared__ int s_h[PASS_ORDER_BINS];
+    __shared__ int s_w[PASS_ORDER_BINS / 32];
+    const int t = threadIdx.x;
+    auto cls = [&](long long b) {
+        const long long D = status[b] == ST_OK ? n_samples[b] : 0;
+        long long x = D * PASS_ORDER_BINS / (D_cap + 1);
+        x = x < 0 ? 0 : (x >= PASS_ORDER_BINS ? PASS_ORDER_BINS - 1 : x);
+        return PASS_ORDER_BINS - 1 - (int)x;
+    };
+    s_h[t] = 0;
+    __syncthreads();
+    for (long long b = t; b < B; b += PASS_ORDER_BINS) atomicAdd(&s_h[cls(b)], 1);
+    __syncthreads();
+    const int x = s_h[t];
+    int incl = x;
+    for (int o = 1; o < 32; o <<= 1) { const int y = __shfl_up_sync(0xffffffffu, incl, o); if ((t & 31) >= o) incl += y; }
+    if ((t & 31) == 31) s_w[t >> 5] = incl;
+    __syncthreads();
+    if (t < 32) {
+        int w = s_w[t];
+        for (int o = 1; o < 32; o <<= 1) { const int y = __shfl_up_sync(0xffffffffu, w, o); if (t >= o) w += y; }
+        s_w[t] = w;
+    }
+    __syncthreads();
+    s_h[t] = (t >= 32 ? s_w[(t >> 5) - 1] : 0) + incl - x;
+    __syncthreads();
+    for (long long b = t; b < B; b += PASS_ORDER_BINS) order[atomicAdd(&s_h[cls(b)], 1)] = (int)b;
+    if (t == 0) *next_path = 0;
+}
+
+template <int NT>
+static int launch_passes(int64_t B, size_t ss, cudaStream_t st, const int32_t* queue, int32_t* next_path, bool backward,
+                         const double* cons, const int32_t* status, double dd, double dt, double start_vel, double end_vel,
+                         long long RS, long long D_cap, const int32_t* n_samples, const double* rec, const double* statB,
+                         int E_cap, const double* max_accels, const int32_t* bidx, const int32_t* bval, const int32_t* n_ev,
+                         const int32_t* vr_idx, const double* vr_val, const int32_t* st_idx, const int32_t* n_vr, double* vel_f,
+                         double* vel, float* t_est, int32_t* rounds, int warm, int max_rounds)
 {
     const int warps = (NT + 31) / 32;
     const int ring_off = (int)((ss + 127) / 128 * 128);
-    const int planes = backward ? 6 : 5;
-    const size_t smem = TMA ? (size_t)ring_off + (size_t)warps * (2 * planes * TMA_PLANE_DOUBLES * 8 + 16) : ss;
+    const size_t smem = (size_t)ring_off + (size_t)warps * (2 * 6 * TMA_PLANE_DOUBLES * 8 + 16);
     cudaError_t e = cudaSuccess;
-    if (!backward) {
-        if (smem > 48 * 1024) e = cudaFuncSetAttribute(k_fwd_chunked<NT, TMA>, cudaFuncAttributeMaxDynamicSharedMemorySize, (int)smem);
-        if (e != cudaSuccess) return set_err("vap_fwd_bwd_chunked/attr", e);
-        k_fwd_chunked<NT, TMA><<<(unsigned)B, NT, smem, st>>>(status, cons, dd, start_vel, end_vel, RS, n_samples, rec, E_cap,
-                                                             max_accels, bidx, bval, n_ev, vr_idx, vr_val, st_idx, n_vr, vel_f,
-                                                             rounds, warm, max_rounds, ring_off);
-    } else {
-        if (smem > 48 * 1024) e = cudaFuncSetAttribute(k_bwd_chunked<NT, TMA>, cudaFuncAttributeMaxDynamicSharedMemorySize, (int)smem);
-        if (e != cudaSuccess) return set_err("vap_fwd_bwd_chunked/attr", e);
-        k_bwd_chunked<NT, TMA><<<(unsigned)B, NT, smem, st>>>(status, cons, dd, dt, end_vel, RS, D_cap, n_samples, rec, E_cap,
-                                                             max_accels, bidx, bval, n_ev, vel_f, vel, t_est, rounds, warm,
-                                                             max_rounds, statB, ring_off);
-    }
-    return 0;
-}
-template <int NT, typename... Args>
-static int launch_passes(bool tma, Args... args)
-{
-    return tma ? launch_passes_v<NT, true>(args...) : launch_passes_v<NT, false>(args...);
+    if (smem > 48 * 1024) e = cudaFuncSetAttribute(k_passes_chunked<NT>, cudaFuncAttributeMaxDynamicSharedMemorySize, (int)smem);
+    if (e != cudaSuccess) return set_err("vap_fwd_bwd_chunked/attr", e);
+    int dev = 0, sms = 0, per_sm = 0;
+    if ((e = cudaGetDevice(&dev)) != cudaSuccess) return set_err("vap_fwd_bwd_chunked/device", e);
+    if ((e = cudaDeviceGetAttribute(&sms, cudaDevAttrMultiProcessorCount, dev)) != cudaSuccess) return set_err("vap_fwd_bwd_chunked/sms", e);
+    if ((e = cudaOccupancyMaxActiveBlocksPerMultiprocessor(&per_sm, k_passes_chunked<NT>, NT, smem)) != cudaSuccess)
+        return set_err("vap_fwd_bwd_chunked/occupancy", e);
+    if (per_sm < 1) return arg_err("vap_fwd_bwd_chunked: the pass kernel does not fit on an SM (E_cap too large)");
+    const long long grid = (long long)sms * per_sm < B ? (long long)sms * per_sm : B;
+    k_passes_chunked<NT><<<(unsigned)grid, NT, smem, st>>>(B, queue, next_path, backward, status, cons, dd, dt, start_vel, end_vel, RS,
+                                                         D_cap, n_samples, rec, statB, E_cap, max_accels, bidx, bval, n_ev, vr_idx,
+                                                         vr_val, st_idx, n_vr, vel_f, vel, t_est, rounds, warm, max_rounds, ring_off);
+    return 0;
 }
 
 static int run_passes(int64_t B, const double* cons, const int32_t* status, double dd, double dt, double start_vel,
                       double end_vel, int64_t D_cap, const int32_t* n_samples, int E_cap, const double* max_accels,
                       const int32_t* bidx, const int32_t* bval, const int32_t* n_ev, const int32_t* vr_idx,
                       const double* vr_val, const int32_t* st_idx, const int32_t* n_vr, const double* rec,
-                      const double* statB, double* vel_f, double* vel, float* t_est, int32_t* rounds, int chunks, int mode,
-                      cudaStream_t stream)
+                      const double* statB, double* vel_f, double* vel, float* t_est, int32_t* rounds, int32_t* queue,
+                      int chunks, int mode, cudaStream_t stream)
 {
     const long long RS = vap_pass_row_slots(D_cap, chunks);
     const size_t VC = 3 * (size_t)E_cap + 2;
-    const size_t ss = ((size_t)chunks * 4 + E_cap + VC) * sizeof(double) + (E_cap + VC) * sizeof(int);
+    const size_t ss = ((size_t)chunks * 4 + 2 * (size_t)E_cap + VC) * sizeof(double) + (E_cap + VC) * sizeof(int);
     int warm = 0, max_rounds = 1 << 30;
     if (const char* ev = getenv("VAP_CHUNK_WARM")) warm = atoi(ev);
 #ifdef VAP_DIAG_MAXROUNDS
     if (const char* ev = getenv("VAP_CHUNK_MAXROUNDS")) max_rounds = atoi(ev);
 #endif
     if (warm < 0) warm = 0;
-    bool tma = true;
-    if (const char* ev = getenv("VAP_PASS_TMA")) tma = atoi(ev) != 0;
-    auto passes = [&](bool backward) -> int {
-        switch (chunks) {
-#define VAP_PASS_CASE(N_) case N_: return launch_passes<N_>(tma, B, ss, STREAM, cons, status, dd, dt, start_vel, end_vel, RS, D_cap,   \
-                                              n_samples, rec, E_cap, max_accels, bidx, bval, n_ev, vr_idx, vr_val, st_idx, n_vr,  \
-                                              vel_f, vel, t_est, rounds, backward, warm, max_rounds, statB);
-            VAP_PASS_CASE(8) VAP_PASS_CASE(16) VAP_PASS_CASE(32) VAP_PASS_CASE(64) VAP_PASS_CASE(128) VAP_PASS_CASE(256)
+    k_pass_order<<<1, PASS_ORDER_BINS, 0, STREAM>>>(B, status, n_samples, D_cap, queue, queue + B);
+    CHECK_LAUNCH("vap_fwd_bwd_chunked/order");
+    int rc = 0;
+    switch (chunks) {
+#define VAP_PASS_CASE(N_) case N_: rc = launch_passes<N_>(B, ss, STREAM, queue, queue + B, mode != 1, cons, status, dd, dt, start_vel, \
+                                                      end_vel, RS, D_cap, n_samples, rec, statB, E_cap, max_accels, bidx, bval, \
+                                                      n_ev, vr_idx, vr_val, st_idx, n_vr, vel_f, vel, t_est, rounds, warm,       \
+                                                      max_rounds); break;
+        VAP_PASS_CASE(8) VAP_PASS_CASE(16) VAP_PASS_CASE(32) VAP_PASS_CASE(64) VAP_PASS_CASE(128) VAP_PASS_CASE(256)
 #undef VAP_PASS_CASE
-        }
-        return 0;
-    };
-    if (int rc = passes(false)) return rc;
-    CHECK_LAUNCH("vap_fwd_bwd_chunked/fwd");
+    }
+    if (rc) return rc;
+    CHECK_LAUNCH("vap_fwd_bwd_chunked/passes");
     if (mode == 1) {
         const unsigned tx2 = blocks_for(D_cap, 256);
         if ((long long)tx2 * B > 2147483647LL) return arg_err("vap_fwd_bwd_chunked: more than 2^31 CTAs (tile the batch)");
         k_untranspose<<<tx2 * (unsigned)B, 256, 0, STREAM>>>(status, n_samples, D_cap, RS, chunks, vel_f, vel, tx2);
         CHECK_LAUNCH("vap_fwd_bwd_chunked/untranspose");
-        return 0;
-    }
-    if (int rc = passes(true)) return rc;
-    CHECK_LAUNCH("vap_fwd_bwd_chunked/bwd");
+    }
     return 0;
 }
 
@@ -1266,10 +1290,11 @@
                                    const int32_t* bidx, const int32_t* bval, const int32_t* n_ev, const int32_t* vr_idx,
                                    const double* vr_val, const int32_t* st_idx, const int32_t* n_vr, double* rec,
                                    double* statB, double* vel_f, double* vel, float* t_est, int32_t* rounds,
-                                   int chunks, int mode, void* stream)
+                                   int32_t* pass_queue, int chunks, int mode, void* stream)
 {
     if (B <= 0) return 0;
     if (check_pass_args("vap_fwd_bwd_chunked", B, D_cap, chunks)) return -1;
+    if (!pass_queue) return arg_err("vap_fwd_bwd_chunked: pass_queue is NULL");
     const long long RS = vap_pass_row_slots(D_cap, chunks);
     const unsigned tx = blocks_for(D_cap + 4 * chunks, 256 * PP_TILES);
     if ((long long)tx * B > 2147483647LL) return arg_err("vap_fwd_bwd_chunked: more than 2^31 CTAs (tile the batch)");
@@ -1279,7 +1304,7 @@
                                          bval, n_ev, statB, tx);
     CHECK_LAUNCH("vap_fwd_bwd_chunked/prepass");
     return run_passes(B, cons, status, dd, dt, start_vel, end_vel, D_cap, n_samples, E_cap, max_accels, bidx, bval, n_ev, vr_idx,
-                      vr_val, st_idx, n_vr, rec, statB, vel_f, vel, t_est, rounds, chunks, mode, STREAM);
+                      vr_val, st_idx, n_vr, rec, statB, vel_f, vel, t_est, rounds, pass_queue, chunks, mode, STREAM);
 }
 
 extern "C" int vap_velocity_profile(int64_t B, int N_max, int A_max, const double* node_attr, const int32_t* node_flags,
@@ -1292,11 +1317,13 @@
                                     double* kap, double* th, int E_cap, double* max_accels, int32_t* bidx, int32_t* bval,
                                     int32_t* n_ev, int32_t* vr_idx, double* vr_val, int32_t* st_idx, int32_t* n_vr,
                                     float* ins_est, int32_t* ev_scratch, double* rec, double* statB, double* vel_f,
-                                    double* vel, float* t_est, int32_t* rounds, int chunks, int mode, void* stream)
+                                    double* vel, float* t_est, int32_t* rounds, int32_t* pass_queue, int chunks, int mode,
+                                    void* stream)
 {
     if (B <= 0) return 0;
     if (E_cap < N_max + A_max + 2) return arg_err("vap_velocity_profile: E_cap < N_max + A_max + 2");
     if (check_pass_args("vap_velocity_profile", B, D_cap, chunks)) return -1;
+    if (!pass_queue) return arg_err("vap_velocity_profile: pass_queue is NULL");
     if ((t != nullptr) != (kap != nullptr) || (t != nullptr) != (th != nullptr))
         return arg_err("vap_velocity_profile: t, kap and th are inspection outputs: pass all three or none");
     int Am = A_max > 0 ? A_max : 1;
@@ -1328,7 +1355,7 @@
                                                   statB);
     CHECK_LAUNCH("vap_velocity_profile/prepass_ovr");
     return run_passes(B, cons, status, dd, dt, start_vel, end_vel, D_cap, n_samples, E_cap, max_accels, bidx, bval, n_ev, vr_idx,
-                      vr_val, st_idx, n_vr, rec, statB, vel_f, vel, t_est, rounds, chunks, mode, STREAM);
+                      vr_val, st_idx, n_vr, rec, statB, vel_f, vel, t_est, rounds, pass_queue, chunks, mode, STREAM);
 }
 
 extern "C" int vap_time_profile(int64_t B, int N_max, int A_max, const double* node_attr, const int32_t* node_flags,
@@ -1633,8 +1660,8 @@
 struct BatchScratch {
     double *seg, *param_end, *seglen, *scratch9, *lut_d, *lut_t, *total_len, *prop_k, *prop_h, *ma, *vr_val, *rec, *statB, *vel_f,
            *stage;
-    int32_t *first_node, *n_splines, *gstatus, *lut_inv, *bidx, *bval, *n_ev, *vr_idx, *st_idx, *n_vr, *scr, *rounds, *seg_tab,
-            *scr2, *n_main;
+    int32_t *first_node, *n_splines, *gstatus, *lut_inv, *bidx, *bval, *n_ev, *vr_idx, *st_idx, *n_vr, *scr, *rounds, *queue,
+            *seg_tab, *scr2, *n_main;
     float *ins_est, *t_est;
     unsigned long long* need;
     int64_t Q_cap, P_cap, RS; int E_cap;
@@ -1672,6 +1699,7 @@
     s.t_est = w.take<float>(B);
     s.scr = w.take<int32_t>(nscr);
     s.rounds = w.take<int32_t>((size_t)B * 2);
+    s.queue = w.take<int32_t>((size_t)B + 1);
     s.rec = w.take<double>((size_t)B * s.RS * 5);
     s.statB = w.take<double>((size_t)B * s.RS);
     s.vel_f = w.take<double>((size_t)B * s.RS);
@@ -1738,7 +1766,8 @@
                                    status, n_grid, dgrid, lut_samples, s.Q_cap, s.lut_d, s.lut_t, s.total_len, samples_per_node,
                                    s.P_cap, s.prop_k, s.prop_h, s.lut_inv, dd, dt, start_vel, end_vel, D_cap, n_samples, nullptr,
                                    nullptr, nullptr, s.E_cap, s.ma, s.bidx, s.bval, s.n_ev, s.vr_idx, s.vr_val, s.st_idx, s.n_vr,
-                                   s.ins_est, s.scr, s.rec, s.statB, s.vel_f, vel, s.t_est, s.rounds, chunks, 0, stream))) return rc;
+                                   s.ins_est, s.scr, s.rec, s.statB, s.vel_f, vel, s.t_est, s.rounds, s.queue, chunks, 0,
+                                   stream))) return rc;
     k_flag_times<<<blocks_for(B, 128), 128, 0, STREAM>>>(B, status, n_samples, s.t_est, s.ins_est, s.need);
     CHECK_LAUNCH("vap_profile_batch/flag_times");
     if ((rc = vap_time_profile(B, N_max, A_max, node_attr, node_flags, n_nodes, ap_attr, ap_flags, n_ap, cons, status, dt, dd,
diff --git a/vexautonomousplanner_b200/csrc/vap_velocity.cuh b/vexautonomousplanner_b200/csrc/vap_velocity.cuh
--- a/vexautonomousplanner_b200/csrc/vap_velocity.cuh
+++ b/vexautonomousplanner_b200/csrc/vap_velocity.cuh
@@ -615,14 +615,12 @@
 }
 
 #define CH_INT_MAX 2147483647
-#ifndef VAP_PASS_REGS
-#define VAP_PASS_REGS 72
-#endif
 #ifndef VAP_PASS_REGS_TMA
 #define VAP_PASS_REGS_TMA 112
 #endif
 
 __device__ __forceinline__ double2 ldg_d2(const double* p) { return __ldg(reinterpret_cast<const double2*>(p)); }
+__device__ __forceinline__ double2 ld_d2(const double* p) { return *reinterpret_cast<const double2*>(p); }
 __device__ __forceinline__ void st_d2(double* p, double x, double y) { *reinterpret_cast<double2*>(p) = make_double2(x, y); }
 
 #define RERUN_PF 4
@@ -639,7 +637,6 @@
     const int* vi; const double* vv; int n_v;
 };
 
-#define RUN_SWEEP 0
 #define RUN_RERUN 1
 #define RUN_DRY 2
 template <int NT, int MODE>
@@ -650,7 +647,6 @@
     constexpr int PS = PB * NT, BS = 5 * PS;
     constexpr bool RERUN = (MODE == RUN_RERUN);
     constexpr bool DRY = (MODE == RUN_DRY);
-    constexpr bool SWEEP = (MODE == RUN_SWEEP);
     int j = 0;
     while (j + 1 < T.n_b && T.bi[j + 1] <= lo) j++;
     double acc = T.acc[j];
@@ -703,7 +699,6 @@
         if (RERUN) oA = *reinterpret_cast<const double2*>(q + PS);
         FWD_ONE(akB.x, GB.x, stB.x, ghB.x, rgB.x, oB.y)
         if (RERUN) st_d2(q + 2, v2, v);
-        if (SWEEP) { st_d2(q, vin, v1); st_d2(q + 2, v2, v); }
         FWD_ONE(akB.y, GB.y, stB.y, ghB.y, rgB.y, ((e + 1 < hi) ? oA.x : old_end))
         q += PS;
     }
@@ -737,6 +732,7 @@
     unsigned bar;
     int planes;
     unsigned bytes;
+    unsigned phase;
 #ifdef VAP_BOUNDS_CHECK
     const double *rec_lo, *rec_hi, *x_lo, *x_hi;
     unsigned smem_lo, smem_hi, bar_hi;
@@ -779,7 +775,7 @@
 }
 
 template <int NT>
-__device__ __forceinline__ void fwd_sweep_tma(const WarpRing& R, const double* __restrict__ rec_w, int lc, double* __restrict__ q,
+__device__ __forceinline__ void fwd_sweep_tma(WarpRing& R, const double* __restrict__ rec_w, int lc, double* __restrict__ q,
                                               double* __restrict__ tail, int lo, int len, const FwdTables& T, double hw,
                                               double dd, double& v, double& sq)
 {
@@ -813,7 +809,8 @@
         }
     for (int blk = 0; blk < nbw; ++blk) {
         const int s = blk & 1;
-        mbar_wait(R.bar + 8 * s, (blk >> 1) & 1);
+        mbar_wait(R.bar + 8 * s, (R.phase >> s) & 1);
+        R.phase ^= 1u << s;
         const double* S = R.stage + (size_t)s * 5 * PD + lc * PB;
         VAP_CHECK(6, lc >= 0 && lc < 32 && (unsigned)__cvta_generic_to_shared(S + 4 * PD + 3) + 8 <= R.smem_hi);
         if (blk < nfull) {
@@ -856,142 +853,8 @@
     st[0] = v; st[1] = sq;
 }
 
-template <int NT, bool TMA>
-__global__ void __maxnreg__(TMA ? VAP_PASS_REGS_TMA : VAP_PASS_REGS) k_fwd_chunked(
-    const int* __restrict__ status, const double* __restrict__ cons, double dd, double start_vel, double end_vel,
-    long long RS, const int* __restrict__ n_samples, const double* __restrict__ rec, int E_cap,
-    const double* __restrict__ max_accels, const int* __restrict__ bidx, const int* __restrict__ bval,
-    const int* __restrict__ n_ev, const int* __restrict__ vr_idx, const double* __restrict__ vr_val,
-    const int* __restrict__ st_idx, const int* __restrict__ n_vr, double* __restrict__ vfT, int* __restrict__ rounds_out,
-    int warm, int max_rounds, int ring_off)
-{
-    extern __shared__ __align__(128) unsigned char s_mem[];
-    const int c = threadIdx.x;
-    const long long b = blockIdx.x;
-    const int VC = 3 * E_cap + 2;
-    double* s_endv = reinterpret_cast<double*>(s_mem);
-    double* s_endw = s_endv + NT;
-    double* s_usev = s_endw + NT;
-    double* s_usew = s_usev + NT;
-    double* s_acc = s_usew + NT;
-    double* s_vv = s_acc + E_cap;
-    int* s_bi = reinterpret_cast<int*>(s_vv + VC);
-    int* s_vi = s_bi + E_cap;
-    __shared__ int s_nv;
-    if (status[b] != ST_OK) return;
-    const int D = n_samples[b];
-    const int steps = D - 1;
-    double* vf = vfT + (size_t)b * RS;
-    if (c == 0) { vf[0] = start_vel; vf[RS - 1] = start_vel; if (rounds_out) rounds_out[2 * b] = 0; }
-    if (steps <= 0) return;
-    const int n_b = n_ev[2 * b + 1];
-    for (int k = c; k < n_b; k += NT) {
-        s_bi[k] = bidx[(size_t)b * E_cap + k];
-        s_acc[k] = max_accels[(size_t)b * E_cap + bval[(size_t)b * E_cap + k]];
-    }
-    if (c == 0) {
-        const int* vi = vr_idx + (size_t)b * E_cap;
-        const double* vv = vr_val + (size_t)b * E_cap;
-        const int* si = st_idx + (size_t)b * E_cap;
-        const int nvr = n_vr[2 * b], nst = n_vr[2 * b + 1];
-        int pv = 0, ps = 0, pa = 0, n = 0, reg = 0;
-        while (true) {
-            int x = CH_INT_MAX;
-            if (pv < nvr) x = vi[pv];
-            if (ps < nst && si[ps] < x) x = si[ps];
-            if (pa < nst && si[pa] + 1 < x) x = si[pa] + 1;
-            if (x >= D - 1) break;
-            bool stop = false;
-            while (pv < nvr && vi[pv] == x) { reg = pv; pv++; }
-            while (ps < nst && si[ps] == x) { stop = true; ps++; }
-            while (pa < nst && si[pa] + 1 == x) pa++;
-            s_vi[n] = x; s_vv[n] = stop ? 0.01 : vv[reg]; n++;
-        }
-        s_vi[n] = D - 1; s_vv[n] = end_vel; n++;
-        s_nv = n;
-    }
-    const int Lc = chunk_len(steps, NT);
-    const int nch = (steps + Lc - 1) / Lc;
-    const bool active = c < nch;
-    const int lo = c * Lc;
-    const int len = (lo + Lc < steps) ? Lc : steps - lo;
-    const double* P = rec + (size_t)b * RS * 5;
-    double* tail = (active && lo + len == steps) ? vf + (RS - 1) : nullptr;
-    const double hw = cons[b * 6 + 5] * 0.5;
-    WarpRing R;
-    if (TMA) {
-        constexpr int WARPS = (NT + 31) / 32;
-        const int w = c >> 5;
-        R.stage = reinterpret_cast<double*>(s_mem + ring_off) + (size_t)w * 2 * 5 * TMA_PLANE_DOUBLES;
-        R.bar = (unsigned)__cvta_generic_to_shared(s_mem + ring_off + (size_t)WARPS * 2 * 5 * TMA_PLANE_DOUBLES * 8 + 16 * w);
-        R.planes = 5;
-        R.bytes = (NT < 32 ? NT : 32) * PB * 8;
-#ifdef VAP_BOUNDS_CHECK
-        R.rec_lo = P; R.rec_hi = P + 5 * RS; R.x_lo = R.x_hi = nullptr;
-        R.smem_lo = (unsigned)__cvta_generic_to_shared(s_mem + ring_off);
-        R.smem_hi = R.smem_lo + WARPS * 2 * 5 * TMA_PLANE_DOUBLES * 8;
-        R.bar_hi = R.smem_hi + 16 * WARPS;
-#endif
-        if ((c & 31) == 0) { mbar_init(R.bar, 1); mbar_init(R.bar + 8, 1); fence_mbar_init(); }
-    }
-    __syncthreads();
-    FwdTables T;
-    T.bi = s_bi; T.acc = s_acc; T.n_b = n_b; T.vi = s_vi; T.vv = s_vv; T.n_v = s_nv;
-
-    {
-        double v = start_vel, sq = 0.0;
-        if (active) {
-            if (c > 0) {
-                auto v0_at = [&](int x) { int q = 0; while (q + 1 < T.n_v && T.vi[q + 1] <= x) q++; return T.vv[q]; };
-                auto term = [&](int x, int fld) { const int cx = x / Lc, rx = x - cx * Lc; return __ldg(P + rec_index(rx, fld, cx, NT)); };
-                int wl = warm < Lc ? warm : Lc;
-                if (wl > lo - 2) wl = lo - 2 > 0 ? lo - 2 : 0;
-                wl &= ~(PB - 1);
-                const int s0 = lo - wl;
-                const double vm1 = (s0 >= 2) ? pymin(v0_at(s0 - 1), term(s0 - 2, 1)) : start_vel;
-                v = pymin(v0_at(s0), term(s0 - 1, 1));
-                const double wp = vm1 * term(s0 - 1, 0);
-                sq = wp * wp;
-                if (wl > 0) {
-                    double st[2] = {v, sq};
-                    fwd_dry<NT>(P + rec_index(Lc - wl, 0, c - 1, NT), s0, wl, T, hw, dd, st);
-                    v = st[0]; sq = st[1];
-                }
-            }
-            s_usev[c] = v; s_usew[c] = sq;
-            VAP_CHECK(4, c * PB + PB <= PB * NT && (size_t)(((len + 3) >> 2) + 1) * 5 * PB * NT <= (size_t)(5 * RS - 3) &&
-                             (size_t)(((len + 3) >> 2) + 1) * PB * NT <= (size_t)(RS - 1) && lo + len <= steps);
-            if (!TMA) fwd_run<NT, RUN_SWEEP>(P + c * PB, vf + c * PB, tail, 0.0, lo, len, T, hw, dd, v, sq, false);
-        }
-        if (TMA) fwd_sweep_tma<NT>(R, P + (c & ~31) * PB, c & 31, vf + c * PB, tail, lo, active ? len : 0, T, hw, dd, v, sq);
-        s_endv[c] = v; s_endw[c] = sq;
-    }
-    __syncthreads();
-
-    int rounds = 0;
-    for (int round = 1; round < NT && round <= max_rounds; round++) {
-        bool need = false;
-        double in_v = 0.0, in_w = 0.0;
-        if (active && c >= round) {
-            in_v = s_endv[c - 1]; in_w = s_endw[c - 1];
-            need = !(same_bits(in_v, s_usev[c]) && same_bits(in_w, s_usew[c]));
-        }
-        if (!__syncthreads_or(need)) break;
-        rounds = round;
-        if (need) {
-            double st[2] = {in_v, in_w};
-            const bool merged = fwd_rerun<NT>(P + c * PB, vf + c * PB, tail, s_endv[c], lo, len, T, hw, dd, st,
-                                              same_bits(in_v, s_usev[c]));
-            s_usev[c] = in_v; s_usew[c] = in_w;
-            if (!merged) { s_endv[c] = st[0]; s_endw[c] = st[1]; }
-        }
-        __syncthreads();
-    }
-    if (c == 0 && rounds_out) rounds_out[2 * b] = rounds;
-}
-
 template <int NT, int MODE, bool OVR>
-__device__ __forceinline__ bool bwd_run(const double* __restrict__ p, const double* __restrict__ f, double* __restrict__ o,
+__device__ __forceinline__ bool bwd_run(const double* __restrict__ p, const double* f, double* __restrict__ o,
                                         const double* __restrict__ sb, int lo, int len, double top_ak, double top_G,
                                         double top_st, const int* s_bi, const double* s_acc, int n_b, double acc0, double hw,
                                         double dd, double& v, double& sq, bool prev_same, float& est, float dd_over_dt,
@@ -1000,7 +863,6 @@
     constexpr int PS = PB * NT, BS = 5 * PS;
     constexpr bool RERUN = (MODE == RUN_RERUN);
     constexpr bool DRY = (MODE == RUN_DRY);
-    constexpr bool SWEEP = (MODE == RUN_SWEEP);
     int e = lo + len - 1;
     int j = n_b - 1;
     double acc = acc0;
@@ -1025,7 +887,7 @@
     double tak = top_ak, tG = top_G, tst = top_st;
     double oup = old_top;
     for (int r = (len & 3) - 1; r >= 0; --r) {
-        const double gh = __ldg(p + 3 * PS + r), rg = __ldg(p + 4 * PS + r), fv = __ldg(f + r);
+        const double gh = __ldg(p + 3 * PS + r), rg = __ldg(p + 4 * PS + r), fv = f[r];
         const double old = RERUN ? o[r] : 0.0;
         BWD_ONE(tak, tG, tst, gh, rg, fv, old, oup)
         if (!DRY) o[r] = v;
@@ -1046,7 +908,7 @@
             }
     }
     double2 akB = ldg_d2(p + 2), GB = ldg_d2(p + PS + 2), stB = OVR ? ldg_d2(sb + 2) : ldg_d2(p + 2 * PS + 2),
-            ghB = ldg_d2(p + 3 * PS + 2), rgB = ldg_d2(p + 4 * PS + 2), fB = ldg_d2(f + 2);
+            ghB = ldg_d2(p + 3 * PS + 2), rgB = ldg_d2(p + 4 * PS + 2), fB = ld_d2(f + 2);
     double2 akA, GA, stA, ghA, rgA, fA;
     double2 oA = make_double2(0.0, 0.0), oB = oA;
     if (RERUN) oB = *reinterpret_cast<const double2*>(o + 2);
@@ -1059,7 +921,7 @@
             if (OVR) l2_prefetch(sb - (size_t)RERUN_PF * PS);
         }
         akA = ldg_d2(p); GA = ldg_d2(p + PS); stA = OVR ? ldg_d2(sb) : ldg_d2(p + 2 * PS); ghA = ldg_d2(p + 3 * PS); rgA = ldg_d2(p + 4 * PS);
-        fA = ldg_d2(f);
+        fA = ld_d2(f);
         if (RERUN) oA = *reinterpret_cast<const double2*>(o);
         BWD_ONE(tak, tG, tst, ghB.y, rgB.y, fB.y, oB.y, oup)
         const double v3 = v;
@@ -1071,14 +933,13 @@
         const bool more = --blk > 0;
         if (more) {
             akB = ldg_d2(p - BS + 2); GB = ldg_d2(p - BS + PS + 2); stB = OVR ? ldg_d2(sb - PS + 2) : ldg_d2(p - BS + 2 * PS + 2);
-            ghB = ldg_d2(p - BS + 3 * PS + 2); rgB = ldg_d2(p - BS + 4 * PS + 2); fB = ldg_d2(f - PS + 2);
+            ghB = ldg_d2(p - BS + 3 * PS + 2); rgB = ldg_d2(p - BS + 4 * PS + 2); fB = ld_d2(f - PS + 2);
             if (RERUN) oB = *reinterpret_cast<const double2*>(o - PB + 2);
         }
         BWD_ONE(a2, g2, s2, ghA.y, rgA.y, fA.y, oA.y, ob0)
         const double v1 = v;
         BWD_ONE(akA.y, GA.y, stA.y, ghA.x, rgA.x, fA.x, oA.x, oA.y)
         if (RERUN) st_d2(o, v, v1);
-        if (SWEEP) { st_d2(o, v, v1); st_d2(o + 2, v2, v3); }
         if (!more) break;
         oup = oA.x;
         tak = akA.x; tG = GA.x; tst = stA.x;
@@ -1089,7 +950,7 @@
 }
 
 template <int NT>
-__device__ __forceinline__ void bwd_sweep_tma(const WarpRing& R, const double* __restrict__ rec_w, const double* __restrict__ vf_w,
+__device__ __forceinline__ void bwd_sweep_tma(WarpRing& R, const double* __restrict__ rec_w, const double* __restrict__ vf_w,
                                               const double* __restrict__ sb_w, int lc, double* __restrict__ o, int lo, int len,
                                               double top_ak, double top_G, double top_st, const int* s_bi, const double* s_acc,
                                               int n_b, double acc0, double hw, double dd, double& v, double& sq, float& est,
@@ -1124,7 +985,8 @@
     for (int it = 0; it < nbw; ++it) {
         const int rb = nbw - 1 - it;
         const int s = it & 1;
-        mbar_wait(R.bar + 8 * s, (it >> 1) & 1);
+        mbar_wait(R.bar + 8 * s, (R.phase >> s) & 1);
+        R.phase ^= 1u << s;
         const double* S = R.stage + (size_t)s * 6 * PD + lc * PB;
         VAP_CHECK(7, lc >= 0 && lc < 32 && (unsigned)__cvta_generic_to_shared(S + 5 * PD + 3) + 8 <= R.smem_hi);
         if (rb < nfull) {
@@ -1172,154 +1034,258 @@
     st[0] = v; st[1] = sq;
 }
 
-template <int NT, bool TMA>
-__global__ void __maxnreg__(TMA ? VAP_PASS_REGS_TMA : VAP_PASS_REGS) k_bwd_chunked(
-    const int* __restrict__ status, const double* __restrict__ cons, double dd, double dt, double end_vel,
-    long long RS, long long D_cap, const int* __restrict__ n_samples, const double* __restrict__ rec, int E_cap,
-    const double* __restrict__ max_accels, const int* __restrict__ bidx, const int* __restrict__ bval,
-    const int* __restrict__ n_ev, const double* __restrict__ vfT, double* __restrict__ vel, float* __restrict__ t_est,
-    int* __restrict__ rounds_out, int warm, int max_rounds, const double* __restrict__ statB, int ring_off)
+template <int NT>
+__global__ void __maxnreg__(VAP_PASS_REGS_TMA) k_passes_chunked(
+    long long B, const int* __restrict__ order, int* __restrict__ next_path, bool backward,
+    const int* __restrict__ status, const double* __restrict__ cons, double dd, double dt, double start_vel, double end_vel,
+    long long RS, long long D_cap, const int* __restrict__ n_samples, const double* __restrict__ rec,
+    const double* __restrict__ statB, int E_cap, const double* __restrict__ max_accels, const int* __restrict__ bidx,
+    const int* __restrict__ bval, const int* __restrict__ n_ev, const int* __restrict__ vr_idx,
+    const double* __restrict__ vr_val, const int* __restrict__ st_idx, const int* __restrict__ n_vr, double* vfT,
+    double* __restrict__ vel, float* __restrict__ t_est, int* __restrict__ rounds_out, int warm, int max_rounds, int ring_off)
 {
     extern __shared__ __align__(128) unsigned char s_mem[];
-    const int k = threadIdx.x;
-    const long long b = blockIdx.x;
+    constexpr int WARPS = (NT + 31) / 32;
+    constexpr int RING = WARPS * 2 * 6 * TMA_PLANE_DOUBLES * 8;
+    const int c = threadIdx.x;
+    const int VC = 3 * E_cap + 2;
     double* s_endv = reinterpret_cast<double*>(s_mem);
     double* s_endw = s_endv + NT;
     double* s_usev = s_endw + NT;
     double* s_usew = s_usev + NT;
     double* s_acc = s_usew + NT;
-    int* s_bi = reinterpret_cast<int*>(s_acc + E_cap);
-    if (k == 0 && t_est) t_est[b] = 0.f;
-    if (status[b] != ST_OK) return;
-    const int D = n_samples[b];
-    const int steps = D - 1;
-    double* vo = vel + (size_t)b * D_cap;
-    if (k == 0) { vo[D - 1] = end_vel; if (rounds_out) rounds_out[2 * b + 1] = 0; }
-    if (steps <= 0) return;
-    const int n_b = n_ev[2 * b + 1];
-    for (int q = k; q < n_b; q += NT) {
-        s_bi[q] = bidx[(size_t)b * E_cap + q];
-        s_acc[q] = max_accels[(size_t)b * E_cap + bval[(size_t)b * E_cap + q] + 1];
-    }
-    const double acc0 = max_accels[(size_t)b * E_cap + bval[(size_t)b * E_cap + n_b - 1]];
-    const int Lc = chunk_len(steps, NT);
-    const int nch = (steps + Lc - 1) / Lc;
-    const bool active = k < nch;
-    const int col = active ? nch - 1 - k : 0;
-    const int lo = col * Lc;
-    const int len = (lo + Lc < steps) ? Lc : steps - lo;
-    const double* P = rec + (size_t)b * RS * 5;
-    const double* vf = vfT + (size_t)b * RS;
-    const double hw = cons[b * 6 + 5] * 0.5;
-    const bool ovr = pass_has_override(max_accels + (size_t)b * E_cap, n_ev[2 * b], cons[b * 6 + 1]) != 0;
-    const double* SB = statB + (size_t)b * RS;
+    double* s_accb = s_acc + E_cap;
+    double* s_vv = s_accb + E_cap;
+    int* s_bi = reinterpret_cast<int*>(s_vv + VC);
+    int* s_vi = s_bi + E_cap;
+    __shared__ int s_nv, s_q;
     WarpRing R;
-    if (TMA) {
-        constexpr int WARPS = (NT + 31) / 32;
-        const int w = k >> 5;
-        R.stage = reinterpret_cast<double*>(s_mem + ring_off) + (size_t)w * 2 * 6 * TMA_PLANE_DOUBLES;
-        R.bar = (unsigned)__cvta_generic_to_shared(s_mem + ring_off + (size_t)WARPS * 2 * 6 * TMA_PLANE_DOUBLES * 8 + 16 * w);
-        R.planes = 6;
-        R.bytes = (NT < 32 ? NT : 32) * PB * 8;
+    R.stage = reinterpret_cast<double*>(s_mem + ring_off) + (size_t)(c >> 5) * 2 * 6 * TMA_PLANE_DOUBLES;
+    R.bar = (unsigned)__cvta_generic_to_shared(s_mem + ring_off + RING + 16 * (c >> 5));
+    R.bytes = (NT < 32 ? NT : 32) * PB * 8;
+    R.phase = 0;
 #ifdef VAP_BOUNDS_CHECK
-        R.rec_lo = P; R.rec_hi = P + 5 * RS; R.x_lo = vf; R.x_hi = vf + RS;
-        R.smem_lo = (unsigned)__cvta_generic_to_shared(s_mem + ring_off);
-        R.smem_hi = R.smem_lo + WARPS * 2 * 6 * TMA_PLANE_DOUBLES * 8;
-        R.bar_hi = R.smem_hi + 16 * WARPS;
+    R.smem_lo = (unsigned)__cvta_generic_to_shared(s_mem + ring_off);
+    R.smem_hi = R.smem_lo + RING;
+    R.bar_hi = R.smem_hi + 16 * WARPS;
 #endif
-        if ((k & 31) == 0) { mbar_init(R.bar, 1); mbar_init(R.bar + 8, 1); fence_mbar_init(); }
-    }
-    __syncthreads();
-
-    auto rec_of = [&](int x, int fld) {
-        if (fld == 2 && ovr) return __ldg(SB + (x >= steps ? (int)(RS - 1) : edge_slot(x, Lc, NT)));
-        if (x >= steps) return __ldg(P + 5 * RS - 3 + fld);
-        const int cx = x / Lc, rx = x - cx * Lc;
-        return __ldg(P + rec_index(rx, fld, cx, NT));
-    };
-    auto vf_at = [&](int x) { return vf[x >= steps ? (int)(RS - 1) : edge_slot(x, Lc, NT)]; };
-    double top_ak = 0.0, top_G = 0.0, top_st = 0.0;
-    if (active) { top_ak = rec_of(lo + len, 0); top_G = rec_of(lo + len, 1); top_st = rec_of(lo + len, 2); }
-    BwdArgs A;
-    A.p = P + col * PB; A.f = vf + col * PB; A.o = vo + lo; A.sb = SB + col * PB; A.lo = lo; A.len = len;
-    A.top_ak = top_ak; A.top_G = top_G; A.top_st = top_st; A.s_bi = s_bi; A.s_acc = s_acc; A.n_b = n_b; A.acc0 = acc0;
-    A.hw = hw; A.dd = dd; A.dd_over_dt = (float)dd / (float)dt;
-    float est = 0.f;
-
-    {
-        double v = end_vel, sq = 0.0;
-        if (active) {
-            if (k > 0) {
-                const int hi = lo + len;
-                const int len_up = (hi + Lc < steps) ? Lc : steps - hi;
-                int wl = warm < len_up ? warm : len_up;
-                if (hi + wl + 2 > D - 1) wl = (D - 1) - hi - 2 > 0 ? (D - 1) - hi - 2 : 0;
-                wl &= ~(PB - 1);
-                const int s0 = hi + wl;
-                v = pymin(vf_at(s0), rec_of(s0 + 1, 1));
-                double vp1 = end_vel;
-                if (s0 + 2 <= D - 1) vp1 = pymin(vf_at(s0 + 1), rec_of(s0 + 2, 1));
-                const double wp = vp1 * rec_of(s0 + 1, 0);
-                sq = wp * wp;
-                if (wl > 0) {
-                    BwdArgs W = A;
-                    W.p = P + (col + 1) * PB; W.f = vf + (col + 1) * PB; W.o = nullptr; W.sb = SB + (col + 1) * PB;
-                    W.lo = hi; W.len = wl; W.top_ak = rec_of(s0, 0); W.top_G = rec_of(s0, 1); W.top_st = rec_of(s0, 2);
-                    double st[2] = {v, sq};
-                    if (ovr) bwd_dry<NT, true>(W, st); else bwd_dry<NT, false>(W, st);
-                    v = st[0]; sq = st[1];
+    if ((c & 31) == 0) { mbar_init(R.bar, 1); mbar_init(R.bar + 8, 1); fence_mbar_init(); }
+
+    while (true) {
+        if (c == 0) s_q = atomicAdd(next_path, 1);
+        __syncthreads();
+        const int qi = s_q;
+        __syncthreads();
+        if (qi >= B) break;
+        const long long b = order[qi];
+        if (backward && c == 0 && t_est) t_est[b] = 0.f;
+        if (status[b] != ST_OK) continue;
+        const int D = n_samples[b];
+        const int steps = D - 1;
+        double* vf = vfT + (size_t)b * RS;
+        double* vo = vel + (size_t)b * D_cap;
+        if (c == 0) {
+            vf[0] = start_vel; vf[RS - 1] = start_vel;
+            if (rounds_out) rounds_out[2 * b] = 0;
+            if (backward) { vo[D - 1] = end_vel; if (rounds_out) rounds_out[2 * b + 1] = 0; }
+        }
+        if (steps <= 0) continue;
+        const int n_b = n_ev[2 * b + 1];
+        for (int k = c; k < n_b; k += NT) {
+            const int bv = bval[(size_t)b * E_cap + k];
+            s_bi[k] = bidx[(size_t)b * E_cap + k];
+            s_acc[k] = max_accels[(size_t)b * E_cap + bv];
+            s_accb[k] = max_accels[(size_t)b * E_cap + bv + 1];
+        }
+        if (c == 0) {
+            const int* vi = vr_idx + (size_t)b * E_cap;
+            const double* vv = vr_val + (size_t)b * E_cap;
+            const int* si = st_idx + (size_t)b * E_cap;
+            const int nvr = n_vr[2 * b], nst = n_vr[2 * b + 1];
+            int pv = 0, ps = 0, pa = 0, n = 0, reg = 0;
+            while (true) {
+                int x = CH_INT_MAX;
+                if (pv < nvr) x = vi[pv];
+                if (ps < nst && si[ps] < x) x = si[ps];
+                if (pa < nst && si[pa] + 1 < x) x = si[pa] + 1;
+                if (x >= D - 1) break;
+                bool stop = false;
+                while (pv < nvr && vi[pv] == x) { reg = pv; pv++; }
+                while (ps < nst && si[ps] == x) { stop = true; ps++; }
+                while (pa < nst && si[pa] + 1 == x) pa++;
+                s_vi[n] = x; s_vv[n] = stop ? 0.01 : vv[reg]; n++;
+            }
+            s_vi[n] = D - 1; s_vv[n] = end_vel; n++;
+            s_nv = n;
+        }
+        const int Lc = chunk_len(steps, NT);
+        const int nch = (steps + Lc - 1) / Lc;
+        const double* P = rec + (size_t)b * RS * 5;
+        const double hw = cons[b * 6 + 5] * 0.5;
+#ifdef VAP_BOUNDS_CHECK
+        R.rec_lo = P; R.rec_hi = P + 5 * RS; R.x_lo = R.x_hi = nullptr;
+#endif
+        __syncthreads();
+
+        {
+            FwdTables T;
+            T.bi = s_bi; T.acc = s_acc; T.n_b = n_b; T.vi = s_vi; T.vv = s_vv; T.n_v = s_nv;
+            const bool active = c < nch;
+            const int lo = c * Lc;
+            const int len = (lo + Lc < steps) ? Lc : steps - lo;
+            double* tail = (active && lo + len == steps) ? vf + (RS - 1) : nullptr;
+            double v = start_vel, sq = 0.0;
+            if (active) {
+                if (c > 0) {
+                    auto v0_at = [&](int x) { int q = 0; while (q + 1 < T.n_v && T.vi[q + 1] <= x) q++; return T.vv[q]; };
+                    auto term = [&](int x, int fld) { const int cx = x / Lc, rx = x - cx * Lc; return __ldg(P + rec_index(rx, fld, cx, NT)); };
+                    int wl = warm < Lc ? warm : Lc;
+                    if (wl > lo - 2) wl = lo - 2 > 0 ? lo - 2 : 0;
+                    wl &= ~(PB - 1);
+                    const int s0 = lo - wl;
+                    const double vm1 = (s0 >= 2) ? pymin(v0_at(s0 - 1), term(s0 - 2, 1)) : start_vel;
+                    v = pymin(v0_at(s0), term(s0 - 1, 1));
+                    const double wp = vm1 * term(s0 - 1, 0);
+                    sq = wp * wp;
+                    if (wl > 0) {
+                        double st[2] = {v, sq};
+                        fwd_dry<NT>(P + rec_index(Lc - wl, 0, c - 1, NT), s0, wl, T, hw, dd, st);
+                        v = st[0]; sq = st[1];
+                    }
                 }
-            }
-            s_usev[k] = v; s_usew[k] = sq;
-            VAP_CHECK(5, col >= 0 && col * PB + PB <= PB * NT && (size_t)(((len + 3) >> 2) + 1) * 5 * PB * NT <= (size_t)(5 * RS - 3) &&
-                             (size_t)(((len + 3) >> 2) + 1) * PB * NT <= (size_t)(RS - 1) && A.o + len <= vo + D - 1 &&
-                             lo + len <= steps && D <= D_cap);
-            if (!TMA) {
-                if (ovr) bwd_run<NT, RUN_SWEEP, true>(A.p, A.f, A.o, A.sb, lo, len, top_ak, top_G, top_st, s_bi, s_acc, n_b, acc0, hw,
-                                                      dd, v, sq, false, est, A.dd_over_dt);
-                else bwd_run<NT, RUN_SWEEP, false>(A.p, A.f, A.o, A.sb, lo, len, top_ak, top_G, top_st, s_bi, s_acc, n_b, acc0, hw,
-                                                   dd, v, sq, false, est, A.dd_over_dt);
-            }
-        }
-        if (TMA) {
-            const int col_hi = nch - 1 - (k & ~31);
-            const int cs = col_hi > 31 ? col_hi - 31 : 0;
-            bwd_sweep_tma<NT>(R, P + cs * PB, vf + cs * PB, ovr ? SB + cs * PB : nullptr, active ? col - cs : 0, vo + lo, lo,
-                              active ? len : 0, top_ak, top_G, top_st, s_bi, s_acc, n_b, acc0, hw, dd, v, sq, est, A.dd_over_dt);
-        }
-        s_endv[k] = v; s_endw[k] = sq;
-    }
-    __syncthreads();
-
-    int rounds = 0;
-    for (int round = 1; round < NT && round <= max_rounds; round++) {
-        bool need = false;
-        double in_v = 0.0, in_w = 0.0;
-        if (active && k >= round) {
-            in_v = s_endv[k - 1]; in_w = s_endw[k - 1];
-            need = !(same_bits(in_v, s_usev[k]) && same_bits(in_w, s_usew[k]));
-        }
-        if (!__syncthreads_or(need)) break;
-        rounds = round;
-        if (need) {
-            double st[2] = {in_v, in_w};
-            const bool ps = same_bits(in_v, s_usev[k]);
-            const bool merged = ovr ? bwd_rerun<NT, true>(A, st, &est, ps, s_usev[k]) : bwd_rerun<NT, false>(A, st, &est, ps, s_usev[k]);
-            s_usev[k] = in_v; s_usew[k] = in_w;
-            if (!merged) { s_endv[k] = st[0]; s_endw[k] = st[1]; }
-        }
+                s_usev[c] = v; s_usew[c] = sq;
+                VAP_CHECK(4, b >= 0 && b < B && c * PB + PB <= PB * NT &&
+                                 (size_t)(((len + 3) >> 2) + 1) * 5 * PB * NT <= (size_t)(5 * RS - 3) &&
+                                 (size_t)(((len + 3) >> 2) + 1) * PB * NT <= (size_t)(RS - 1) && lo + len <= steps);
+            }
+            R.planes = 5;
+            fwd_sweep_tma<NT>(R, P + (c & ~31) * PB, c & 31, vf + c * PB, tail, lo, active ? len : 0, T, hw, dd, v, sq);
+            s_endv[c] = v; s_endw[c] = sq;
+            __syncthreads();
+
+            int rounds = 0;
+            for (int round = 1; round < NT && round <= max_rounds; round++) {
+                bool need = false;
+                double in_v = 0.0, in_w = 0.0;
+                if (active && c >= round) {
+                    in_v = s_endv[c - 1]; in_w = s_endw[c - 1];
+                    need = !(same_bits(in_v, s_usev[c]) && same_bits(in_w, s_usew[c]));
+                }
+                if (!__syncthreads_or(need)) break;
+                rounds = round;
+                if (need) {
+                    double st[2] = {in_v, in_w};
+                    const bool merged = fwd_rerun<NT>(P + c * PB, vf + c * PB, tail, s_endv[c], lo, len, T, hw, dd, st,
+                                                      same_bits(in_v, s_usev[c]));
+                    s_usev[c] = in_v; s_usew[c] = in_w;
+                    if (!merged) { s_endv[c] = st[0]; s_endw[c] = st[1]; }
+                }
+                __syncthreads();
+            }
+            if (c == 0 && rounds_out) rounds_out[2 * b] = rounds;
+        }
+        if (!backward) continue;
+        fence_proxy_async_global();
         __syncthreads();
-    }
-    if (k == 0 && rounds_out) rounds_out[2 * b + 1] = rounds;
-
-    __syncthreads();
-    float* s_f = reinterpret_cast<float*>(s_endv);
-    s_f[k] = active ? est : 0.f;
-    __syncthreads();
-    if (k == 0 && t_est) {
-        float tot = 0.f;
-        for (int q = 0; q < NT; q++) tot += s_f[q];
-        t_est[b] = tot;
+
+        {
+            const int k = c;
+            const double acc0 = s_acc[n_b - 1];
+            const bool active = k < nch;
+            const int col = active ? nch - 1 - k : 0;
+            const int lo = col * Lc;
+            const int len = (lo + Lc < steps) ? Lc : steps - lo;
+            const bool ovr = pass_has_override(max_accels + (size_t)b * E_cap, n_ev[2 * b], cons[b * 6 + 1]) != 0;
+            const double* SB = statB + (size_t)b * RS;
+#ifdef VAP_BOUNDS_CHECK
+            R.x_lo = vf; R.x_hi = vf + RS;
+#endif
+            auto rec_of = [&](int x, int fld) {
+                if (fld == 2 && ovr) return __ldg(SB + (x >= steps ? (int)(RS - 1) : edge_slot(x, Lc, NT)));
+                if (x >= steps) return __ldg(P + 5 * RS - 3 + fld);
+                const int cx = x / Lc, rx = x - cx * Lc;
+                return __ldg(P + rec_index(rx, fld, cx, NT));
+            };
+            auto vf_at = [&](int x) { return vf[x >= steps ? (int)(RS - 1) : edge_slot(x, Lc, NT)]; };
+            double top_ak = 0.0, top_G = 0.0, top_st = 0.0;
+            if (active) { top_ak = rec_of(lo + len, 0); top_G = rec_of(lo + len, 1); top_st = rec_of(lo + len, 2); }
+            BwdArgs A;
+            A.p = P + col * PB; A.f = vf + col * PB; A.o = vo + lo; A.sb = SB + col * PB; A.lo = lo; A.len = len;
+            A.top_ak = top_ak; A.top_G = top_G; A.top_st = top_st; A.s_bi = s_bi; A.s_acc = s_accb; A.n_b = n_b; A.acc0 = acc0;
+            A.hw = hw; A.dd = dd; A.dd_over_dt = (float)dd / (float)dt;
+            float est = 0.f;
+
+            double v = end_vel, sq = 0.0;
+            if (active) {
+                if (k > 0) {
+                    const int hi = lo + len;
+                    const int len_up = (hi + Lc < steps) ? Lc : steps - hi;
+                    int wl = warm < len_up ? warm : len_up;
+                    if (hi + wl + 2 > D - 1) wl = (D - 1) - hi - 2 > 0 ? (D - 1) - hi - 2 : 0;
+                    wl &= ~(PB - 1);
+                    const int s0 = hi + wl;
+                    v = pymin(vf_at(s0), rec_of(s0 + 1, 1));
+                    double vp1 = end_vel;
+                    if (s0 + 2 <= D - 1) vp1 = pymin(vf_at(s0 + 1), rec_of(s0 + 2, 1));
+                    const double wp = vp1 * rec_of(s0 + 1, 0);
+                    sq = wp * wp;
+                    if (wl > 0) {
+                        BwdArgs W = A;
+                        W.p = P + (col + 1) * PB; W.f = vf + (col + 1) * PB; W.o = nullptr; W.sb = SB + (col + 1) * PB;
+                        W.lo = hi; W.len = wl; W.top_ak = rec_of(s0, 0); W.top_G = rec_of(s0, 1); W.top_st = rec_of(s0, 2);
+                        double st[2] = {v, sq};
+                        if (ovr) bwd_dry<NT, true>(W, st); else bwd_dry<NT, false>(W, st);
+                        v = st[0]; sq = st[1];
+                    }
+                }
+                s_usev[k] = v; s_usew[k] = sq;
+                VAP_CHECK(5, b >= 0 && b < B && col >= 0 && col * PB + PB <= PB * NT &&
+                                 (size_t)(((len + 3) >> 2) + 1) * 5 * PB * NT <= (size_t)(5 * RS - 3) &&
+                                 (size_t)(((len + 3) >> 2) + 1) * PB * NT <= (size_t)(RS - 1) && A.o + len <= vo + D - 1 &&
+                                 lo + len <= steps && D <= D_cap);
+            }
+            {
+                const int col_hi = nch - 1 - (k & ~31);
+                const int cs = col_hi > 31 ? col_hi - 31 : 0;
+                R.planes = 6;
+                bwd_sweep_tma<NT>(R, P + cs * PB, vf + cs * PB, ovr ? SB + cs * PB : nullptr, active ? col - cs : 0, vo + lo, lo,
+                                  active ? len : 0, top_ak, top_G, top_st, s_bi, s_accb, n_b, acc0, hw, dd, v, sq, est,
+                                  A.dd_over_dt);
+            }
+            s_endv[k] = v; s_endw[k] = sq;
+            __syncthreads();
+
+            int rounds = 0;
+            for (int round = 1; round < NT && round <= max_rounds; round++) {
+                bool need = false;
+                double in_v = 0.0, in_w = 0.0;
+                if (active && k >= round) {
+                    in_v = s_endv[k - 1]; in_w = s_endw[k - 1];
+                    need = !(same_bits(in_v, s_usev[k]) && same_bits(in_w, s_usew[k]));
+                }
+                if (!__syncthreads_or(need)) break;
+                rounds = round;
+                if (need) {
+                    double st[2] = {in_v, in_w};
+                    const bool ps = same_bits(in_v, s_usev[k]);
+                    const bool merged = ovr ? bwd_rerun<NT, true>(A, st, &est, ps, s_usev[k]) : bwd_rerun<NT, false>(A, st, &est, ps, s_usev[k]);
+                    s_usev[k] = in_v; s_usew[k] = in_w;
+                    if (!merged) { s_endv[k] = st[0]; s_endw[k] = st[1]; }
+                }
+                __syncthreads();
+            }
+            if (k == 0 && rounds_out) rounds_out[2 * b + 1] = rounds;
+
+            __syncthreads();
+            float* s_f = reinterpret_cast<float*>(s_endv);
+            s_f[k] = active ? est : 0.f;
+            __syncthreads();
+            if (k == 0 && t_est) {
+                float tot = 0.f;
+                for (int q = 0; q < NT; q++) tot += s_f[q];
+                t_est[b] = tot;
+            }
+        }
     }
 }
 
diff --git a/vexautonomousplanner_b200/engine.py b/vexautonomousplanner_b200/engine.py
--- a/vexautonomousplanner_b200/engine.py
+++ b/vexautonomousplanner_b200/engine.py
@@ -304,6 +304,7 @@
         vel_f = self._empty((B, RS)); vel = outs["vel"] if outs else self._empty((B, D_cap))
         t_est = self._empty((B,), torch.float32)
         rounds = torch.zeros((B, 2), dtype=torch.int32, device=self.device)
+        queue = self._empty((B + 1,), torch.int32)
         inv = t.lut_inv if self.accelerators else None
         if fused:
             with self._stage("S345_velocity"):
@@ -315,9 +316,9 @@
                     C.c_double(self.dd), C.c_double(self.dt), C.c_double(self.start_vel), C.c_double(self.end_vel),
                     C.c_int64(D_cap), _p(n_samples), _p(tq), _p(kap), _p(th), C.c_int(E_cap), _p(ma), _p(bidx), _p(bval),
                     _p(n_ev), _p(vr_idx), _p(vr_val), _p(st_idx), _p(n_vr), _p(ins_est), _p(scr), _p(rec), _p(statB),
-                    _p(vel_f), _p(vel), _p(t_est), _p(rounds), C.c_int(chunks), C.c_int(mode), self._stream()),
-                    "vap_velocity_profile")
-                self.launches += 6 if mode == 0 else 6
+                    _p(vel_f), _p(vel), _p(t_est), _p(rounds), _p(queue), C.c_int(chunks), C.c_int(mode),
+                    self._stream()), "vap_velocity_profile")
+                self.launches += 6 if mode == 0 else 7
         else:
             with self._stage("S3_dist_sample"):
                 _lib.check(self.lib.vap_dist_sample_events(
@@ -334,7 +335,8 @@
                     C.c_int64(B), _p(db.cons), _p(status), C.c_double(self.dd), C.c_double(self.dt), C.c_double(self.start_vel),
                     C.c_double(self.end_vel), C.c_int64(D_cap), _p(n_samples), _p(kap), _p(th), C.c_int(E_cap), _p(ma),
                     _p(bidx), _p(bval), _p(n_ev), _p(vr_idx), _p(vr_val), _p(st_idx), _p(n_vr), _p(rec), _p(statB),
-                    _p(vel_f), _p(vel), _p(t_est), _p(rounds), C.c_int(chunks), C.c_int(mode), self._stream()), "vap_fwd_bwd_chunked")
+                    _p(vel_f), _p(vel), _p(t_est), _p(rounds), _p(queue), C.c_int(chunks), C.c_int(mode), self._stream()),
+                    "vap_fwd_bwd_chunked")
                 self.launches += 3
         extra = dict(t=tq, kap=kap, th=th, max_accels=ma, bidx=bidx, bval=bval, n_ev=n_ev, vel_f=vel_f, rounds=rounds,
                      vr_idx=vr_idx, vr_val=vr_val, st_idx=st_idx, n_vr=n_vr)
```

Result: faster. 1.261 million (median of 6 runs) (+3.6%).
